# Intel-HLS/GenomicsDB

Measured on AMD Instinct MI355X. Metric: combined-gVCF positions/sec, higher is better.
Workload: dtype u8/int32

## Files before the change

__graft_entry__.py:

```python
import os
import sys

ROOT = os.path.dirname(os.path.abspath(__file__))
sys.path.insert(0, ROOT)
sys.path.insert(0, os.path.join(ROOT, "tests"))


def build():
    from genomicsdb_amd import build as b
    lib = b.build_native(verbose=True)
    b.build_oracle()
    b.build_hostsim()
    b.build_hostsim_variants()
    b.build_hostsim_import()
    b.build_hostsim_inflate()
    b.build_hostsim_import_bcf()
    b.build_hostsim_import_csv()
    b.build_hostsim_dispatch()
    b.build_hostsim_merge()
    b.build_hostsim_merge_files()
    b.build_hostsim_split()
    b.build_hostsim_histogram()
    b.build_hostsim_index()
    b.build_hostsim_vcfdiff()
    b.build_hostsim_import_stream()
    b.build_hostsim_columns()
    b.build_jni_importer_harness()
    from genomicsdb_amd import synth
    synth.lib()
    import genomicsdb_amd
    from genomicsdb_amd import _lib
    L = _lib.lib()
    for s in _lib.SYMBOLS:
        getattr(L, s)
    print("built", lib)


def smoke():
    import helpers
    from golden_cases import CASES
    import genomicsdb_amd
    case = [c for c in CASES if c[0] == "t6_7_8_vcf_at_0"][0]
    name, callsets, vid, ov, golden, mode = case
    cells = helpers.cells_for(callsets, vid)
    q, pb = helpers.query_json(callsets, vid, ov, mode)
    want, _, _ = helpers.oracle_run(q, cells)
    s = genomicsdb_amd.GenomicsDBQueryStream(query_json=q, cells=cells, buffer_capacity=4096)
    got = s.read()
    s.close()
    assert got == want, "device output differs from the oracle"
    assert got == helpers.golden_text(golden)
    print("smoke ok: %d bytes, bit-exact vs oracle and reference golden" % len(got))


if __name__ == "__main__":
    build()
    if len(sys.argv) > 1 and sys.argv[1] == "smoke":
        smoke()
```

genomicsdb_amd/build.py:

```python
import os
import subprocess
import sys

PKG = os.path.dirname(os.path.abspath(__file__))
ROOT = os.path.dirname(PKG)
CSRC = os.path.join(PKG, "csrc")
OBJ = os.path.join(ROOT, "build", "obj")
LIB = os.path.join(PKG, "libgenomicsdb_amd.so")
TOOL = os.path.join(PKG, "gt_mpi_gather")
TOOLS = {"gt_mpi_gather": TOOL, "vcf2tiledb": os.path.join(PKG, "vcf2tiledb"), "test_genomicsdb_importer": os.path.join(PKG, "test_genomicsdb_importer"),
         "vcf_histogram": os.path.join(PKG, "vcf_histogram"), "vcfdiff": os.path.join(PKG, "vcfdiff")}

SOURCES = [
    "kernels/gdb_pipeline.hip",
    "kernels/gdb_bgzf.hip",
    "kernels/gdb_import.hip",
    "kernels/gdb_import_stream.hip",
    "kernels/gdb_inflate.hip",
    "kernels/gdb_merge.hip",
    "kernels/gdb_split.hip",
    "kernels/gdb_histogram.hip",
    "kernels/gdb_index.hip",
    "kernels/gdb_vcfdiff.hip",
    "kernels/gdb_columns.hip",
# ... 83 lines not shown

def build_hostsim():
    subprocess.check_call(["make", "-s", "-C", os.path.join(ROOT, "tests", "hostsim")])
    subprocess.check_call(["make", "-s", "-C", os.path.join(ROOT, "tests", "jni_harness")])
    subprocess.check_call(["make", "-s", "-C", os.path.join(ROOT, "tests", "compat")])


def build_hostsim_variants():
    subprocess.check_call(["make", "-s", "-C", os.path.join(ROOT, "tests", "hostsim_variants")])
    return os.path.join(ROOT, "tests", "hostsim_variants", "libhostsim_variants.so")


def build_hostsim_import():
    subprocess.check_call(["make", "-s", "-C", os.path.join(ROOT, "tests", "hostsim_import")])
    return os.path.join(ROOT, "tests", "hostsim_import", "libhostsim_import.so")


def build_hostsim_import_bcf():
    d = os.path.join(ROOT, "tests", "hostsim_import_bcf")
    subprocess.check_call(["make", "-s", "-C", d])
    return os.path.join(d, "libhostsim_import_bcf.so"), os.path.join(d, "malformed_bcf")


def build_hostsim_import_csv():
    d = os.path.join(ROOT, "tests", "hostsim_import_csv")
    subprocess.check_call(["make", "-s", "-C", d])
    return os.path.join(d, "libhostsim_import_csv.so"), os.path.join(d, "hostsim_import_csv_main")


def build_hostsim_import_stream():
    d = os.path.join(ROOT, "tests", "hostsim_import_stream")
    subprocess.check_call(["make", "-s", "-C", d])
    return os.path.join(d, "libhostsim_import_stream.so"), os.path.join(d, "hostsim_import_stream_main")


def build_jni_importer_harness():
    d = os.path.join(ROOT, "tests", "jni_importer_harness")
    subprocess.check_call(["make", "-s", "-C", d])
    return os.path.join(d, "jni_importer_harness")


def build_hostsim_merge():
    d = os.path.join(ROOT, "tests", "hostsim_merge")
    subprocess.check_call(["make", "-s", "-C", d])
    return os.path.join(d, "libhostsim_merge.so"), os.path.join(d, "hostsim_merge_main")


def build_hostsim_merge_files():
    d = os.path.join(ROOT, "tests", "hostsim_merge_files")
    subprocess.check_call(["make", "-s", "-C", d])
    return os.path.join(d, "libhostsim_merge_files.so"), os.path.join(d, "hostsim_merge_files_main")


def build_hostsim_split():
    d = os.path.join(ROOT, "tests", "hostsim_split")
    subprocess.check_call(["make", "-s", "-C", d])
    return os.path.join(d, "hostsim_split")


def build_hostsim_histogram():
    d = os.path.join(ROOT, "tests", "hostsim_histogram")
    subprocess.check_call(["make", "-s", "-C", d])
    return os.path.join(d, "hostsim_histogram")


def build_hostsim_index():
    d = os.path.join(ROOT, "tests", "hostsim_index")
    subprocess.check_call(["make", "-s", "-C", d])
    return os.path.join(d, "libhostsim_index.so"), os.path.join(d, "hostsim_index")


def build_hostsim_vcfdiff():
    d = os.path.join(ROOT, "tests", "hostsim_vcfdiff")
    subprocess.check_call(["make", "-s", "-C", d])
    return os.path.join(d, "hostsim_vcfdiff")


def build_hostsim_columns():
    d = os.path.join(ROOT, "tests", "hostsim_columns")
    subprocess.check_call(["make", "-s", "-C", d])
    return os.path.join(d, "libhostsim_columns.so"), os.path.join(d, "hostsim_columns_main")


def build_hostsim_inflate():
    subprocess.check_call(["make", "-s", "-C", os.path.join(ROOT, "tests", "hostsim_inflate")])
    return os.path.join(ROOT, "tests", "hostsim_inflate", "libhostsim_inflate.so")


def build_hostsim_tile_inflate():
    d = os.path.join(ROOT, "tests", "hostsim_tile_inflate")
    subprocess.check_call(["make", "-s", "-C", d])
    return os.path.join(d, "libhostsim_tile_inflate.so"), os.path.join(d, "tile_inflate_fuzz")


def build_hostsim_dispatch():
    subprocess.check_call(["make", "-s", "-C", os.path.join(ROOT, "tests", "hostsim_dispatch")])
    return os.path.join(ROOT, "tests", "hostsim_dispatch", "libhostsim_dispatch.so")


if __name__ == "__main__":
    print(build_native(verbose=True))
    print(build_oracle())
```

genomicsdb_amd/csrc/core/gdb_core.hpp:

```cpp
#pragma once
#include "gdb_types.h"

#if defined(__HIP_DEVICE_COMPILE__)
#define GDB_FETCH_ADD_U64(p, v) atomicAdd((unsigned long long*)(p), (unsigned long long)(v))
#else
static inline unsigned long long gdb_fetch_add_u64(unsigned long long* p, unsigned long long v) { const unsigned long long o = *p; *p = o + v; return o; }
#define GDB_FETCH_ADD_U64(p, v) gdb_fetch_add_u64((unsigned long long*)(p), (unsigned long long)(v))
#endif

#define GDB_CF_REFBLOCK 1u
#define GDB_CF_DELETION 2u
#define GDB_CF_HAS_NR 4u
#define GDB_CF_HEAVY 8u
#define GDB_CF_IN_WINDOW 16u
#define GDB_CF_NALT(f) (((f) >> 8) & 0xFFu)
#define GDB_CF_PLOIDY(f) (((f) >> 16) & 0xFu)

#define GDB_RF_NON_REF_EXISTS 1u
#define GDB_RF_REMAPPING_NEEDED 2u
#define GDB_RF_SKIP_G_FIELDS 4u

#define GDB_IF_SPANNING 1u
#define GDB_IF_GT_OVERRIDE 2u
#define GDB_IF_NO_NR 4u
// ... 58 lines not shown
};
struct ByteSink {
  char* p;
  char* base;
  GDB_HD explicit ByteSink(char* q) : p(q), base(q) {}
  GDB_HD void put(char c) { *p++ = c; }
  GDB_HD void write(const char* s, int len) { for (int i = 0; i < len; ++i) *p++ = s[i]; }
  GDB_HD uint32_t pos() const { return (uint32_t)(p - base); }
  GDB_HD void patch_u32(uint32_t at, uint32_t v) { for (int i = 0; i < 4; ++i) base[at + i] = (char)((v >> (8 * i)) & 0xFFu); }
};

#if defined(__HIPCC__)
typedef __attribute__((address_space(3))) char gdb_lds_char;
struct LdsCapSink {
  gdb_lds_char* p;
  uint32_t n, cap;
  __device__ __forceinline__ LdsCapSink(gdb_lds_char* q, uint32_t c) : p(q), n(0), cap(c) {}
  __device__ __forceinline__ void put(char c) { if (n < cap) p[n] = c; ++n; }
  __device__ __forceinline__ void write(const char* s, int len) { for (int i = 0; i < len; ++i) put(s[i]); }
  __device__ __forceinline__ void put_word(uint64_t w, int len) {
    if (n + 8u <= cap) { const uint32_t a = (uint32_t)(uintptr_t)p + n; asm volatile("ds_write_b64 %0, %1" ::"v"(a), "v"(w) : "memory"); n += (uint32_t)len; }
    else for (int i = 0; i < len; ++i) { put((char)(w & 0xFFu)); w >>= 8; }
  }
  __device__ __forceinline__ uint32_t pos() const { return n; }
  __device__ __forceinline__ void patch_u32(uint32_t at, uint32_t v) { for (int i = 0; i < 4; ++i) if (at + i < cap) p[at + i] = (char)((v >> (8 * i)) & 0xFFu); }
};
constexpr uint32_t kSpillTail = 512;
struct SpillPool { char* buf; };
struct LdsSpillSink {
  gdb_lds_char* p;
  uint32_t n, cap;
  uint32_t acc;
  char* tail;
  __device__ __forceinline__ LdsSpillSink(gdb_lds_char* q, uint32_t c, const SpillPool& sp, int64_t record) : p(q), n(0), cap(c), acc(0), tail(sp.buf + (size_t)record * kSpillTail) {}
  __device__ __forceinline__ void put(char c) {
    if (n < cap) p[n] = c;
    else {
      const uint32_t at = n - cap;
      acc |= (uint32_t)(uint8_t)c << (8u * (at & 3u));
      if ((at & 3u) == 3u) { if (at < kSpillTail) *reinterpret_cast<uint32_t*>(tail + (at & ~3u)) = acc; acc = 0; }
    }
    ++n;
  }
  __device__ __forceinline__ void flush() { if (n > cap && ((n - cap) & 3u) && n - cap < kSpillTail) { *reinterpret_cast<uint32_t*>(tail + ((n - cap) & ~3u)) = acc; acc = 0; } }
  __device__ __forceinline__ void write(const char* s, int len) { for (int i = 0; i < len; ++i) put(s[i]); }
  __device__ __forceinline__ void put_word(uint64_t w, int len) {
    if (n + 8u <= cap) { const uint32_t a = (uint32_t)(uintptr_t)p + n; asm volatile("ds_write_b64 %0, %1" ::"v"(a), "v"(w) : "memory"); n += (uint32_t)len; }
    else for (int i = 0; i < len; ++i) { put((char)(w & 0xFFu)); w >>= 8; }
  }
  __device__ __forceinline__ bool complete() const { return n <= cap + kSpillTail; }
  __device__ __forceinline__ uint32_t pos() const { return n; }
  __device__ __forceinline__ void patch_u32(uint32_t at, uint32_t v) { for (int i = 0; i < 4; ++i) if (at + i < cap) p[at + i] = (char)((v >> (8 * i)) & 0xFFu); }
};
#endif

GDB_HD uint32_t gdb_f2u(float f) { union { float f; uint32_t u; } x; x.f = f; return x.u; }
GDB_HD bool gdb_int_valid(int32_t v) { return v != GDB_BCF_INT32_MISSING && v != GDB_BCF_INT32_VECTOR_END; }
GDB_HD bool gdb_float_valid(float v) { uint32_t u = gdb_f2u(v); return u != GDB_BCF_FLOAT_MISSING_BITS && u != GDB_BCF_FLOAT_VECTOR_END_BITS; }
GDB_HD int gdb_alleles2gt(int a, int b) { return a > b ? a * (a + 1) / 2 + b : b * (b + 1) / 2 + a; }
GDB_HD int64_t gdb_choose(int n, int k) {
  if (k < 0 || k > n) return 0;
  int64_t r = 1;
  for (int i = 1; i <= k; ++i) r = r * (n - k + i) / i;
  return r;
}
GDB_HD int64_t gdb_genotype_index_sorted(const int* a, int p) {
  int64_t g = 0;
  for (int i = 0; i < p; ++i) g += gdb_choose(a[i] + i, i + 1);
  return g;
}
GDB_HD int64_t gdb_genotype_index(const int* a, int p) {
  int t[GDB_MAX_PLOIDY];
  for (int i = 0; i < p; ++i) { int v = a[i], j = i; while (j > 0 && t[j - 1] > v) { t[j] = t[j - 1]; --j; } t[j] = v; }
  return gdb_genotype_index_sorted(t, p);
}
GDB_HD bool gdb_next_genotype(int* a, int p, int nalleles) {
  for (int i = 0; i < p; ++i) {
    const int bound = i + 1 < p ? a[i + 1] : nalleles - 1;
    if (a[i] < bound) { ++a[i]; for (int j = 0; j < i; ++j) a[j] = 0; return true; }
  }
  return false;
}

template <class Sink> GDB_HD void put_u64(Sink& s, uint64_t v) {
  char buf[20];
  int n = 0;
  do { buf[n++] = (char)('0' + (v % 10)); v /= 10; } while (v);
  while (n) s.put(buf[--n]);
}
template <class Sink> GDB_HD void put_i64(Sink& s, int64_t v) {
  if (v < 0) { s.put('-'); put_u64(s, (uint64_t)(-(v + 1)) + 1u); } else put_u64(s, (uint64_t)v);
}
GDB_HD uint64_t gdb_pack_digits(uint32_t v, int& n) {
  uint64_t w = 0;
  n = 0;
  do { const uint32_t q = v / 10u; w = (w << 8) | (uint64_t)('0' + (v - q * 10u)); v = q; ++n; } while (v);
  return w;
}
template <class Sink> GDB_HD void put_packed(Sink& s, uint64_t w, int n) {
  for (int i = 0; i < n; ++i) { s.put((char)(w & 0xFFu)); w >>= 8; }
}
#if defined(__HIPCC__)
__device__ __forceinline__ void put_packed(LdsCapSink& s, uint64_t w, int n) { s.put_word(w, n); }
__device__ __forceinline__ void put_packed(LdsSpillSink& s, uint64_t w, int n) { s.put_word(w, n); }
#endif
template <class Sink> GDB_HD void put_u32(Sink& s, uint32_t v) {
  if (v < 10u) { s.put((char)('0' + v)); return; }
  if (v < 100u) { const uint32_t q = v / 10u; s.put((char)('0' + q)); s.put((char)('0' + (v - q * 10u))); return; }
  int n = 0;
  if (v >= 100000000u) {
    const uint32_t hi = v / 100000000u;
    v -= hi * 100000000u;
    const uint64_t wh = gdb_pack_digits(hi, n);
    put_packed(s, wh, n);
    uint64_t w = gdb_pack_digits(v, n);
    for (; n < 8; ++n) w = (w << 8) | (uint64_t)'0';
    put_packed(s, w, 8);
    return;
  }
  const uint64_t w = gdb_pack_digits(v, n);
  put_packed(s, w, n);
}
template <class Sink> GDB_HD void put_i32(Sink& s, int32_t v) {
  if (v < 0) { s.put('-'); put_u32(s, 0u - (uint32_t)v); } else put_u32(s, (uint32_t)v);
}

struct GdbBig { uint32_t w[7]; };
GDB_HD void gdb_big_mul10(GdbBig& b) {
  uint64_t c = 0;
  for (int i = 0; i < 7; ++i) { const uint64_t t = (uint64_t)b.w[i] * 10u + c; b.w[i] = (uint32_t)t; c = t >> 32; }
}
GDB_HD uint32_t gdb_big_divmod10(GdbBig& b) {
  uint64_t r = 0;
  for (int i = 6; i >= 0; --i) { const uint64_t t = (r << 32) | b.w[i]; b.w[i] = (uint32_t)(t / 10u); r = t % 10u; }
  return (uint32_t)r;
}
GDB_HD bool gdb_big_is_zero(const GdbBig& b) { uint32_t o = 0; for (int i = 0; i < 7; ++i) o |= b.w[i]; return o == 0; }
GDB_HD uint32_t gdb_big_bit(const GdbBig& b, int i) { return i >= 0 && i < 224 ? (b.w[i >> 5] >> (i & 31)) & 1u : 0u; }
GDB_HD bool gdb_big_any_below(const GdbBig& b, int n) {
  uint32_t o = 0;
  for (int i = 0; i < 7; ++i) {
    const int lo = i * 32;
    if (n >= lo + 32) o |= b.w[i]; else if (n > lo) o |= b.w[i] & ((1u << (n - lo)) - 1u);
  }
  return o != 0;
}
GDB_HD GdbBig gdb_big_shr(const GdbBig& b, int n) {
  GdbBig r;
  const int ws = n >> 5, bs = n & 31;
  for (int i = 0; i < 7; ++i) {
    const uint32_t lo = i + ws < 7 ? b.w[i + ws] : 0u, hi = i + ws + 1 < 7 ? b.w[i + ws + 1] : 0u;
    r.w[i] = bs ? (lo >> bs) | (hi << (32 - bs)) : lo;
  }
  return r;
}
GDB_HD bool gdb_big_below(const GdbBig& b, uint32_t v) { uint32_t o = 0; for (int i = 1; i < 7; ++i) o |= b.w[i]; return o == 0 && b.w[0] < v; }
GDB_HD void gdb_round_6_digits(uint32_t M, int e2, uint32_t& q, int& X) {
  GdbBig N;
  for (int i = 0; i < 7; ++i) N.w[i] = 0;
  N.w[0] = M;
  bool up;
  if (e2 >= 0 || !gdb_big_below(gdb_big_shr(N, -e2), 100000u)) {
    int s = 0;
    if (e2 >= 0) { const int ws = e2 >> 5, bs = e2 & 31; N.w[ws] = M << bs; N.w[0] = ws ? 0u : N.w[0]; if (bs && ws + 1 < 7) N.w[ws + 1] = M >> (32 - bs); }
    else s = -e2;
    GdbBig I = gdb_big_shr(N, s);
    const bool half_bit = s > 0 && gdb_big_bit(N, s - 1);
    bool sticky = s > 1 && gdb_big_any_below(N, s - 1);
    int dropped = 0;
    uint32_t last = 0;
    while (!gdb_big_below(I, 1000000u)) { if (dropped) sticky = sticky || last != 0; else sticky = sticky || half_bit; last = gdb_big_divmod10(I); ++dropped; }
    q = I.w[0];
    if (dropped) up = last > 5u || (last == 5u && (sticky || (q & 1u)));
    else up = half_bit && (sticky || (q & 1u));
    X = 5 + dropped;
  } else {
    const int s = -e2;
    int k = 0;
    while (gdb_big_below(gdb_big_shr(N, s), 100000u)) { gdb_big_mul10(N); ++k; }
    q = gdb_big_shr(N, s).w[0];
    const bool half_bit = gdb_big_bit(N, s - 1) != 0, sticky = s > 1 && gdb_big_any_below(N, s - 1);
    up = half_bit && (sticky || (q & 1u));
    X = 5 - k;
  }
  if (up && ++q == 1000000u) { q = 100000u; ++X; }
}
template <class Sink> GDB_HD void put_float_g(Sink& s, float f) {
  const uint32_t u = gdb_f2u(f) & 0x7FFFFFFFu;
  const uint32_t ex = u >> 23, man = u & 0x7FFFFFu;
  uint32_t q; int X;
  gdb_round_6_digits(ex ? man | 0x800000u : man, ex ? (int)ex - 150 : -149, q, X);
  char dg[6];
  for (int i = 5; i >= 0; --i) { dg[i] = (char)('0' + q % 10u); q /= 10u; }
  int last = 5;
  while (last > 0 && dg[last] == '0') --last;
  if (X < -4 || X >= 6) {
    s.put(dg[0]);
    if (last > 0) { s.put('.'); for (int i = 1; i <= last; ++i) s.put(dg[i]); }
    s.put('e');
    uint32_t ax = (uint32_t)(X < 0 ? -X : X);
    s.put(X < 0 ? '-' : '+');
    if (ax < 10u) s.put('0');
    put_u64(s, ax);
  } else if (X >= 0) {
    for (int i = 0; i <= X; ++i) s.put(dg[i]);
    if (last > X) { s.put('.'); for (int i = X + 1; i <= last; ++i) s.put(dg[i]); }
  } else {
    s.put('0'); s.put('.');
    for (int i = 0; i < -X - 1; ++i) s.put('0');
    for (int i = 0; i <= last; ++i) s.put(dg[i]);
  }
}

template <class Sink> GDB_HD bool put_float(Sink& s, float f) {
  const uint32_t bits = gdb_f2u(f);
  if ((bits & 0x7F800000u) == 0x7F800000u) {
    if (bits >> 31) s.put('-');
    if (bits & 0x7FFFFFu) { s.put('n'); s.put('a'); s.put('n'); } else { s.put('i'); s.put('n'); s.put('f'); }
    return true;
  }
  double d = (double)f;
  if (d == 0) { if (bits >> 31) s.put('-'); s.put('0'); return true; }
  if (d < 0) { s.put('-'); d = -d; }
  if (!(d >= 0.0001 && d <= 999999)) { put_float_g(s, f); return true; }
  uint64_t i = (uint64_t)(d * 10000000000.0);
  if (d < 0.001) i += 5; else if (d < 0.01) i += 50; else if (d < 0.1) i += 500; else if (d < 1) i += 5000;
  else if (d < 10) i += 50000; else if (d < 100) i += 500000; else if (d < 1000) i += 5000000;
  else if (d < 10000) i += 50000000; else if (d < 100000) i += 500000000; else i += 5000000000ULL;
  char dg[24];
  int p = 0;
  { char tmp[24]; int n = 0; do { tmp[n++] = (char)('0' + i % 10); i /= 10; } while (i); while (n) dg[p++] = tmp[--n]; }
  char out[40];
  int m = 0, dot = -1;
  if (p <= 10) {
    out[m++] = '0'; dot = m; out[m++] = '.';
    for (int z = 0; z < 10 - p; ++z) out[m++] = '0';
    int take = p < 6 ? p : 6;
    for (int z = 0; z < take; ++z) out[m++] = dg[z];
  } else {
    int ip = p - 10;
    for (int z = 0; z < ip; ++z) out[m++] = dg[z];
    if (ip < 6) { dot = m; out[m++] = '.'; for (int z = ip; z < 6; ++z) out[m++] = dg[z]; }
  }
  if (dot >= 0) while (m > dot + 2 && out[m - 1] == '0') --m;
  s.write(out, m);
  return true;
}

template <class T> GDB_HD const T* cell_field(const FragmentView& fr, const CombinePlan& pl, int f, int64_t c, int& n) {
  const GdbColumn& col = fr.col[f];
  if (col.off) { uint32_t a = col.off[c], b = col.off[c + 1]; n = (int)(b - a); return (const T*)col.data + a; }
  n = pl.field[f].fixed_num;
  return (const T*)col.data + (int64_t)c * n;
}
GDB_HD bool field_valid(const CellMeta& cm, int64_t c, int f) { return (cm.vmask[c] >> f) & 1ull; }

GDB_HD bool alt_token(const char* s, int len, int idx, const char*& tok, int& tlen) {
  int i = 0, k = -1;
  while (i < len) {
    while (i < len && s[i] == '|') ++i;
    if (i >= len) break;
    int j = i;
    while (j < len && s[j] != '|') ++j;
    if (++k == idx) { tok = s + i; tlen = j - i; return true; }
    i = j;
  }
  return false;
}
GDB_HD bool allele_is_symbolic(const char* a, int n) {
  if (n > 0 && a[0] == '&') return true;
  if (n == 1 && a[0] == '*') return true;
  if (n > 0 && a[0] == '<' && a[n - 1] == '>') return true;
  for (int i = 0; i < n; ++i) if (a[i] == '[' || a[i] == ']') return true;
  return false;
}
GDB_HD bool allele_is_deletion(int ref_len, const char* a, int n) {
  return ref_len > 1 && ((n == 1 && a[0] == '*') || (!allele_is_symbolic(a, n) && n < ref_len));
}

GDB_HD void classify_cell(const FragmentView& fr, const CombinePlan& pl, const CellMeta& cm, int64_t c, uint32_t* err) {
  uint64_t vmask = 0;
  for (int f = 0; f < pl.nfields; ++f) {
    const GdbFieldDesc& fd = pl.field[f];
    int n;
    bool valid = false;
    if (fd.elem == GDB_ET_INT) {
      const int32_t* p = cell_field<int32_t>(fr, pl, f, c, n);
      for (int i = 0; i < n; ++i) if (p[i] != GDB_TILEDB_NULL_INT32) { valid = true; break; }
    } else if (fd.elem == GDB_ET_FLOAT) {
      const float* p = cell_field<float>(fr, pl, f, c, n);
      for (int i = 0; i < n; ++i) if (gdb_f2u(p[i]) != GDB_TILEDB_NULL_FLOAT_BITS) { valid = true; break; }
    } else {
      const char* p = cell_field<char>(fr, pl, f, c, n);
      for (int i = 0; i < n; ++i) if (p[i] != GDB_TILEDB_NULL_CHAR) { valid = true; break; }
    }
    if (valid) vmask |= 1ull << f;
  }
  uint32_t flags = 0;
  int nalt = 0, ref_len = 0;
  if (pl.f_REF >= 0 && pl.f_ALT >= 0 && ((vmask >> pl.f_REF) & 1) && ((vmask >> pl.f_ALT) & 1)) {
    int alt_len;
    cell_field<char>(fr, pl, pl.f_REF, c, ref_len);
    const char* alt = cell_field<char>(fr, pl, pl.f_ALT, c, alt_len);
    bool deletion = false, has_nr = false;
    const char* tok; int tl;
    for (int i = 0; alt_token(alt, alt_len, i, tok, tl); ++i) {
      ++nalt;
      if (tl > 0 && tok[0] == '&') has_nr = true;
      if (ref_len > 1 && !allele_is_symbolic(tok, tl) && tl < ref_len) deletion = true;
    }
    if (deletion) flags |= GDB_CF_DELETION;
    if (has_nr) flags |= GDB_CF_HAS_NR;
    if (ref_len == 1 && nalt == 1 && has_nr) flags |= GDB_CF_REFBLOCK;
  }
  if (nalt + 1 > GDB_MAX_INPUT_ALLELES) { *err |= GDB_ERR_TOO_MANY_INPUT_ALLELES; nalt = GDB_MAX_INPUT_ALLELES - 1; }
  int ploidy = 0;
  if (pl.f_GT >= 0 && ((vmask >> pl.f_GT) & 1)) {
    int n;
    cell_field<int32_t>(fr, pl, pl.f_GT, c, n);
    ploidy = pl.field[pl.f_GT].length == GDB_VL_PP ? (n + 1) >> 1 : n;
    if (ploidy > 15) ploidy = 15;
  }
  bool heavy = !(flags & GDB_CF_REFBLOCK);
  for (int i = 0; i < pl.n_info; ++i) if ((vmask >> pl.info_field[i]) & 1) heavy = true;
  for (int i = 0; i < pl.n_histogram; ++i) if ((vmask >> pl.histogram_bin_field[i]) & 1) heavy = true;
  if (pl.qual_combine_op != GDB_OP_UNKNOWN && pl.f_QUAL >= 0 && ((vmask >> pl.f_QUAL) & 1)) heavy = true;
  if (pl.produce_FILTER_field && pl.f_FILTER >= 0 && ((vmask >> pl.f_FILTER) & 1)) heavy = true;
  if (pl.f_ID >= 0 && ((vmask >> pl.f_ID) & 1)) heavy = true;
  if (heavy) flags |= GDB_CF_HEAVY;
  flags |= ((uint32_t)nalt & 0xFFu) << 8;
  flags |= ((uint32_t)ploidy & 0xFu) << 16;
  int32_t dp = 0;
  {
    int n; bool got = false;
    if (pl.f_DP >= 0 && ((vmask >> pl.f_DP) & 1)) { const int32_t* p = cell_field<int32_t>(fr, pl, pl.f_DP, c, n); if (n > 0 && gdb_int_valid(p[0])) { dp = p[0]; got = true; } }
    if (!got && pl.f_MIN_DP >= 0 && ((vmask >> pl.f_MIN_DP) & 1)) { const int32_t* p = cell_field<int32_t>(fr, pl, pl.f_MIN_DP, c, n); if (n > 0 && gdb_int_valid(p[0])) { dp = p[0]; got = true; } }
    if (!got && pl.f_DP_FORMAT >= 0 && ((vmask >> pl.f_DP_FORMAT) & 1)) { const int32_t* p = cell_field<int32_t>(fr, pl, pl.f_DP_FORMAT, c, n); if (n > 0 && gdb_int_valid(p[0])) { dp = p[0]; got = true; } }
  }
  cm.vmask[c] = vmask;
  cm.cflags[c] = flags;
  cm.dpval[c] = dp;
}

GDB_HD uint32_t allele_hash(const char* p, int len, int suffix_from, const char* mref, int mref_len) {
  uint32_t h = 2166136261u;
  for (int i = 0; i < len; ++i) h = (h ^ (uint32_t)(unsigned char)p[i]) * 16777619u;
  if (suffix_from >= 0) for (int i = suffix_from; i < mref_len; ++i) h = (h ^ (uint32_t)(unsigned char)mref[i]) * 16777619u;
  return h;
}

GDB_HD bool allele_equal(const AlleleRef& a, const AlleleRef& b, const char* mref, int mref_len) {
  if (a.hash != b.hash) return false;
  int la = a.len + (a.suffix_from >= 0 ? mref_len - a.suffix_from : 0);
  int lb = b.len + (b.suffix_from >= 0 ? mref_len - b.suffix_from : 0);
  if (la != lb) return false;
  for (int i = 0; i < la; ++i) {
    char ca = i < a.len ? a.p[i] : mref[a.suffix_from + (i - a.len)];
    char cb = i < b.len ? b.p[i] : mref[b.suffix_from + (i - b.len)];
    if (ca != cb) return false;
  }
  return true;
}

struct MedianOrder {
  const uint64_t* keys;
  const uint32_t* inc;
  int64_t stride;
  int8_t slot[GDB_MAX_FIELDS];
  int32_t enabled;
};
GDB_HD uint32_t gdb_orderable_bits(float v) {
  uint32_t u = gdb_f2u(v);
  if (u == 0x80000000u) u = 0;
  return (u & 0x80000000u) ? ~u : (u | 0x80000000u);
}
GDB_HD uint32_t gdb_orderable_bits(int32_t v) { return (uint32_t)v ^ 0x80000000u; }

struct BigMedians {
  const int32_t* index;
  const uint32_t* value;
  const uint8_t* ok;
  int64_t stride;
  int8_t slot[GDB_MAX_FIELDS];
  int32_t enabled;
};

GDB_HD void gdb_swapf(float* a, int64_t i, int64_t j) { const float t = a[i]; a[i] = a[j]; a[j] = t; }
GDB_HD void gdb_heap_adjust(float* a, int64_t hole, int64_t len, float value) {
  const int64_t top = hole;
// ... 191 lines not shown
  ++s.n;
}
GDB_HD void gdb_id_union_add(const char* p, int len, const char** tp, int* tn, int& nt, GdbUSetHashOrder& us, int release_order, uint32_t* err) {
  if (release_order) {
    for (int i = 0; i < nt; ++i) {
      if (tn[i] != len) continue;
      bool same = true;
      for (int j = 0; j < len && same; ++j) same = tp[i][j] == p[j];
      if (same) return;
    }
    if (nt >= GDB_MAX_ID_TOKENS) { *err |= GDB_ERR_TOO_MANY_ID_TOKENS; return; }
    tp[nt] = p; tn[nt] = len;
    gdb_useth_insert_new(us, gdb_libstdcxx_hash_bytes(p, len), nt);
    ++nt;
    return;
  }
  int pos = 0, cmp = 1;
  for (; pos < nt; ++pos) {
    const int m = len < tn[pos] ? len : tn[pos];
    cmp = 0;
    for (int j = 0; j < m && cmp == 0; ++j) cmp = (int)(unsigned char)p[j] - (int)(unsigned char)tp[pos][j];
    if (cmp == 0) cmp = len - tn[pos];
    if (cmp <= 0) break;
  }
  if (pos == nt || cmp != 0) {
    if (nt >= GDB_MAX_ID_TOKENS) { *err |= GDB_ERR_TOO_MANY_ID_TOKENS; }
    else { for (int j = nt; j > pos; --j) { tp[j] = tp[j - 1]; tn[j] = tn[j - 1]; } tp[pos] = p; tn[pos] = len; ++nt; }
  }
}
GDB_HD void gdb_id_union_value(const char* p, int n, const char** tp, int* tn, int& nt, GdbUSetHashOrder& us, int release_order, uint32_t* err) {
  int last = 0;
  for (int i = 0; i <= n; ++i) {
    if (i < n && p[i] != ';') continue;
    const int len = i - last;
    if (i == n && len == 0) break;
    gdb_id_union_add(p + last, len, tp, tn, nt, us, release_order, err);
    last = i + 1;
  }
}
GDB_HD int gdb_id_union_at(const GdbUSetHashOrder& us, int release_order, int i) { return release_order ? us.tok[i] : i; }

struct TieScratch {
  float* buf;
  unsigned long long* used;
  uint64_t capacity;
};

struct ScalarPre {
  const uint32_t* val;
  int64_t stride;
  int8_t slot[GDB_MAX_FIELDS];
  int32_t enabled;
};

struct HugeScalar { int64_t nvalid, nbelow, nneg0, npos0; uint32_t sum_bits, median_bits; int32_t median_ok, pad; };
struct HugeSiteOut {
  AlleleRef merged[GDB_MAX_MERGED_ALLELES];
  const char* mref;
  int32_t mref_len, nmerged;
  int32_t filter_first_id, filter_multi, any_id, fallback;
  HugeScalar scalar[GDB_MAX_INFO_FIELDS + 2];
};
struct HugeSites {
  const int32_t* index;
  const HugeSiteOut* out;
  int32_t enabled;
};

struct SiteCtx {
  FragmentView fr;
  CombinePlan pl;
  CellMeta cm;
  RecordTable rec;
  HeavyLists hl;
  PresenceCounts pc;
  NameTables names;
  QueryWindow qw;
  SiteOut so;
  MedianOrder med;
  BigMedians big;
  TieScratch tie;
  ScalarPre pre;
  HugeSites huge;
};

GDB_HD bool inc_is_spanning(const SiteCtx& cx, int64_t t, int64_t s_k) {
  int64_t c = cx.hl.cell[t];
  return (cx.cm.cflags[c] & GDB_CF_DELETION) && s_k > cx.fr.begin[c];
}
template <class T> GDB_HD bool scalar_at(const SiteCtx& cx, const uint32_t* pre, int64_t t, int64_t s_k, int f, bool keep_spanning, bool is_float, T& v,
                                         int alt_merged = 0, bool non_ref_exists = false) {
  if (pre) {
    union { uint32_t u; T v; } x;
    x.u = pre[t];
    if (is_float ? x.u == GDB_BCF_FLOAT_MISSING_BITS : x.u == (uint32_t)GDB_BCF_INT32_MISSING) return false;
    v = x.v;
    return true;
  }
  if (!keep_spanning && inc_is_spanning(cx, t, s_k)) return false;
  const int64_t c = cx.hl.cell[t];
  if (!field_valid(cx.cm, c, f)) return false;
  int n;
  const T* p = cell_field<T>(cx.fr, cx.pl, f, c, n);
  int idx = 0;
  if (alt_merged > 0) {
    const int8_t* lut = cx.hl.i2m + cx.hl.i2m_off[t];
    const int nal = (int)GDB_CF_NALT(cx.cm.cflags[c]) + 1;
    int in = -1;
    for (int a = 0; a < nal; ++a) if (lut[a] == 1) { in = a; break; }
    if (in < 0 && non_ref_exists) for (int a = 0; a < nal; ++a) if (lut[a] == alt_merged - 1) in = a;
    idx = in - 1;
    if (in < 0 || idx < 0 || idx >= n) return false;
  }
  v = p[idx];
  return is_float ? gdb_float_valid((float)v) : gdb_int_valid((int32_t)v);
}
template <class T> GDB_HD bool reduce_scalar(const SiteCtx& cx, int64_t k, int f, int op, bool keep_spanning, T& result, uint32_t* err, int num_merged = 0,
                                             bool non_ref_exists = false, bool remapping_needed = false) {
  const int alt_merged = (remapping_needed && cx.pl.field[f].length == GDB_VL_A) ? num_merged : 0;
  const int64_t b = cx.hl.base[k], e = cx.hl.base[k + 1];
  if (op == GDB_OP_MEDIAN && cx.big.enabled && cx.big.slot[f] >= 0 && cx.big.index[k] >= 0) {
    const int64_t at = (int64_t)cx.big.slot[f] * cx.big.stride + cx.big.index[k];
    if (!cx.big.ok[at]) return false;
    if (cx.big.ok[at] == 1) {
      union { uint32_t u; T v; } x;
      x.u = cx.big.value[at];
      result = x.v;
      return true;
    }
  }
  const int64_t s_k = cx.rec.start[k];
  const bool is_float = cx.pl.field[f].elem == GDB_ET_FLOAT;
  const uint32_t* pre = (cx.pre.enabled && cx.pre.slot[f] >= 0) ? cx.pre.val + (int64_t)cx.pre.slot[f] * cx.pre.stride : nullptr;
  int64_t nvalid = 0, nbelow = 0, nneg0 = 0, npos0 = 0;
  T sum = 0;
  const HugeSiteOut* hs = (cx.huge.enabled && pre && cx.huge.index[k] >= 0 && !cx.huge.out[cx.huge.index[k]].fallback) ? &cx.huge.out[cx.huge.index[k]] : nullptr;
  if (hs) {
    const HugeScalar& hv = hs->scalar[cx.pre.slot[f]];
    nvalid = hv.nvalid; nbelow = hv.nbelow; nneg0 = hv.nneg0; npos0 = hv.npos0;
    union { uint32_t u; T v; } x;
    x.u = hv.sum_bits; sum = x.v;
    if (nvalid && op == GDB_OP_MEDIAN && hv.median_ok == 1) { x.u = hv.median_bits; result = x.v; return true; }
  } else
  for (int64_t t = b; t < e; ++t) {
    T v;
    if (!scalar_at<T>(cx, pre, t, s_k, f, keep_spanning, is_float, v, alt_merged, non_ref_exists)) continue;
    sum += v;
    ++nvalid;
    if (is_float) {
      const uint32_t u = gdb_f2u((float)v);
      nneg0 += u == 0x80000000u;
      npos0 += u == 0u;
      nbelow += v < (T)0;
    }
  }
  if (!nvalid) return false;
  if (op == GDB_OP_SUM) { result = sum; return true; }
  if (op == GDB_OP_MEAN) {
    if (is_float) result = sum / (T)nvalid;
    else result = (T)(int32_t)((uint32_t)(int32_t)sum / (uint32_t)nvalid);
    return true;
  }
  if (is_float && nneg0 && npos0 && nbelow <= nvalid / 2 && nvalid / 2 < nbelow + nneg0 + npos0) {
    const uint64_t at = cx.tie.buf ? GDB_FETCH_ADD_U64(cx.tie.used, (uint64_t)nvalid) : 0;
    if (!cx.tie.buf || at + (uint64_t)nvalid > cx.tie.capacity) { *err |= GDB_ERR_INTERNAL; return false; }
    float* a = cx.tie.buf + at;
// ... 213 lines not shown
}

template <class T, class Sink> GDB_HD bool info_vector_combine_bcf(const SiteCtx& cx, int64_t k, int f, int op, int num_merged, bool non_ref_exists, bool remapping_needed,
                                                                 Sink& sink, uint32_t* err) {
  const CombinePlan& pl = cx.pl;
  const GdbFieldDesc& fd = pl.field[f];
  const int64_t b = cx.hl.base[k], e = cx.hl.base[k + 1];
  const int64_t s_k = cx.rec.start[k];
  const int mode = info_element_mode(fd, remapping_needed);
  const bool is_float = fd.elem == GDB_ET_FLOAT;
  T r[GDB_MAX_INFO_VECTOR];
  int num_valid = 0;
  int n_total = 0;
  int32_t mn = INT32_MAX, mx = INT32_MIN + 1;
  int type = is_float ? GDB_BT_FLOAT : GDB_BT_INT8;
  for (int pass = (op == GDB_OP_CONCATENATE ? 0 : 1); pass < 2; ++pass) {
    if (pass == 1 && op == GDB_OP_CONCATENATE) {
      if (n_total == 0) return false;
      bcf_enc_int1(sink, pl.bcf_id[f]);
      if (!is_float) type = bcf_int_type(mn, mx);
      if (!is_float && n_total == 1) {}
      bcf_enc_size(sink, n_total, type);
    }
    for (int64_t t = b; t < e; ++t) {
      if (inc_is_spanning(cx, t, s_k)) continue;
      const int64_t c = cx.hl.cell[t];
      if (!field_valid(cx.cm, c, f)) continue;
      int n_in;
      const T* p = cell_field<T>(cx.fr, pl, f, c, n_in);
      info_for_each_element<T>(p, n_in, mode, cx.hl.i2m + cx.hl.i2m_off[t], (int)GDB_CF_NALT(cx.cm.cflags[c]) + 1, num_merged, non_ref_exists, (int)GDB_CF_PLOIDY(cx.cm.cflags[c]), err,
                               [&](int i, T v) -> bool {
        if (op == GDB_OP_CONCATENATE) {
          if (pass == 0) {
            ++n_total;
            if (!is_float && !elem_is_missing(v) && !elem_is_vector_end(v)) { const int32_t iv = (int32_t)v; if (iv < mn) mn = iv; if (iv > mx) mx = iv; }
          } else if (is_float) { union { T t; uint32_t u; } x; x.u = 0; x.t = v; bcf_put_u32(sink, x.u); }
          else bcf_put_int(sink, (int32_t)v, type);
          return true;
        }
        if (elem_is_missing(v) || elem_is_vector_end(v)) return true;
        if (i >= GDB_MAX_INFO_VECTOR) { *err |= GDB_ERR_INFO_VECTOR_TOO_LONG; return false; }
        if (i < num_valid && !elem_is_missing(r[i])) r[i] += v;
        else { r[i] = v; if (i >= num_valid) { for (int j = num_valid; j < i; ++j) elem_set_missing(r[j]); num_valid = i + 1; } }
        return true;
      });
    }
  }
  if (op == GDB_OP_CONCATENATE) return true;
  if (num_valid == 0) return false;
  bcf_enc_int1(sink, pl.bcf_id[f]);
  if (is_float) {
    bcf_enc_size(sink, num_valid, GDB_BT_FLOAT);
    for (int i = 0; i < num_valid; ++i) { union { T t; uint32_t u; } x; x.u = 0; x.t = r[i]; bcf_put_u32(sink, x.u); }
  } else {
    int32_t tmp[GDB_MAX_INFO_VECTOR];
    for (int i = 0; i < num_valid; ++i) tmp[i] = (int32_t)r[i];
    bcf_enc_vint(sink, tmp, num_valid);
  }
  return true;
}

#include "gdb_asa.hpp"

constexpr int kMergeScan = 8;
struct MergeIndex { uint8_t slot[256]; bool built; };
GDB_HD int merged_find_or_add(AlleleRef* merged, int& nmerged, MergeIndex& ix, const AlleleRef& cand, const char* mref, int mref_len, uint32_t* err) {
  if (nmerged <= kMergeScan) {
    for (int j = 1; j < nmerged; ++j) if (allele_equal(merged[j], cand, mref, mref_len)) return j;
  } else {
    if (!ix.built) {
      for (int h = 0; h < 256; ++h) ix.slot[h] = 0;
      for (int j = 1; j < nmerged; ++j) { uint32_t h = merged[j].hash & 255u; while (ix.slot[h]) h = (h + 1) & 255u; ix.slot[h] = (uint8_t)j; }
      ix.built = true;
    }
    for (uint32_t h = cand.hash & 255u; ix.slot[h]; h = (h + 1) & 255u)
      if (allele_equal(merged[ix.slot[h]], cand, mref, mref_len)) return ix.slot[h];
  }
  if (nmerged >= GDB_MAX_MERGED_ALLELES - 1) { *err |= GDB_ERR_TOO_MANY_MERGED_ALLELES; return nmerged - 1; }
  merged[nmerged] = cand;
  if (ix.built) { uint32_t h = cand.hash & 255u; while (ix.slot[h]) h = (h + 1) & 255u; ix.slot[h] = (uint8_t)nmerged; }
  return nmerged++;
}

GDB_HD const char* site_first_ref(const SiteCtx& cx, int64_t s_k, int& len) {
  int64_t lo = 0, hi = cx.fr.ncells;
  while (lo < hi) { int64_t mid = (lo + hi) >> 1; if (cx.fr.begin[mid] < s_k) lo = mid + 1; else hi = mid; }
  len = 0;
  if (lo < cx.fr.ncells && cx.fr.begin[lo] == s_k && field_valid(cx.cm, lo, cx.pl.f_REF)) return cell_field<char>(cx.fr, cx.pl, cx.pl.f_REF, lo, len);
  return nullptr;
}
GDB_HD const char* gdb_star_allele() { return "*"; }
template <class F> GDB_HD void site_merge_call(const SiteCtx& cx, int64_t t, int64_t s_k, const char* mref, int mref_len, bool write_luts, F& find_or_add, uint32_t* err) {
  const CombinePlan& pl = cx.pl;
    int64_t c = cx.hl.cell[t];
    uint32_t cf = cx.cm.cflags[c];
    int ref_len = 0, alt_len = 0;
    cell_field<char>(cx.fr, pl, pl.f_REF, c, ref_len);
    const char* alt = cell_field<char>(cx.fr, pl, pl.f_ALT, c, alt_len);
    int nalt = (int)GDB_CF_NALT(cf);
    int8_t* lut = write_luts ? cx.hl.i2m + cx.hl.i2m_off[t] : nullptr;
    bool spanning = (cf & GDB_CF_DELETION) && s_k > cx.fr.begin[c];
    uint8_t iflag = 0;
    if (lut) { lut[0] = 0; for (int a = 1; a <= nalt; ++a) lut[a] = -1; }
    if (spanning) {
      iflag |= GDB_IF_SPANNING;
      if (!(cf & GDB_CF_HAS_NR)) iflag |= GDB_IF_NO_NR;
      int ploidy = (int)GDB_CF_PLOIDY(cf);
      int npl = 0;
      const int32_t* plv = nullptr;
      bool pl_exists = pl.f_PL >= 0 && field_valid(cx.cm, c, pl.f_PL);
      if (pl_exists) plv = cell_field<int32_t>(cx.fr, pl, pl.f_PL, c, npl);
      int lowest = -1;
      int lowest_pl = 0x7FFFFFFF;
      const char* tok; int tl;
      for (int i = 0; alt_token(alt, alt_len, i, tok, tl); ++i) {
        int aidx = i + 1;
        if (allele_is_deletion(ref_len, tok, tl)) {
          if (lowest < 0) lowest = aidx;
          if (pl_exists) {
            int64_t gt_idx;
            if (ploidy == 0) gt_idx = 0;
            else if (ploidy == 1) gt_idx = aidx;
            else if (ploidy == 2) gt_idx = gdb_alleles2gt(aidx, aidx);
            else if (ploidy <= GDB_MAX_PLOIDY) { int hom[GDB_MAX_PLOIDY]; for (int q = 0; q < ploidy; ++q) hom[q] = aidx; gt_idx = gdb_genotype_index_sorted(hom, ploidy); }
            else { *err |= GDB_ERR_UNSUPPORTED_PLOIDY; gt_idx = 0x7FFFFFFF; }
            if (gt_idx < npl && plv[gt_idx] < lowest_pl) { lowest_pl = plv[gt_idx]; lowest = aidx; }
          }
        }
      }
      if (lowest < 0) { *err |= GDB_ERR_INTERNAL; lowest = 1; }
      AlleleRef cand{gdb_star_allele(), 1, -1, 0u};
      cand.hash = allele_hash(cand.p, cand.len, cand.suffix_from, mref, mref_len);
      const int found = find_or_add(cand);
      if (lut) lut[lowest] = (int8_t)found;
      if (lut && pl.min_PL_GT_for_spanning_deletions && pl.produce_GT_field && pl_exists && pl.f_GT >= 0 && field_valid(cx.cm, c, pl.f_GT)) {
        int nr_idx = -1;
        for (int i = 0; alt_token(alt, alt_len, i, tok, tl); ++i) if (tl > 0 && tok[0] == '&') nr_idx = i + 1;
        int red2in[3] = {0, lowest, nr_idx};
        int nred = nr_idx >= 0 ? 3 : 2;
        int best_min = 0x7FFFFFFF, best_a = -1, best_b = -1;
        if (ploidy == 1) {
          for (int a = 0; a < nred; ++a) {
            int64_t gi = red2in[a];
            int32_t v = gi < npl ? plv[gi] : GDB_BCF_INT32_MISSING;
            if (gdb_int_valid(v) && v < best_min) { best_min = v; best_a = a; }
          }
        } else if (ploidy == 2) {
          for (int a = 0; a < nred; ++a) for (int b2 = a; b2 < nred; ++b2) {
            int64_t gi = gdb_alleles2gt(red2in[a], red2in[b2]);
            int32_t v = gi < npl ? plv[gi] : GDB_BCF_INT32_MISSING;
            if (gdb_int_valid(v) && v < best_min) { best_min = v; best_a = a; best_b = b2; }
          }
        } else if (ploidy <= GDB_MAX_PLOIDY) {
          int g[GDB_MAX_PLOIDY], in[GDB_MAX_PLOIDY];
          for (int q = 0; q < ploidy; ++q) g[q] = 0;
          do {
            for (int q = 0; q < ploidy; ++q) in[q] = red2in[g[q]];
            const int64_t gi = gdb_genotype_index(in, ploidy);
            const int32_t v = gi < npl ? plv[gi] : GDB_BCF_INT32_MISSING;
            if (gdb_int_valid(v) && v < best_min) {
              best_min = v; best_a = g[0];
              for (int q = 0; q < ploidy; ++q) cx.hl.gt_override[GDB_MAX_PLOIDY * t + q] = (int8_t)g[q];
            }
          } while (gdb_next_genotype(g, ploidy, nred));
        } else *err |= GDB_ERR_UNSUPPORTED_PLOIDY;
        if (best_a >= 0) {
          iflag |= GDB_IF_GT_OVERRIDE;
          if (ploidy <= 2) {
            cx.hl.gt_override[GDB_MAX_PLOIDY * t] = (int8_t)best_a;
            cx.hl.gt_override[GDB_MAX_PLOIDY * t + 1] = (int8_t)best_b;
          }
        }
      }
    } else {
      bool suffix_needed = ref_len < mref_len;
      const char* tok; int tl;
      for (int i = 0; alt_token(alt, alt_len, i, tok, tl); ++i) {
        if (tl > 0 && tok[0] == '&') continue;
        AlleleRef cand{tok, tl, (suffix_needed && !allele_is_symbolic(tok, tl)) ? ref_len : -1, 0u};
        cand.hash = allele_hash(cand.p, cand.len, cand.suffix_from, mref, mref_len);
        const int found = find_or_add(cand);
        if (lut && i + 1 <= nalt) lut[i + 1] = (int8_t)found;
      }
    }
    if (write_luts) cx.hl.iflags[t] = iflag;
}

template <class Sink> GDB_HD void site_emit(const SiteCtx& cx, int64_t k, Sink& sink, bool write_luts, uint32_t* err) {
  const CombinePlan& pl = cx.pl;
  const int64_t s_k = cx.rec.start[k], e_k = cx.rec.end[k];
  const int64_t hb = cx.hl.base[k], he = cx.hl.base[k + 1];
  const char* mref = nullptr;
  int mref_len = 0;
  char ref_base = 'N';
  const HugeSiteOut* hsite = (cx.huge.enabled && cx.huge.index[k] >= 0 && !cx.huge.out[cx.huge.index[k]].fallback) ? &cx.huge.out[cx.huge.index[k]] : nullptr;
  {
    if (hsite) { mref = hsite->mref; mref_len = hsite->mref_len; }
    else mref = site_first_ref(cx, s_k, mref_len);
    if (!hsite) for (int64_t t = hb; t < he; ++t) {
      int64_t c = cx.hl.cell[t];
      if (cx.fr.begin[c] != s_k || !field_valid(cx.cm, c, pl.f_REF)) continue;
      int n;
      const char* r = cell_field<char>(cx.fr, pl, pl.f_REF, c, n);
      if (n > mref_len) { mref = r; mref_len = n; }
    }
    if (mref_len == 0 || (mref_len == 1 && mref[0] == 'N')) {
      int64_t off = s_k - cx.qw.ref_begin;
      char b = (cx.qw.ref_bases && off >= 0 && off < cx.qw.ref_len) ? cx.qw.ref_bases[off] : 'N';
      ref_base = (b == 'A' || b == 'C' || b == 'G' || b == 'T') ? b : 'N';
      mref = &ref_base;
      mref_len = 1;
    }
  }
  AlleleRef merged[GDB_MAX_MERGED_ALLELES];
  MergeIndex mix;
  mix.built = false;
  int nmerged = 1;
  bool non_ref_exists = cx.pc.nr_cnt[k] > 0;
  if (hsite) {
    nmerged = hsite->nmerged;
    for (int j = 1; j < nmerged; ++j) merged[j] = hsite->merged[j];
  } else {
    struct SerialMerge {
      AlleleRef* merged; int* nmerged; MergeIndex* mix; const char* mref; int mref_len; uint32_t* err;
      GDB_HD int operator()(const AlleleRef& cand) { return merged_find_or_add(merged, *nmerged, *mix, cand, mref, mref_len, err); }
    } fa{merged, &nmerged, &mix, mref, mref_len, err};
    for (int64_t t = hb; t < he; ++t) site_merge_call(cx, t, s_k, mref, mref_len, write_luts, fa, err);
  }
  const int num_merged = nmerged + (non_ref_exists ? 1 : 0);
  if (write_luts && non_ref_exists && !hsite) {
    for (int64_t t = hb; t < he; ++t) {
      int64_t c = cx.hl.cell[t];
      uint32_t cf = cx.cm.cflags[c];
      if (!(cf & GDB_CF_HAS_NR)) continue;
      int alt_len;
      const char* alt = cell_field<char>(cx.fr, pl, pl.f_ALT, c, alt_len);
      const char* tok; int tl;
      for (int i = 0; alt_token(alt, alt_len, i, tok, tl); ++i)
        if (tl > 0 && tok[0] == '&' && i + 1 <= (int)GDB_CF_NALT(cf)) cx.hl.i2m[cx.hl.i2m_off[t] + i + 1] = (int8_t)(num_merged - 1);
    }
  }
  const bool ref_block_only = (mref_len == 1 && nmerged == 1 && non_ref_exists);
  const bool skip_G = (num_merged - 1) > pl.max_diploid_alt_alleles;
  uint32_t fmt_mask = 0;
  if (!pl.sites_only_query)
    for (int i = 0; i < pl.n_format; ++i) {
      int f = pl.format_field[i];
      if (cx.pc.fmt_cnt[(int64_t)i * cx.pc.stride + k] <= 0) continue;
      if (pl.field[f].length == GDB_VL_G && skip_G) continue;
      fmt_mask |= 1u << i;
    }
  if (write_luts) {
    cx.so.num_alleles[k] = (uint8_t)num_merged;
    cx.so.rflags[k] = (uint8_t)((non_ref_exists ? GDB_RF_NON_REF_EXISTS : 0) | (!ref_block_only ? GDB_RF_REMAPPING_NEEDED : 0) | (skip_G ? GDB_RF_SKIP_G_FIELDS : 0));
    cx.so.fmt_mask[k] = fmt_mask;
  }
  int ci = find_contig(cx.qw, s_k);
  if (ci < 0) { *err |= GDB_ERR_INTERNAL; ci = 0; }
  const GdbContig& ctg = cx.qw.contigs[ci];
  if (pl.bcf_mode) {
    int n_fmt = 0;
    for (uint32_t m = fmt_mask; m; m &= m - 1) ++n_fmt;
    bcf_put_u32(sink, (uint32_t)ctg.rid);
    bcf_put_u32(sink, (uint32_t)(s_k - ctg.offset));
    bcf_put_u32(sink, (uint32_t)(e_k > s_k ? e_k - s_k + 1 : (int64_t)mref_len));
    float qv;
    uint32_t qbits = GDB_BCF_FLOAT_MISSING_BITS;
    if (pl.qual_combine_op != GDB_OP_UNKNOWN && pl.f_QUAL >= 0 && reduce_scalar<float>(cx, k, pl.f_QUAL, pl.qual_combine_op, true, qv, err)) qbits = gdb_f2u(qv);
    bcf_put_u32(sink, qbits);
    const uint32_t at_counts = sink.pos();
    bcf_put_u32(sink, (uint32_t)num_merged << 16);
    bcf_put_u32(sink, ((uint32_t)n_fmt << 24) | ((uint32_t)pl.bcf_n_sample & 0xFFFFFFu));
    {
      const char* tp[GDB_MAX_ID_TOKENS]; int tn[GDB_MAX_ID_TOKENS]; int nt = 0;
      GdbUSetHashOrder us;
      gdb_useth_init(us);
      if (pl.f_ID >= 0 && !(hsite && !hsite->any_id))
        for (int64_t t = hb; t < he; ++t) {
          const int64_t c = cx.hl.cell[t];
          if (!field_valid(cx.cm, c, pl.f_ID)) continue;
          int n;
          const char* p = cell_field<char>(cx.fr, pl, pl.f_ID, c, n);
          gdb_id_union_value(p, n, tp, tn, nt, us, pl.id_order_unordered_set, err);
        }
      int total = nt ? nt - 1 : 0;
      for (int i = 0; i < nt; ++i) total += tn[i];
      bcf_enc_size(sink, total, GDB_BT_CHAR);
      for (int i = 0; i < nt; ++i) { const int w = gdb_id_union_at(us, pl.id_order_unordered_set, i); if (i) sink.put(';'); sink.write(tp[w], tn[w]); }
    }
    bcf_enc_size(sink, mref_len, GDB_BT_CHAR);
    sink.write(mref, mref_len);
    for (int j = 1; j < nmerged; ++j) {
      const int sl = merged[j].suffix_from >= 0 ? mref_len - merged[j].suffix_from : 0;
      bcf_enc_size(sink, merged[j].len + sl, GDB_BT_CHAR);
      sink.write(merged[j].p, merged[j].len);
      if (sl) sink.write(mref + merged[j].suffix_from, sl);
    }
    if (non_ref_exists) { const char nr[] = "<NON_REF>"; bcf_enc_size(sink, 9, GDB_BT_CHAR); sink.write(nr, 9); }
    {
      int first_id = -1;
      bool multi = false;
      if (hsite) { first_id = hsite->filter_first_id; multi = hsite->filter_multi != 0; }
      else if (pl.produce_FILTER_field && pl.f_FILTER >= 0)
        for (int64_t t = hb; t < he; ++t) {
          int64_t c = cx.hl.cell[t];
          if (!field_valid(cx.cm, c, pl.f_FILTER)) continue;
          int n;
          const int32_t* p = cell_field<int32_t>(cx.fr, pl, pl.f_FILTER, c, n);
          for (int i = 0; i < n; ++i) { if (first_id < 0) first_id = p[i]; else if (p[i] != first_id) multi = true; }
        }
      if (multi) {
        GdbUSetOrder us;
        filter_union_order(cx, hb, he, us, err);
        int32_t hids[GDB_MAX_FILTER_IDS];
        int nh = 0;
        for (int i = 0; i < us.n; ++i) {
          const int32_t id = us.key[i];
          const int32_t hid = (id >= 0 && id < cx.names.n_filter_names) ? cx.names.filter_bcf_id[id] : -1;
          if (hid >= 0) hids[nh++] = hid;
        }
        bcf_enc_vint(sink, hids, nh);
      } else {
        const int32_t hid = (first_id >= 0 && first_id < cx.names.n_filter_names) ? cx.names.filter_bcf_id[first_id] : -1;
        if (hid >= 0) bcf_enc_int1(sink, hid); else sink.put((char)0);
      }
    }
    uint32_t n_info = 0;
    if (e_k > s_k) { bcf_enc_int1(sink, pl.bcf_end_id); bcf_enc_int1(sink, (int32_t)(e_k - ctg.offset + 1)); ++n_info; }
    for (int i = 0; i < pl.n_info; ++i) {
      const int f = pl.info_field[i];
      const GdbFieldDesc& fd = pl.field[f];
      if (fd.length == GDB_VL_G && (num_merged - 1) > pl.max_diploid_alt_alleles) continue;
      if (fd.ndim == 2) { bool any2 = false; if (info_asa_sum(cx, k, f, num_merged, non_ref_exists, !ref_block_only, true, sink, any2, err)) ++n_info; continue; }
      if (fd.combine_op == GDB_OP_ELEMENT_WISE_SUM || fd.combine_op == GDB_OP_CONCATENATE) {
        bool found;
        if (fd.elem == GDB_ET_FLOAT) found = info_vector_combine_bcf<float>(cx, k, f, fd.combine_op, num_merged, non_ref_exists, !ref_block_only, sink, err);
        else found = info_vector_combine_bcf<int32_t>(cx, k, f, fd.combine_op, num_merged, non_ref_exists, !ref_block_only, sink, err);
        if (found) ++n_info;
        continue;
      }
      if (fd.elem == GDB_ET_FLOAT) {
        float v;
        if (!reduce_scalar<float>(cx, k, f, fd.combine_op, false, v, err, num_merged, non_ref_exists, !ref_block_only)) continue;
// ... 57 lines not shown
  }
  sink.put('\t');
  {
    int first_id = -1;
    bool multi = false;
    if (hsite) { first_id = hsite->filter_first_id; multi = hsite->filter_multi != 0; }
    else if (pl.produce_FILTER_field && pl.f_FILTER >= 0)
      for (int64_t t = hb; t < he; ++t) {
        int64_t c = cx.hl.cell[t];
        if (!field_valid(cx.cm, c, pl.f_FILTER)) continue;
        int n;
        const int32_t* p = cell_field<int32_t>(cx.fr, pl, pl.f_FILTER, c, n);
        for (int i = 0; i < n; ++i) { if (first_id < 0) first_id = p[i]; else if (p[i] != first_id) multi = true; }
      }
    if (multi) {
      GdbUSetOrder us;
      filter_union_order(cx, hb, he, us, err);
      bool any = false;
      for (int i = 0; i < us.n; ++i) {
        const int32_t id = us.key[i];
        if (!(id >= 0 && id < cx.names.n_filter_names && cx.names.filter_name_len[id] > 0)) continue;
        if (any) sink.put(';');
        sink.write(cx.names.text + cx.names.filter_name_off[id], cx.names.filter_name_len[id]);
        any = true;
      }
      if (!any) sink.put('.');
    } else if (first_id >= 0 && first_id < cx.names.n_filter_names && cx.names.filter_name_len[first_id] > 0)
      sink.write(cx.names.text + cx.names.filter_name_off[first_id], cx.names.filter_name_len[first_id]);
    else sink.put('.');
  }
  sink.put('\t');
  {
    bool any = false;
    if (e_k > s_k) { const char t[] = "END="; sink.write(t, 4); put_i64(sink, e_k - ctg.offset + 1); any = true; }
    for (int i = 0; i < pl.n_info; ++i) {
      int f = pl.info_field[i];
      const GdbFieldDesc& fd = pl.field[f];
      if (fd.length == GDB_VL_G && (num_merged - 1) > pl.max_diploid_alt_alleles) continue;
      if (fd.ndim == 2) { info_asa_sum(cx, k, f, num_merged, non_ref_exists, !ref_block_only, false, sink, any, err); continue; }
      if (fd.combine_op == GDB_OP_ELEMENT_WISE_SUM || fd.combine_op == GDB_OP_CONCATENATE) {
        if (fd.elem == GDB_ET_FLOAT) info_vector_combine<float>(cx, k, f, fd.combine_op, num_merged, non_ref_exists, !ref_block_only, sink, any, err);
        else info_vector_combine<int32_t>(cx, k, f, fd.combine_op, num_merged, non_ref_exists, !ref_block_only, sink, any, err);
        continue;
      }
      if (fd.elem == GDB_ET_FLOAT) {
        float v;
        if (!reduce_scalar<float>(cx, k, f, fd.combine_op, false, v, err, num_merged, non_ref_exists, !ref_block_only)) continue;
        if (any) sink.put(';');
        sink.write(cx.names.text + cx.names.field_name_off[f], cx.names.field_name_len[f]);
        sink.put('=');
        put_float(sink, v);
      } else {
        int32_t v;
        if (!reduce_scalar<int32_t>(cx, k, f, fd.combine_op, false, v, err, num_merged, non_ref_exists, !ref_block_only)) continue;
        if (any) sink.put(';');
        sink.write(cx.names.text + cx.names.field_name_off[f], cx.names.field_name_len[f]);
        sink.put('=');
        put_i32(sink, v);
      }
      any = true;
    }
    for (int i = 0; i < pl.n_histogram; ++i)
      info_asa_histogram(cx, k, pl.histogram_bin_field[i], pl.histogram_count_field[i], num_merged, non_ref_exists, !ref_block_only, false, sink, any, err);
    int32_t dp = cx.pc.dp_sum[k];
    if ((pl.f_DP >= 0 || pl.f_DP_FORMAT >= 0) && dp > 0 && !ref_block_only) {
      if (any) sink.put(';');
      const char t[] = "DP="; sink.write(t, 3); put_i32(sink, dp);
      any = true;
    }
    if (!any) sink.put('.');
  }
  if (fmt_mask) {
    sink.put('\t');
    bool first = true;
    for (int i = 0; i < pl.n_format; ++i) {
      if (!((fmt_mask >> i) & 1)) continue;
      if (!first) sink.put(':');
      first = false;
      int f = pl.format_field[i];
      if (f == pl.f_DP_FORMAT || f == pl.f_DP) { sink.put('D'); sink.put('P'); }
      else sink.write(cx.names.text + cx.names.field_name_off[f], cx.names.field_name_len[f]);
    }
  }
}

struct EntryCtx {
  FragmentView fr;
  CombinePlan pl;
  CellMeta cm;
  HeavyLists hl;
};
struct RecordInfo { int num_merged; uint32_t rflags; uint32_t fmt_mask; int64_t hbase, hend; };

template <class Sink> GDB_HD void put_int_vector(Sink& s, const int32_t* p, int n) {
  if (n == 0) { s.put('.'); return; }
  for (int j = 0; j < n; ++j) {
    if (p[j] == GDB_BCF_INT32_VECTOR_END) break;
    if (j) s.put(',');
    if (p[j] == GDB_BCF_INT32_MISSING) s.put('.'); else put_i32(s, p[j]);
  }
}
template <class Sink> GDB_HD void put_int_or_missing(Sink& s, bool has, int32_t v) {
  if (!has || v == GDB_BCF_INT32_MISSING) s.put('.'); else put_i32(s, v);
}

struct EntryMaps {
  int8_t* m2i;
  const int8_t* i2m;
  int nr_in;
  int n_in;
  int64_t inc;
  uint32_t cf;
  uint8_t iflag;
  bool remap, nr_exists;
  bool light;
  GDB_HD int lookup(int j) const {
    if (light) return j == 0 ? 0 : nr_in;
    const int v = m2i[j];
    return v >= 0 ? v : nr_in;
  }
};

#define GDB_FIELD_FN GDB_HD

GDB_FIELD_FN int32_t gt_merged_allele(const EntryCtx& cx, const RecordInfo& ri, const EntryMaps& em, int32_t a, int out_i) {
  int32_t m = -1;
  if (em.iflag & GDB_IF_GT_OVERRIDE) {
    const int ra = cx.hl.gt_override[GDB_MAX_PLOIDY * em.inc + (out_i < GDB_MAX_PLOIDY ? out_i : GDB_MAX_PLOIDY - 1)];
    if (ra == 0) m = 0;
    else if (ra == 2) m = ri.num_merged - 1;
    else { for (int q = 1; q < em.n_in; ++q) if (em.i2m && em.i2m[q] >= 0 && em.i2m[q] != ri.num_merged - 1) { m = em.i2m[q]; break; } }
  } else if (a == GDB_TILEDB_NULL_INT32 || a == -1 || a == GDB_BCF_INT32_MISSING) {
    m = -1;
  } else if (!em.remap) {
    m = a;
  } else {
    int8_t mm = -1;
    if (a >= 0 && a < em.n_in) mm = em.i2m ? em.i2m[a] : (a == 0 ? (int8_t)0 : ((em.nr_exists && a == 1) ? (int8_t)(ri.num_merged - 1) : (int8_t)-1));
    if (mm >= 0) m = mm;
    else if ((em.iflag & GDB_IF_SPANNING) && (em.iflag & GDB_IF_NO_NR)) m = -1;
    else m = em.nr_exists ? ri.num_merged - 1 : -1;
  }
  return m;
}
template <class Sink> GDB_FIELD_FN Sink emit_GT(Sink s, const EntryCtx& cx, const RecordInfo& ri, const EntryMaps& em, int64_t c) {
  const CombinePlan& pl = cx.pl;
  const int f = pl.f_GT;
  int n;
  const int32_t* g = cell_field<int32_t>(cx.fr, pl, f, c, n);
  const bool pp = pl.field[f].length == GDB_VL_PP;
  const int step = pp ? 2 : 1;
  int out_i = 0;
  for (int j = 0; j < n; j += step, ++out_i) {
    if (out_i) s.put((pp && g[j - 1] > 0) ? '|' : '/');
    const int32_t m = pl.produce_GT_field ? gt_merged_allele(cx, ri, em, g[j], out_i) : -1;
    if (m < 0) s.put('.'); else put_i32(s, m);
  }
  if (out_i == 0) s.put('.');
  return s;
}

template <class Sink> GDB_FIELD_FN Sink emit_chars(Sink s, const EntryCtx& cx, int f, int64_t c) {
  int n;
  const char* p = cell_field<char>(cx.fr, cx.pl, f, c, n);
  int len = 0;
  while (len < n && p[len]) ++len;
// ... 169 lines not shown
```

genomicsdb_amd/csrc/core/gdb_stages.hpp:

```cpp
#pragma once
#include "gdb_core.hpp"

#if defined(__HIP_DEVICE_COMPILE__)
#define GDB_ATOMIC_ADD_I32(p, v) atomicAdd((int*)(p), (int)(v))
#define GDB_ATOMIC_OR_U32(p, v) atomicOr((unsigned*)(p), (unsigned)(v))
#define GDB_ATOMIC_ADD_U64(p, v) atomicAdd((unsigned long long*)(p), (unsigned long long)(v))
#else
#define GDB_ATOMIC_ADD_I32(p, v) (*(p) += (v))
#define GDB_ATOMIC_OR_U32(p, v) (*(p) |= (v))
#define GDB_ATOMIC_ADD_U64(p, v) (*(p) += (uint64_t)(v))
#endif

#define GDB_EVENT_SENTINEL 0xFFFFFFFFFFFFFFFFull

GDB_HD void stage_eff_end(const FragmentView& fr, const CellMeta& cm, const int64_t* perm, int64_t j, int64_t* rm_begin, int64_t* span, uint32_t* err) {
  const int64_t C = fr.ncells;
  const int64_t c = perm[j];
  int64_t eff = fr.end[c];
  if (j + 1 < C) {
    const int64_t nx = perm[j + 1];
    if (fr.row[nx] == fr.row[c] && fr.begin[nx] <= eff) {
      eff = fr.begin[nx] - 1;
      if (!(cm.cflags[c] & (GDB_CF_DELETION | GDB_CF_REFBLOCK))) *err |= GDB_ERR_OVERLAP_NOT_REFBLOCK_OR_DELETION;
    }
// ... 11 lines not shown
  keys += 2 * (c - c_base) - 2 * c;
  if (!cell_in_window(fr, cm, c, qb, qe)) { keys[2 * c] = GDB_EVENT_SENTINEL; keys[2 * c + 1] = GDB_EVENT_SENTINEL; return; }
  const int64_t b = fr.begin[c] > qb ? fr.begin[c] : qb;
  const int64_t e = cm.eff_end[c] < qe ? cm.eff_end[c] : qe;
  const uint64_t del = (f & GDB_CF_DELETION) ? 1u : 0u;
  keys[2 * c] = ((uint64_t)(b - qb) << 2) | del;
  keys[2 * c + 1] = ((uint64_t)(e + 1 - qb) << 2) | 2u | del;
}
GDB_HD void stage_marker_keys(const FragmentView& fr, int64_t m, int64_t qb, int64_t qe, uint64_t* two_keys) {
  const int64_t p = fr.marker_begin[m];
  if (p < qb || p > qe) { two_keys[0] = GDB_EVENT_SENTINEL; two_keys[1] = GDB_EVENT_SENTINEL; return; }
  two_keys[0] = (uint64_t)(p - qb) << 2;
  two_keys[1] = ((uint64_t)(p - qb) << 2) | 2u;
}
GDB_HD int64_t stage_event_delta(uint64_t key) {
  if (key == GDB_EVENT_SENTINEL) return 0;
  const int32_t dc = (key & 2u) ? -1 : 1;
  const int32_t dd = (key & 1u) ? dc : 0;
  return (int64_t)(((uint64_t)(uint32_t)dc << 32) | (uint64_t)(uint32_t)dd);
}
GDB_HD int64_t packed_add(int64_t a, int64_t b) {
  const uint32_t hi = (uint32_t)((uint64_t)a >> 32) + (uint32_t)((uint64_t)b >> 32);
  const uint32_t lo = (uint32_t)a + (uint32_t)b;
  return (int64_t)(((uint64_t)hi << 32) | lo);
}
GDB_HD int32_t stage_is_run_end(const uint64_t* keys, int64_t n_events, int64_t i) {
  if (keys[i] == GDB_EVENT_SENTINEL) return 0;
  if (i + 1 >= n_events || keys[i + 1] == GDB_EVENT_SENTINEL) return 1;
  return (keys[i] >> 2) != (keys[i + 1] >> 2);
}
struct Boundaries {
  int64_t* pos; int32_t* cov; int32_t* del; int64_t* nrec;
};
GDB_HD void stage_boundary_write(const uint64_t* keys, const int64_t* incl_scan, const int32_t* run_end_excl, int64_t i, int32_t is_end, const Boundaries& b, int64_t qb) {
  if (!is_end) return;
  const int64_t u = run_end_excl[i];
  b.pos[u] = (int64_t)(keys[i] >> 2) + qb;
  b.cov[u] = (int32_t)(uint32_t)((uint64_t)incl_scan[i] >> 32);
  b.del[u] = (int32_t)(uint32_t)incl_scan[i];
}
GDB_HD int64_t stage_boundary_nrec(const Boundaries& b, int64_t U, int64_t u) {
  if (u + 1 >= U || b.cov[u] <= 0) return 0;
  return b.del[u] > 0 ? (b.pos[u + 1] - b.pos[u]) : 1;
}
GDB_HD void stage_record_expand(const Boundaries& b, const int64_t* rbase, int64_t U, int64_t k, int64_t* rstart, int64_t* rend) {
  int64_t lo = 0, hi = U;
  while (lo < hi) { int64_t mid = (lo + hi) >> 1; if (rbase[mid] <= k) lo = mid + 1; else hi = mid; }
  const int64_t u = lo - 1;
  const int64_t t = k - rbase[u];
  if (b.del[u] > 0) { rstart[k] = b.pos[u] + t; rend[k] = b.pos[u] + t; }
  else { rstart[k] = b.pos[u]; rend[k] = b.pos[u + 1] - 1; }
}

GDB_HD int presence_field(const CombinePlan& pl, int i) {
  const int f = pl.format_field[i];
  if (f == pl.f_DP && pl.f_DP >= 0) return pl.f_DP_FORMAT;
  return f;
}
struct DiffArrays { int32_t* fmt; int32_t* dp; int32_t* nr; int64_t stride; };
struct DiffPacked { uint64_t* w; int64_t stride; int32_t width, per_word, nwords; };

GDB_HD bool stage_cell_range(const FragmentView& fr, const CellMeta& cm, const RecordTable& rec, int64_t c, int64_t c_base, int64_t qb, int64_t qe,
                             int64_t* heavy_count, const int32_t* first_record_at, int64_t& klo, int64_t& khi) {
  cm.k_lo[c] = -1; cm.k_hi[c] = -1; heavy_count[c - c_base] = 0;
  if (!cell_in_window(fr, cm, c, qb, qe) || rec.npos == 0) return false;
  const int64_t b = fr.begin[c] > qb ? fr.begin[c] : qb;
  const int64_t e = cm.eff_end[c] < qe ? cm.eff_end[c] : qe;
  if (first_record_at) {
    klo = first_record_at[b - qb];
    khi = (int64_t)first_record_at[e + 1 - qb] - 1;
  } else {
    int64_t lo = 0, hi = rec.npos;
    while (lo < hi) { int64_t mid = (lo + hi) >> 1; if (rec.start[mid] < b) lo = mid + 1; else hi = mid; }
    klo = lo;
    hi = rec.npos;
    while (lo < hi) { int64_t mid = (lo + hi) >> 1; if (rec.start[mid] <= e) lo = mid + 1; else hi = mid; }
    khi = lo - 1;
  }
  if (khi < klo) return false;
  cm.k_lo[c] = (int32_t)klo; cm.k_hi[c] = (int32_t)khi;
  if (cm.cflags[c] & GDB_CF_HEAVY) heavy_count[c - c_base] = khi - klo + 1;
  return true;
}
GDB_HD uint64_t stage_packed_word(const CombinePlan& pl, const DiffPacked& pk, uint64_t vmask, uint32_t cflags, int word) {
  uint64_t acc = 0;
  const int j0 = word * pk.per_word;
  for (int j = j0; j < j0 + pk.per_word && j <= pl.n_format; ++j) {
    bool on;
    if (j < pl.n_format) { const int pf = presence_field(pl, j); on = pf >= 0 && ((vmask >> pf) & 1); }
    else on = (cflags & GDB_CF_HAS_NR) != 0;
    if (on) acc |= 1ull << ((j - j0) * pk.width);
  }
  return acc;
}
GDB_HD void stage_cell_ranges(const FragmentView& fr, const CombinePlan& pl, const CellMeta& cm, const RecordTable& rec, int64_t c, int64_t c_base,
                              int64_t qb, int64_t qe, const DiffArrays& d, int64_t* heavy_count) {
  int64_t klo, khi;
  if (!stage_cell_range(fr, cm, rec, c, c_base, qb, qe, heavy_count, nullptr, klo, khi)) return;
  const uint32_t f = cm.cflags[c];
  const uint64_t vm = cm.vmask[c];
  for (int i = 0; i < pl.n_format; ++i) {
    const int pf = presence_field(pl, i);
    if (pf < 0 || !((vm >> pf) & 1)) continue;
    GDB_ATOMIC_ADD_I32(d.fmt + (int64_t)i * d.stride + klo, 1);
    GDB_ATOMIC_ADD_I32(d.fmt + (int64_t)i * d.stride + khi + 1, -1);
  }
  const int32_t dp = cm.dpval[c];
  if (dp) { GDB_ATOMIC_ADD_I32(d.dp + klo, dp); GDB_ATOMIC_ADD_I32(d.dp + khi + 1, -dp); }
  if (f & GDB_CF_HAS_NR) { GDB_ATOMIC_ADD_I32(d.nr + klo, 1); GDB_ATOMIC_ADD_I32(d.nr + khi + 1, -1); }
}

GDB_HD void stage_incidence_fill(const FragmentView& fr, const CellMeta& cm, const int64_t* hoff, int64_t c, int64_t c_base, int64_t nrows,
                                 uint64_t* keys, int64_t* vals, uint32_t* lut_len) {
  if (!(cm.cflags[c] & GDB_CF_HEAVY) || cm.k_lo[c] < 0) return;
  const int64_t base = hoff[c - c_base];
  const int64_t klo = cm.k_lo[c], khi = cm.k_hi[c];
  for (int64_t k = klo; k <= khi; ++k) {
    keys[base + (k - klo)] = (uint64_t)k * (uint64_t)nrows + (uint64_t)fr.row[c];
    vals[base + (k - klo)] = c;
  }
  (void)lut_len;
}
GDB_HD int64_t stage_heavy_base(const uint64_t* sorted_keys, int64_t T, int64_t nrows, int64_t k) {
  const uint64_t want = (uint64_t)k * (uint64_t)nrows;
  int64_t lo = 0, hi = T;
  while (lo < hi) { int64_t mid = (lo + hi) >> 1; if (sorted_keys[mid] < want) lo = mid + 1; else hi = mid; }
  return lo;
}

struct RowIndex {
  const int64_t* row_ptr;
  const int64_t* rm_cell;
  const int64_t* rm_begin;
};
struct RowWalker {
  int64_t j, j_begin, j_end;
  GDB_HD void init(const RowIndex& ri, int32_t row, int64_t s0) {
    j_begin = ri.row_ptr[row]; j_end = ri.row_ptr[row + 1];
    int64_t lo = j_begin, hi = j_end;
    while (lo < hi) { int64_t mid = (lo + hi) >> 1; if (ri.rm_begin[mid] <= s0) lo = mid + 1; else hi = mid; }
    j = lo - 1;
  }
  GDB_HD int64_t live(const RowIndex& ri, const CellMeta& cm, int64_t s) {
    while (j + 1 < j_end && ri.rm_begin[j + 1] <= s) ++j;
    if (j < j_begin) return -1;
    const int64_t c = ri.rm_cell[j];
    return (s <= cm.eff_end[c]) ? c : -1;
  }
};

GDB_HD RecordInfo load_record_info(const SiteOut& so, const HeavyLists& hl, int64_t k) {
  RecordInfo ri;
  ri.num_merged = so.num_alleles[k];
  ri.rflags = so.rflags[k];
  ri.fmt_mask = so.fmt_mask[k];
  ri.hbase = hl.base[k];
  ri.hend = hl.base[k + 1];
  return ri;
}
```

genomicsdb_amd/csrc/kernels/gdb_pipeline.hip:

```cpp
#include <hip/hip_runtime.h>

#include <fcntl.h>
#include <sys/stat.h>
#include <unistd.h>
#include <zlib.h>

#include <algorithm>
#include <cstdio>
#include <cstdlib>
#include <chrono>
#include <cstring>
#include <memory>
#include <mutex>
#include <thread>
#include <vector>

#include <rocprim/device/device_radix_sort.hpp>
#include <rocprim/device/device_reduce.hpp>
#include <rocprim/device/device_scan.hpp>
#include <rocprim/iterator/reverse_iterator.hpp>

#include "../core/gdb_stages.hpp"
#include "../core/gdb_bcf.hpp"
#include "../core/gdb_calls.hpp"
// ... 126 lines not shown
  row_ptr[r] = lo;
}
__global__ void k_eff_end(FragmentView fr, CellMeta cm, const int64_t* perm, int64_t* rm_begin, int64_t* span, uint32_t* err) {
  int64_t j = (int64_t)blockIdx.x * blockDim.x + threadIdx.x;
  if (j >= fr.ncells) return;
  uint32_t e = 0;
  stage_eff_end(fr, cm, perm, j, rm_begin, span, &e);
  if (e) atomicOr(err, e);
}
__global__ void k_cell_window(const int64_t* begin, int64_t C, int64_t lo_pos, int64_t hi_pos, int64_t* out) {
  if (blockIdx.x || threadIdx.x) return;
  int64_t lo = 0, hi = C;
  while (lo < hi) { int64_t mid = (lo + hi) >> 1; if (begin[mid] < lo_pos) lo = mid + 1; else hi = mid; }
  out[0] = lo;
  hi = C;
  while (lo < hi) { int64_t mid = (lo + hi) >> 1; if (begin[mid] <= hi_pos) lo = mid + 1; else hi = mid; }
  out[1] = lo;
}
__global__ void k_first_begin_at_or_after(const int64_t* begin, int64_t C, int64_t pos, int64_t* out) {
  if (blockIdx.x || threadIdx.x) return;
  int64_t lo = 0, hi = C;
  while (lo < hi) { const int64_t mid = (lo + hi) >> 1; if (begin[mid] < pos) lo = mid + 1; else hi = mid; }
  *out = lo < C ? begin[lo] : INT64_MAX;
}
__global__ void k_event_keys(FragmentView fr, CellMeta cm, int64_t c_base, int64_t n, int64_t qb, int64_t qe, uint64_t* keys) {
  int64_t i = (int64_t)blockIdx.x * blockDim.x + threadIdx.x;
  if (i >= n) return;
  stage_event_keys(fr, cm, c_base + i, c_base, qb, qe, keys);
}
__global__ void k_marker_keys(FragmentView fr, int64_t m_base, int64_t n, int64_t qb, int64_t qe, uint64_t* keys) {
  const int64_t i = (int64_t)blockIdx.x * blockDim.x + threadIdx.x;
  if (i < n) stage_marker_keys(fr, m_base + i, qb, qe, keys + 2 * i);
}
__global__ void k_event_delta(const uint64_t* keys, int64_t n, int64_t* delta, int32_t* run_end) {
  int64_t i = (int64_t)blockIdx.x * blockDim.x + threadIdx.x;
  if (i >= n) return;
  delta[i] = stage_event_delta(keys[i]);
  run_end[i] = stage_is_run_end(keys, n, i);
}
struct PackedAdd { __host__ __device__ int64_t operator()(const int64_t& a, const int64_t& b) const { return packed_add(a, b); } };
__global__ void k_boundary_write(const uint64_t* keys, const int64_t* incl, const int32_t* run_end, const int32_t* run_excl, int64_t n, Boundaries b, int64_t qb) {
  int64_t i = (int64_t)blockIdx.x * blockDim.x + threadIdx.x;
  if (i >= n) return;
  stage_boundary_write(keys, incl, run_excl, i, run_end[i], b, qb);
}
__global__ void k_boundary_nrec(Boundaries b, int64_t U) {
  int64_t u = (int64_t)blockIdx.x * blockDim.x + threadIdx.x;
  if (u >= U) return;
  b.nrec[u] = stage_boundary_nrec(b, U, u);
}
__global__ void k_record_expand(Boundaries b, const int64_t* rbase, int64_t U, int64_t P, int64_t* rstart, int64_t* rend) {
  int64_t k = (int64_t)blockIdx.x * blockDim.x + threadIdx.x;
  if (k >= P) return;
  stage_record_expand(b, rbase, U, k, rstart, rend);
}
__global__ void k_mark_record_starts(const int64_t* rstart, int64_t P, int64_t qb, int32_t* first_record_at) {
  const int64_t k = (int64_t)blockIdx.x * blockDim.x + threadIdx.x;
  if (k < P) first_record_at[rstart[k] - qb] = (int32_t)k;
}
__global__ void k_fill_i32(int32_t* p, int64_t n, int32_t v) {
  const int64_t i = (int64_t)blockIdx.x * blockDim.x + threadIdx.x;
  if (i < n) p[i] = v;
}
__global__ void k_unpack_counts(DiffPacked pk, int n_format, int64_t n, DiffArrays d) {
  const int64_t k = (int64_t)blockIdx.x * blockDim.x + threadIdx.x;
  if (k >= n) return;
  const uint64_t mask = pk.width >= 64 ? ~0ull : ((1ull << pk.width) - 1ull);
  for (int j = 0; j <= n_format; ++j) {
    const uint64_t w = pk.w[(int64_t)(j / pk.per_word) * pk.stride + k];
    const int32_t v = (int32_t)((w >> ((j % pk.per_word) * pk.width)) & mask);
    if (j < n_format) d.fmt[(int64_t)j * d.stride + k] = v; else d.nr[k] = v;
  }
  d.dp[k] = (int32_t)(int64_t)pk.w[(int64_t)(pk.nwords - 1) * pk.stride + k];
}
__device__ __forceinline__ uint64_t wave_run_sum(uint32_t key, uint64_t v, int lane) {
  for (int off = 1; off < 64; off <<= 1) {
    const uint32_t ok = __shfl_down(key, off, 64);
    const uint64_t ov = __shfl_down(v, off, 64);
    if (lane + off < 64 && ok == key) v += ov;
  }
  return v;
}
__global__ void k_cell_ranges(FragmentView fr, CombinePlan pl, CellMeta cm, RecordTable rec, int64_t c_base, int64_t n, int64_t qb, int64_t qe,
                              int64_t* heavy_count, int32_t* in_window_count, const int32_t* first_record_at, DiffPacked pk) {
  const int64_t i = (int64_t)blockIdx.x * blockDim.x + threadIdx.x;
  const int lane = threadIdx.x & 63;
  bool live = false;
  int64_t klo = -1 - (int64_t)lane, khi = -1;
  uint64_t vm = 0; uint32_t cf = 0; int32_t dp = 0;
  if (i < n) {
    const int64_t c = c_base + i;
    live = stage_cell_range(fr, cm, rec, c, c_base, qb, qe, heavy_count, first_record_at, klo, khi);
    if (live) { vm = cm.vmask[c]; cf = cm.cflags[c]; dp = cm.dpval[c]; } else klo = -1 - (int64_t)lane;
  }
  const int64_t prev_key = __shfl_up(klo, 1, 64);
  const bool head = lane == 0 || prev_key != klo;
  const uint32_t run_id = wave_inclusive_scan_dpp(head ? 1u : 0u);
  const int64_t prev_khi = __shfl_up(khi, 1, 64);
  const bool same_khi = live && lane > 0 && prev_key == klo && prev_khi == khi;
  const bool runs_end_together = __popcll(__ballot(same_khi)) >= 32;
  const bool head2 = head || prev_khi != khi;
  const uint32_t run_id2 = runs_end_together ? wave_inclusive_scan_dpp(head2 ? 1u : 0u) : 0u;
  for (int word = 0; word < pk.nwords; ++word) {
    uint64_t acc = 0;
    if (live) acc = word + 1 < pk.nwords ? stage_packed_word(pl, pk, vm, cf, word) : (uint64_t)(int64_t)dp;
    const uint64_t run = wave_run_sum(run_id, acc, lane);
    uint64_t* w = pk.w + (int64_t)word * pk.stride;
    if (live && head && run) atomicAdd((unsigned long long*)(w + klo), (unsigned long long)run);
    if (runs_end_together) {
      const uint64_t run2 = wave_run_sum(run_id2, acc, lane);
      if (live && head2 && run2) atomicAdd((unsigned long long*)(w + khi + 1), (unsigned long long)(0 - run2));
    } else if (live && acc) atomicAdd((unsigned long long*)(w + khi + 1), (unsigned long long)(0 - acc));
  }
  const uint64_t m = __ballot(live);
  if (lane == 0 && m) atomicAdd(in_window_count + 16 + ((blockIdx.x * 4u + (threadIdx.x >> 6)) & (kCountSpread - 1)), (int32_t)__popcll(m));
  bool left = false, cut = false;
  if (live) { const int64_t c = c_base + i; left = fr.begin[c] < qb; cut = cm.eff_end[c] < fr.end[c]; }
  const uint64_t ml = __ballot(left), mc = __ballot(cut);
  if (lane == 0 && ml) atomicAdd(in_window_count + 4, (int32_t)__popcll(ml));
  if (lane == 0 && mc) atomicAdd(in_window_count + 5, (int32_t)__popcll(mc));
}
__global__ void k_incidence_fill(FragmentView fr, CellMeta cm, const int64_t* hoff, int64_t c_base, int64_t n, int64_t nrows, uint64_t* keys, int64_t* vals) {
  int64_t i = (int64_t)blockIdx.x * blockDim.x + threadIdx.x;
  if (i >= n) return;
  stage_incidence_fill(fr, cm, hoff, c_base + i, c_base, nrows, keys, vals, nullptr);
}
__global__ void k_heavy_base(const uint64_t* sorted_keys, int64_t T, int64_t nrows, int64_t P, int64_t* hbase) {
  int64_t k = (int64_t)blockIdx.x * blockDim.x + threadIdx.x;
  if (k > P) return;
  hbase[k] = stage_heavy_base(sorted_keys, T, nrows, k);
}
__global__ void k_lut_len(const int64_t* inc_cell, const uint32_t* cflags, int64_t T, uint32_t* len) {
  int64_t t = (int64_t)blockIdx.x * blockDim.x + threadIdx.x;
  if (t >= T) return;
  len[t] = GDB_CF_NALT(cflags[inc_cell[t]]) + 1;
}

constexpr int kSortedMedianThreshold = 16;
__global__ void k_median_keys(FragmentView fr, CombinePlan pl, CellMeta cm, RecordTable rec, const uint64_t* inc_keys_sorted, const int64_t* inc_cell, int64_t T,
                              int64_t nrows, int f, int keep_spanning, uint64_t* keys, uint32_t* idx) {
  const int64_t t = (int64_t)blockIdx.x * blockDim.x + threadIdx.x;
  if (t >= T) return;
  const int64_t k = (int64_t)(inc_keys_sorted[t] / (uint64_t)nrows);
  const int64_t c = inc_cell[t];
  bool valid = field_valid(cm, c, f);
  if (valid && !keep_spanning && (cm.cflags[c] & GDB_CF_DELETION) && rec.start[k] > fr.begin[c]) valid = false;
  uint32_t bits = 0;
  if (valid) {
    int n;
    if (pl.field[f].elem == GDB_ET_FLOAT) { const float v = cell_field<float>(fr, pl, f, c, n)[0]; valid = gdb_float_valid(v); bits = gdb_orderable_bits(v); }
    else { const int32_t v = cell_field<int32_t>(fr, pl, f, c, n)[0]; valid = gdb_int_valid(v); bits = gdb_orderable_bits(v); }
  }
  keys[t] = ((uint64_t)k << 33) | (valid ? 0ull : 1ull << 32) | (valid ? bits : 0u);
  idx[t] = (uint32_t)t;
}

__global__ void k_scalar_values(FragmentView fr, CombinePlan pl, CellMeta cm, RecordTable rec, const uint64_t* inc_keys_sorted, const int64_t* inc_cell, int64_t T,
                                int64_t nrows, int f, int keep_spanning, uint32_t* out) {
  const int64_t t = (int64_t)blockIdx.x * blockDim.x + threadIdx.x;
  if (t >= T) return;
  const bool is_float = pl.field[f].elem == GDB_ET_FLOAT;
  const int64_t c = inc_cell[t];
  uint32_t bits = is_float ? GDB_BCF_FLOAT_MISSING_BITS : (uint32_t)GDB_BCF_INT32_MISSING;
  bool valid = field_valid(cm, c, f);
  if (valid && !keep_spanning && (cm.cflags[c] & GDB_CF_DELETION)) {
    const int64_t k = (int64_t)(inc_keys_sorted[t] / (uint64_t)nrows);
    if (rec.start[k] > fr.begin[c]) valid = false;
  }
  if (valid) {
    int n;
    if (is_float) { const float v = cell_field<float>(fr, pl, f, c, n)[0]; if (gdb_float_valid(v)) bits = gdb_f2u(v); }
    else { const int32_t v = cell_field<int32_t>(fr, pl, f, c, n)[0]; if (gdb_int_valid(v)) bits = (uint32_t)v; }
  }
  out[t] = bits;
}

// ... 117 lines not shown
  const uint32_t r = s_w[wv] + incl - v;
  total = s_w[kHugeBlock / 64];
  __syncthreads();
  return r;
}
__device__ uint32_t huge_tie_median(const uint32_t* __restrict__ val, int64_t hb, int64_t he, uint32_t missing, float* a, uint32_t* posL, uint32_t* posR,
                                    uint32_t* s_w, uint32_t* s_m, uint32_t* s_res) {
  const int tid = threadIdx.x;
  uint32_t total;
  {
    const int64_t ninc = he - hb, per = (ninc + kHugeBlock - 1) / kHugeBlock;
    const int64_t b = hb + min(ninc, (int64_t)tid * per), e = hb + min(ninc, (int64_t)(tid + 1) * per);
    uint32_t cnt = 0;
    for (int64_t t = b; t < e; ++t) cnt += val[t] != missing;
    uint32_t at = huge_block_scan(cnt, s_w, total);
    for (int64_t t = b; t < e; ++t) { const uint32_t u = val[t]; if (u != missing) a[at++] = __uint_as_float(u); }
  }
  __syncthreads();
  const int64_t n = total, nth = n / 2;
  int depth = 0;
  for (int64_t m = n; m > 1; m >>= 1) ++depth;
  depth *= 2;
  int64_t first = 0, last = n;
  while (last - first > 3) {
    if (depth == 0) break;
    --depth;
    if (tid == 0) { gdb_median3_to_first(a, first, last); *s_m = 0u; }
    __syncthreads();
    const float pivot = a[first];
    const int64_t len = last - first - 1, per = (len + kHugeBlock - 1) / kHugeBlock;
    const int64_t b = first + 1 + min(len, (int64_t)tid * per), e = first + 1 + min(len, (int64_t)(tid + 1) * per);
    uint32_t cl = 0, cr = 0;
    for (int64_t i = b; i < e; ++i) { const float v = a[i]; cl += !(v < pivot); cr += !(pivot < v); }
    uint32_t nl, nr;
    uint32_t atl = huge_block_scan(cl, s_w, nl);
    const uint32_t fwd = huge_block_scan(cr, s_w, nr);
    uint32_t atr = nr - fwd - cr;
    for (int64_t i = b; i < e; ++i) if (!(a[i] < pivot)) posL[atl++] = (uint32_t)i;
    for (int64_t i = e - 1; i >= b; --i) if (!(pivot < a[i])) posR[atr++] = (uint32_t)i;
    __syncthreads();
    const uint32_t both = min(nl, nr);
    uint32_t mine = 0;
    for (uint32_t k = tid; k < both; k += kHugeBlock) mine += posL[k] < posR[k];
    if (mine) atomicAdd(s_m, mine);
    __syncthreads();
    const uint32_t m = *s_m;
    for (uint32_t k = tid; k < m; k += kHugeBlock) { const uint32_t i = posL[k], j = posR[k]; const float x = a[i]; a[i] = a[j]; a[j] = x; }
    const int64_t cut = (m < nl && (m == 0 || posL[m] < posR[m - 1])) ? (int64_t)posL[m] : (int64_t)posR[m - 1];
    __syncthreads();
    if (cut <= nth) first = cut; else last = cut;
  }
  if (tid == 0) *s_res = __float_as_uint(gdb_introselect_libstdcxx(a + first, last - first, nth - first, last - first > 3 ? 0 : 1));
  __syncthreads();
  const uint32_t r = *s_res;
  __syncthreads();
  return r;
}
__global__ void __launch_bounds__(kHugeBlock) k_site_huge(const SiteCtx* __restrict__ sxp, const int32_t* __restrict__ huge_list, const int32_t* __restrict__ counter,
                                                      HugeSiteOut* __restrict__ out, uint32_t* err, int32_t* fallbacks) {
  const SiteCtx& cx = *sxp;
  const CombinePlan& pl = cx.pl;
  __shared__ uint32_t tab_hash[kHugeTable], tab_order[kHugeTable];
  __shared__ int16_t tab_midx[kHugeTable];
  __shared__ unsigned long long s_key, s_cnt[4], s_filter;
  __shared__ int32_t s_flags[4];
  __shared__ int32_t s_nocc, s_isum;
  __shared__ const char* s_mref;
  __shared__ int32_t s_mref_len;
  __shared__ uint32_t s_hist[256], s_prefix, s_mask, s_first_t;
  __shared__ long long s_rank;
  __shared__ uint32_t s_stage[2048];
  __shared__ uint32_t s_scan_w[kHugeBlock / 64 + 1], s_tie_m, s_tie_res;
  __shared__ unsigned long long s_tie_at;
  const int tid = threadIdx.x;
  const int count = min(*counter, kMaxHugeRecords);
  uint32_t e = 0;
  for (int bi = blockIdx.x; bi < count; bi += gridDim.x) {
    const int64_t k = huge_list[bi];
    const int64_t hb = cx.hl.base[k], he = cx.hl.base[k + 1];
    const int64_t s_k = cx.rec.start[k];
    HugeSiteOut& o = out[bi];
    if (tid == 0) {
      int len0 = 0;
      s_mref = site_first_ref(cx, s_k, len0);
      s_mref_len = len0;
      s_key = ((unsigned long long)(uint32_t)len0 << 32) | 0xFFFFFFFFull;
      s_flags[0] = s_flags[1] = s_flags[2] = s_flags[3] = 0;
      s_nocc = 0;
      s_filter = ~0ull;
    }
    for (int s = tid; s < kHugeTable; s += kHugeBlock) { tab_hash[s] = kHugeEmpty; tab_order[s] = 0xFFFFFFFFu; tab_midx[s] = 0; }
    __syncthreads();
    for (int64_t t = hb + tid; t < he; t += kHugeBlock) {
      const int64_t c = cx.hl.cell[t];
      if (cx.fr.begin[c] != s_k || !field_valid(cx.cm, c, pl.f_REF)) continue;
      int n;
      cell_field<char>(cx.fr, pl, pl.f_REF, c, n);
      atomicMax(&s_key, ((unsigned long long)(uint32_t)n << 32) | (unsigned long long)(0xFFFFFFFEu - (uint32_t)(t - hb)));
    }
    __syncthreads();
    if (tid == 0 && (uint32_t)s_key != 0xFFFFFFFFu) {
      const int64_t t = hb + (int64_t)(0xFFFFFFFEu - (uint32_t)s_key);
      int n;
      s_mref = cell_field<char>(cx.fr, pl, pl.f_REF, cx.hl.cell[t], n);
      s_mref_len = n;
    }
    __syncthreads();
    const char* mref = s_mref;
    const int mref_len = s_mref_len;
    HugeTable tb{tab_hash, tab_order, tab_midx, &s_flags[0]};
    for (int64_t t = hb + tid; t < he; t += kHugeBlock) {
      HugeInsert fa{tb, (uint32_t)(t - hb) << 6, 0u};
      site_merge_call(cx, t, s_k, mref, mref_len, false, fa, &e);
      if (fa.i > 63u) s_flags[1] = 1;
    }
    __syncthreads();
    const bool skip_a = (s_flags[0] | s_flags[1]) != 0;
    for (int s = tid; s < kHugeTable && !skip_a; s += kHugeBlock) {
      if (tab_hash[s] == kHugeEmpty) continue;
      const uint32_t mine = tab_order[s];
      int rank = 0;
      for (int s2 = 0; s2 < kHugeTable; ++s2) rank += (tab_hash[s2] != kHugeEmpty && tab_order[s2] < mine) ? 1 : 0;
      atomicAdd(&s_nocc, 1);
      if (rank + 1 >= GDB_MAX_MERGED_ALLELES - 1) { e |= GDB_ERR_TOO_MANY_MERGED_ALLELES; tab_midx[s] = 1; continue; }
      tab_midx[s] = (int16_t)(rank + 1);
      HugePick pk{mine & 63u, 0u, AlleleRef{nullptr, 0, -1, 0u}, false};
      uint32_t e2 = 0;
      site_merge_call(cx, hb + (int64_t)(mine >> 6), s_k, mref, mref_len, false, pk, &e2);
      if (pk.found) o.merged[rank + 1] = pk.out; else s_flags[1] = 1;
    }
    __syncthreads();
    const int nmerged = min(1 + s_nocc, GDB_MAX_MERGED_ALLELES - 1);
    const int num_merged = nmerged + (cx.pc.nr_cnt[k] > 0 ? 1 : 0);
    const bool skip_b = (s_flags[0] | s_flags[1]) != 0;
    for (int64_t t = hb + tid; t < he && !skip_b; t += kHugeBlock) {
      HugeLookup fc{tb, o.merged, mref, mref_len, &s_flags[1]};
      site_merge_call(cx, t, s_k, mref, mref_len, true, fc, &e);
      const int64_t c = cx.hl.cell[t];
      const uint32_t cf = cx.cm.cflags[c];
      if (cx.pc.nr_cnt[k] > 0 && (cf & GDB_CF_HAS_NR)) {
        int alt_len;
        const char* alt = cell_field<char>(cx.fr, pl, pl.f_ALT, c, alt_len);
        const char* tok; int tl;
        for (int i = 0; alt_token(alt, alt_len, i, tok, tl); ++i)
          if (tl > 0 && tok[0] == '&' && i + 1 <= (int)GDB_CF_NALT(cf)) cx.hl.i2m[cx.hl.i2m_off[t] + i + 1] = (int8_t)(num_merged - 1);
      }
    }
    const bool do_filter = pl.produce_FILTER_field && pl.f_FILTER >= 0;
    if (do_filter || pl.f_ID >= 0)
      for (int64_t t = hb + tid; t < he; t += kHugeBlock) {
        const int64_t c = cx.hl.cell[t];
        if (pl.f_ID >= 0 && field_valid(cx.cm, c, pl.f_ID)) s_flags[3] = 1;
        if (do_filter && field_valid(cx.cm, c, pl.f_FILTER)) {
          int n;
          const int32_t* p = cell_field<int32_t>(cx.fr, pl, pl.f_FILTER, c, n);
          if (n > 0) atomicMin(&s_filter, ((unsigned long long)(uint32_t)(t - hb) << 32) | (unsigned long long)(uint32_t)p[0]);
        }
      }
    __syncthreads();
    if (do_filter && s_filter != ~0ull) {
      const int32_t first_id = (int32_t)(uint32_t)s_filter;
      for (int64_t t = hb + tid; t < he; t += kHugeBlock) {
        const int64_t c = cx.hl.cell[t];
        if (!field_valid(cx.cm, c, pl.f_FILTER)) continue;
        int n;
        const int32_t* p = cell_field<int32_t>(cx.fr, pl, pl.f_FILTER, c, n);
        for (int i = 0; i < n; ++i) if (p[i] != first_id) s_flags[2] = 1;
// ... 44 lines not shown
            if (tid == 0) for (int64_t j = 0; j < m; ++j) { const uint32_t u = s_stage[j]; if (u != missing) fsum += __uint_as_float(u); }
            __syncthreads();
          }
          sum_bits = __float_as_uint(fsum);
        }
        uint32_t median_bits = 0;
        int32_t median_ok = 0;
        if (op == GDB_OP_MEDIAN && total_valid > 0) {
          if (tid == 0) { s_prefix = 0; s_mask = 0; s_rank = total_valid / 2; }
          __syncthreads();
          for (int pass = 0; pass < 4; ++pass) {
            const int shift = 24 - 8 * pass;
            if (tid < 256) s_hist[tid] = 0;
            __syncthreads();
            const uint32_t prefix = s_prefix, mask = s_mask;
            for (int64_t t = hb + tid; t < he; t += kHugeBlock) {
              const uint32_t u = val[t];
              if (u == missing) continue;
              const uint32_t key = is_float ? gdb_orderable_bits(__uint_as_float(u)) : gdb_orderable_bits((int32_t)u);
              if ((key & mask) == prefix) atomicAdd(&s_hist[(key >> shift) & 255u], 1u);
            }
            __syncthreads();
            if (tid == 0) {
              long long r = s_rank;
              uint32_t b = 0;
              for (; b < 255u && r >= (long long)s_hist[b]; ++b) r -= s_hist[b];
              s_rank = r; s_prefix = prefix | (b << shift); s_mask = mask | (255u << shift);
            }
            __syncthreads();
          }
          const uint32_t want = s_prefix;
          for (int64_t t = hb + tid; t < he; t += kHugeBlock) {
            const uint32_t u = val[t];
            if (u == missing) continue;
            const uint32_t key = is_float ? gdb_orderable_bits(__uint_as_float(u)) : gdb_orderable_bits((int32_t)u);
            if (key == want) atomicMin(&s_first_t, (uint32_t)(t - hb));
          }
          __syncthreads();
          if (s_first_t != 0xFFFFFFFFu) {
            median_bits = val[hb + s_first_t];
            const bool zero = is_float && (median_bits << 1) == 0u;
            median_ok = (zero && s_cnt[2] && s_cnt[3]) ? 2 : 1;
          }
          if (median_ok == 2 && cx.tie.buf) {
            if (tid == 0) s_tie_at = atomicAdd(cx.tie.used, 3ull * (unsigned long long)total_valid);
            __syncthreads();
            const unsigned long long at = s_tie_at;
            if (at + 3ull * (unsigned long long)total_valid <= cx.tie.capacity) {
              float* a = cx.tie.buf + at;
              median_bits = huge_tie_median(val, hb, he, missing, a, (uint32_t*)(a + total_valid), (uint32_t*)(a + 2 * total_valid), s_scan_w, &s_tie_m, &s_tie_res);
              median_ok = 1;
            }
            __syncthreads();
          }
        }
        if (tid == 0) {
          HugeScalar& hv = o.scalar[slot];
          hv.nvalid = total_valid; hv.nbelow = (long long)s_cnt[1]; hv.nneg0 = (long long)s_cnt[2]; hv.npos0 = (long long)s_cnt[3];
          hv.sum_bits = sum_bits; hv.median_bits = median_bits; hv.median_ok = median_ok; hv.pad = 0;
        }
        __syncthreads();
      }
    __syncthreads();
  }
  if (e) atomicOr(err, e);
}

constexpr int kSiteStride = 256;
#ifndef GDBAMD_SITE_CAP
#define GDBAMD_SITE_CAP 128
#endif
constexpr int kSiteCap = GDBAMD_SITE_CAP;
constexpr int kSiteStripWords = kSiteCap / 4 + 1;
__global__ void k_site_order_keys(const int64_t* __restrict__ hbase, int64_t P, uint32_t* __restrict__ key, int32_t* __restrict__ val) {
  const int64_t k = (int64_t)blockIdx.x * blockDim.x + threadIdx.x;
  if (k >= P) return;
  const int64_t n = hbase[k + 1] - hbase[k];
  key[k] = (uint32_t)(n > 255 ? 255 : n);
  val[k] = (int32_t)k;
}
#ifndef GDBAMD_SITE_ATTR
#define GDBAMD_SITE_ATTR __attribute__((amdgpu_waves_per_eu(4)))
#endif
__global__ void __launch_bounds__(64) GDBAMD_SITE_ATTR k_site_size(const SiteCtx* __restrict__ sxp, const int32_t* __restrict__ order, char* __restrict__ staging, SpillPool spill, int32_t* __restrict__ spill_chunk, uint32_t* err) {
  const SiteCtx& sx = *sxp;
  __shared__ uint32_t strip[64 * kSiteStripWords];
  int64_t k = (int64_t)blockIdx.x * blockDim.x + threadIdx.x;
  if (k >= sx.rec.npos) return;
  if (order) k = order[k];
  uint32_t e = 0;
  uint32_t* mine = strip + threadIdx.x * kSiteStripWords;
  LdsSpillSink cs((gdb_lds_char*)mine, (uint32_t)kSiteCap, spill, k);
  site_emit(sx, k, cs, true, &e);
  cs.flush();
  sx.so.prefix_len[k] = cs.n;
  spill_chunk[k] = (cs.n > (uint32_t)kSiteCap && cs.complete()) ? 0 : -1;
  const uint32_t nstaged = min(cs.n, (uint32_t)kSiteCap);
  uint4* dst = reinterpret_cast<uint4*>(staging + (size_t)k * kSiteStride);
  for (uint32_t q = 0; (q << 4) < nstaged; ++q) dst[q] = make_uint4(mine[4 * q], mine[4 * q + 1], mine[4 * q + 2], mine[4 * q + 3]);
  if (e) atomicOr(err, e);
}
__global__ void __launch_bounds__(256) k_site_copy(const uint32_t* __restrict__ prefix_len, const char* __restrict__ staging, const char* __restrict__ spill_buf,
                                                   const int32_t* __restrict__ spill_chunk, int64_t k_begin, int64_t k_end,
                                                   const uint64_t* __restrict__ chunk_off, int nchunks, uint64_t page_base, char* __restrict__ arena) {
  const int64_t k = k_begin + (int64_t)blockIdx.x * 4 + (threadIdx.x >> 6);
  const uint32_t lane = threadIdx.x & 63u;
  if (k >= k_end) return;
  const uint32_t n_all = prefix_len[k];
  char* rec = arena + (chunk_off[k * nchunks] - page_base);
  if (lane == 0) arena[chunk_off[(k + 1) * nchunks] - page_base - 1] = '\n';
  uint32_t n = n_all;
  if (n_all > (uint32_t)kSiteCap) {
    const int32_t sc = spill_chunk[k];
    if (sc < 0) return;
    const char* tail = spill_buf + (size_t)k * kSpillTail;
    for (uint32_t i = lane; i < n_all - (uint32_t)kSiteCap; i += 64u) rec[(uint32_t)kSiteCap + i] = tail[i];
    n = (uint32_t)kSiteCap;
  }
  const uint32_t a = (uint32_t)((uintptr_t)rec & 3u);
  const uint32_t cur = reinterpret_cast<const uint32_t*>(staging + (size_t)k * kSiteStride)[lane];
  uint32_t prev = (uint32_t)__shfl_up((int)cur, 1);
  if (lane == 0) prev = 0;
  const uint32_t w = a ? __builtin_amdgcn_alignbyte(cur, prev, 4u - a) : cur;
  const int32_t r0 = (int32_t)(4u * lane) - (int32_t)a;
  if (r0 >= 0 && r0 + 3 < (int32_t)n) {
    *reinterpret_cast<uint32_t*>(rec + r0) = w;
  } else {
#pragma unroll
    for (int b = 0; b < 4; ++b) if (r0 + b >= 0 && r0 + b < (int32_t)n) rec[r0 + b] = (char)((w >> (8 * b)) & 0xFFu);
  }
  if (lane == 63 && a && 256 - (int32_t)a < (int32_t)n)
    for (int32_t r = 256 - (int32_t)a; r < (int32_t)n; ++r) rec[r] = (char)((cur >> (8 * (r & 3))) & 0xFFu);
}
__global__ void k_site_write(const SiteCtx* __restrict__ sxp, const char* __restrict__ staging, const char* __restrict__ spill_buf, const int32_t* __restrict__ spill_chunk, int64_t k_begin, int64_t k_end, const uint64_t* chunk_off, int nchunks,
                             uint64_t page_base, char* arena, uint32_t* err) {
  const SiteCtx& sx = *sxp;
  int64_t k = k_begin + (int64_t)blockIdx.x * blockDim.x + threadIdx.x;
  if (k >= k_end) return;
  uint32_t e = 0;
  char* dst = arena + (chunk_off[k * nchunks] - page_base);
  const uint32_t n = sx.so.prefix_len[k];
  if (n <= (uint32_t)kSiteCap) {
    return;
  } else if (spill_chunk[k] >= 0) {
    return;
  } else {
    ByteSink bs(dst);
    site_emit(sx, k, bs, false, &e);
  }
  arena[chunk_off[(k + 1) * nchunks] - page_base - 1] = '\n';
  if (e) atomicOr(err, e);
}

constexpr int kCtxSlots = GDB_MAX_PIPELINES_PER_PROCESS;
__constant__ EntryCtx c_ex[kCtxSlots];
static std::mutex g_ctx_slot_mutex;
static bool g_ctx_slot_used[kCtxSlots];

__device__ __noinline__ void entry_store(int cs, RecordInfo ri, int64_t c, char* dst, uint32_t* e) {
  (void)entry_emit(c_ex[cs], ri, c, ByteSink(dst), e);
}
__device__ __noinline__ uint32_t entry_store_lds_capped(int cs, RecordInfo ri, int64_t c, gdb_lds_char* dst, uint32_t cap, uint32_t* e) {
  return entry_emit(c_ex[cs], ri, c, LdsCapSink(dst, cap), e).n;
}

__device__ __noinline__ void entry_bin_store(int cs, RecordInfo ri, int64_t c, char* dst, uint32_t* e) {
  (void)entry_emit_bin(c_ex[cs], ri, c, ByteSink(dst), e);
}
__device__ __noinline__ uint32_t entry_bin_lds_capped(int cs, RecordInfo ri, int64_t c, gdb_lds_char* dst, uint32_t cap, uint32_t* e) {
  return entry_emit_bin(c_ex[cs], ri, c, LdsCapSink(dst, cap), e).n;
}

constexpr int kTypeHash = 4096;
constexpr int kMaxTypes = 64;
constexpr uint32_t kUntabledType = 255u;
constexpr uint64_t kEmptyKey = ~0ull;

__device__ __forceinline__ uint64_t record_type_key(uint32_t fmt_mask, uint32_t num_merged, uint32_t rflags) {
  return (uint64_t)fmt_mask | ((uint64_t)num_merged << 32) | ((uint64_t)rflags << 40);
}
__device__ __forceinline__ uint32_t type_hash(uint64_t k) {
  k ^= k >> 33; k *= 0xff51afd7ed558ccdull; k ^= k >> 29;
  return (uint32_t)k & (kTypeHash - 1);
}
__device__ __forceinline__ void type_insert_global(uint64_t key, int32_t k, unsigned long long* hkeys, int32_t* hrep) {
  uint32_t h = type_hash(key);
  for (int probe = 0; probe < kTypeHash; ++probe, h = (h + 1) & (kTypeHash - 1)) {
    unsigned long long cur = __atomic_load_n(&hkeys[h], __ATOMIC_RELAXED);
    if (cur == kEmptyKey) cur = atomicCAS(&hkeys[h], (unsigned long long)kEmptyKey, (unsigned long long)key);
    if (cur == kEmptyKey || cur == key) {
      if (__atomic_load_n(&hrep[h], __ATOMIC_RELAXED) > k) atomicMin(&hrep[h], k);
      return;
    }
  }
}
__global__ void __launch_bounds__(kBlock) k_type_insert(SiteOut so, int64_t P, unsigned long long* hkeys, int32_t* hrep) {
  constexpr int kLocal = 128;
  __shared__ unsigned long long lkey[kLocal];
  __shared__ int32_t lrep[kLocal];
  if (threadIdx.x < kLocal) { lkey[threadIdx.x] = kEmptyKey; lrep[threadIdx.x] = INT32_MAX; }
  __syncthreads();
  const int64_t k = (int64_t)blockIdx.x * blockDim.x + threadIdx.x;
  if (k < P) {
    const uint64_t key = record_type_key(so.fmt_mask[k], so.num_alleles[k], so.rflags[k]);
    uint32_t h = type_hash(key) & (kLocal - 1);
    bool placed = false;
    for (int probe = 0; probe < kLocal && !placed; ++probe, h = (h + 1) & (kLocal - 1)) {
      unsigned long long cur = lkey[h];
      if (cur == kEmptyKey) cur = atomicCAS(&lkey[h], (unsigned long long)kEmptyKey, (unsigned long long)key);
      if (cur == kEmptyKey || cur == key) { atomicMin(&lrep[h], (int32_t)k); placed = true; }
    }
    if (!placed) type_insert_global(key, (int32_t)k, hkeys, hrep);
  }
  __syncthreads();
  if (threadIdx.x < kLocal && lkey[threadIdx.x] != kEmptyKey) type_insert_global(lkey[threadIdx.x], lrep[threadIdx.x], hkeys, hrep);
}
__global__ void k_type_assign(const unsigned long long* hkeys, const int32_t* hrep, int max_types, uint8_t* hid, int32_t* type_rep, int32_t* ntypes) {
  if (blockIdx.x) return;
  constexpr int per = kTypeHash / 64;
  const int lane = threadIdx.x;
  uint32_t cnt = 0;
  for (int j = 0; j < per; ++j) cnt += hkeys[lane * per + j] != kEmptyKey;
  const uint32_t incl = wave_inclusive_scan_dpp(cnt);
  int n = (int)(incl - cnt);
  for (int j = 0; j < per; ++j) {
    const int h = lane * per + j;
    if (hkeys[h] == kEmptyKey) continue;
    if (n < max_types) { hid[h] = (uint8_t)n; type_rep[n] = hrep[h]; } else hid[h] = (uint8_t)kUntabledType;
    ++n;
  }
  if (lane == 63) *ntypes = min((int)incl, max_types);
// ... 1564 lines not shown
      uint32_t* const out = part + ((int64_t)ch * P + k) * W;
      const uint32_t key = d.y ? d.x : 0xFFFFFFFEu;
      const bool same = words == prev_words && !__any((int)(key != prev_key));
      prev_key = key; prev_words = words;
      if (!same) {
        mine = 0;
        const char* src = ((d.x & kOverflowBit) ? pool_ovf : pool) + (size_t)(d.x & ~kOverflowBit) * 16;
        for (int w0 = 0; w0 < words; w0 += 4) {
          u32x4 v = {0u, 0u, 0u, 0u};
          if (d.y) v = w0 == 0 ? h : *reinterpret_cast<const u32x4*>(src + 4 * w0);
#pragma unroll
          for (int c = 0; c < 4; ++c) {
            if (w0 + c >= words) break;
            const uint32_t r = bcf_pair_reduce(v[c]);
            if (lane == w0 + c) mine = r;
          }
        }
      }
      if (lane < words) out[lane] = mine;
    }
  }
}
struct BcfLayout {
  uint32_t* fmeta;
  uint32_t* foff;
  uint32_t* l_indiv;
  uint64_t* rec_size;
};
__global__ void k_bcf_layout(CombinePlan pl, const uint32_t* __restrict__ part, const uint32_t* __restrict__ fmt_mask, const uint32_t* __restrict__ prefix_len, int64_t P, int nchunks,
                             int F, BcfLayout lay) {
  const int64_t k = (int64_t)blockIdx.x * blockDim.x + threadIdx.x;
  if (k >= P) return;
  const uint32_t mask = fmt_mask[k];
  const int W = (F + 1) >> 1;
  uint32_t at = 8u + prefix_len[k];
  const uint32_t indiv_begin = at;
  int q = 0;
  for (int i = 0; i < pl.n_format; ++i) {
    if (!((mask >> i) & 1u)) continue;
    uint32_t sum = 0;
    for (int ch = 0; ch < nchunks; ++ch) sum = bcf_summary_max(sum, (part[((int64_t)ch * P + k) * W + (q >> 1)] >> (16 * (q & 1))) & 0xFFFFu);
    const int t = bcf_field_type(pl, i, sum);
    const uint32_t cnt = bcf_summary_n(sum) ? bcf_summary_n(sum) : 1u;
    const int f = pl.format_field[i];
    const int32_t key = (f == pl.f_DP && pl.f_DP_FORMAT >= 0) ? pl.bcf_dp_id : pl.bcf_id[f];
    const uint32_t hdr = (uint32_t)bcf_enc_int1_bytes(key) + (uint32_t)bcf_enc_size_bytes((int)cnt);
    lay.fmeta[k * F + q] = cnt | ((uint32_t)t << 16) | (hdr << 24);
    lay.foff[k * F + q] = at;
    at += hdr + (uint32_t)pl.bcf_n_sample * cnt * (uint32_t)bcf_type_width(t);
    ++q;
  }
  lay.l_indiv[k] = at - indiv_begin;
  lay.rec_size[k] = at;
}
__global__ void k_bcf_max_record(const uint64_t* rec_size, int64_t P, unsigned long long* max_record) {
  const int64_t k = (int64_t)blockIdx.x * blockDim.x + threadIdx.x;
  unsigned long long mine = k < P ? rec_size[k] : 0ull;
  for (int d = 32; d > 0; d >>= 1) { const unsigned long long o = __shfl_xor(mine, d); mine = o > mine ? o : mine; }
  if ((threadIdx.x & 63) == 0 && mine) atomicMax(max_record, mine);
}
__global__ void k_bcf_shared(const SiteCtx* __restrict__ sxp, const char* __restrict__ staging, const char* __restrict__ spill_buf, const int32_t* __restrict__ spill_chunk,
                             int64_t k_begin, int64_t k_end, const uint64_t* __restrict__ rec_off, uint64_t page_base, BcfLayout lay, int F, char* __restrict__ arena, uint32_t* err) {
  const SiteCtx& sx = *sxp;
  const int64_t k = k_begin + (int64_t)blockIdx.x * blockDim.x + threadIdx.x;
  if (k >= k_end) return;
  const CombinePlan& pl = sx.pl;
  char* rec = arena + (rec_off[k] - page_base);
  const uint32_t n = sx.so.prefix_len[k];
  ByteSink head(rec);
  bcf_put_u32(head, n);
  bcf_put_u32(head, lay.l_indiv[k]);
  char* dst = rec + 8;
  uint32_t e = 0;
  if (n <= (uint32_t)kSiteCap) {
    const char* src = staging + (size_t)k * kSiteStride;
    for (uint32_t i = 0; i < n; ++i) dst[i] = src[i];
  } else if (spill_chunk[k] >= 0) {
    const char* src = staging + (size_t)k * kSiteStride;
    for (uint32_t i = 0; i < (uint32_t)kSiteCap; ++i) dst[i] = src[i];
    const char* tail = spill_buf + (size_t)k * kSpillTail;
    for (uint32_t i = kSiteCap; i < n; ++i) dst[i] = tail[i - kSiteCap];
  } else {
    ByteSink bs(dst);
    site_emit(sx, k, bs, false, &e);
  }
  const uint32_t mask = sx.so.fmt_mask[k];
  int q = 0;
  for (int i = 0; i < pl.n_format; ++i) {
    if (!((mask >> i) & 1u)) continue;
    const uint32_t m = lay.fmeta[k * F + q];
    ByteSink fs(rec + lay.foff[k * F + q]);
    const int f = pl.format_field[i];
    bcf_enc_int1(fs, (f == pl.f_DP && pl.f_DP_FORMAT >= 0) ? pl.bcf_dp_id : pl.bcf_id[f]);
    bcf_enc_size(fs, (int)(m & 0xFFFFu), (int)((m >> 16) & 0xFu));
    ++q;
  }
  if (e) atomicOr(err, e);
}
struct __attribute__((packed)) PackedU16 { uint16_t v; };
#ifndef GDB_BCF_ENTRY_CAP
#define GDB_BCF_ENTRY_CAP 96
#endif
constexpr int kBcfEntryCap = GDB_BCF_ENTRY_CAP;
constexpr int kBcfImageSample = 32;
template <class Out, class In> __device__ __forceinline__ void bcf_sample_values(Out* out, const In* in, uint32_t n, uint32_t cnt, uint32_t t, uint32_t first, uint32_t rest) {
  if (t == GDB_BT_CHAR) {
    for (uint32_t j = 0; j < cnt; ++j) out[j] = j < n ? in[j] : (char)(j == 0 ? first : rest);
  } else if (t == GDB_BT_INT8) {
    for (uint32_t j = 0; j < cnt; ++j) {
      const int32_t v = (int32_t)(j < n ? reinterpret_cast<const uint32_t*>(in)[j] : (j == 0 ? first : rest));
      out[j] = v == GDB_BCF_INT32_MISSING ? (char)0x80 : v == GDB_BCF_INT32_VECTOR_END ? (char)0x81 : (char)v;
    }
  } else if (t == GDB_BT_INT16) {
    for (uint32_t j = 0; j < cnt; ++j) {
      const int32_t v = (int32_t)(j < n ? reinterpret_cast<const uint32_t*>(in)[j] : (j == 0 ? first : rest));
      reinterpret_cast<PackedU16*>(out + 2u * j)->v = v == GDB_BCF_INT32_MISSING ? (uint16_t)0x8000u : v == GDB_BCF_INT32_VECTOR_END ? (uint16_t)0x8001u : (uint16_t)v;
    }
  } else {
    for (uint32_t j = 0; j < cnt; ++j) reinterpret_cast<PackedU32*>(out + 4u * j)->v = j < n ? reinterpret_cast<const uint32_t*>(in)[j] : (j == 0 ? first : rest);
  }
}
__global__ void k_bcf_same_layout(const int32_t* __restrict__ order, const uint32_t* __restrict__ fmt_mask, const uint32_t* __restrict__ fmeta, int64_t np, int F, uint8_t* __restrict__ same) {
  const int64_t idx = (int64_t)blockIdx.x * blockDim.x + threadIdx.x;
  if (idx >= np) return;
  bool eq = idx > 0;
  if (eq) {
    const int64_t k = order[idx], kp = order[idx - 1];
    const uint32_t m = fmt_mask[k];
    eq = m == fmt_mask[kp];
    const int nf = __popc(m);
    for (int q = 0; eq && q < nf; ++q) eq = fmeta[k * F + q] == fmeta[kp * F + q];
  }
  same[idx] = eq ? 1 : 0;
}
#ifdef GDB_BCF_PROF
#define BCF_PROF_PARAM , unsigned long long* prof
#define BCF_PROF_ARG , bcf_prof_buffer()
#define BCF_STAMP(n) { const uint64_t now_ = __builtin_amdgcn_s_memtime(); prof_acc[n] += now_ - prof_t; prof_t = now_; }
#define BCF_COUNT(n) { ++prof_acc[n]; }
static unsigned long long* bcf_prof_buffer() { static unsigned long long* p = nullptr; if (!p) { (void)hipMalloc((void**)&p, 128); (void)hipMemset(p, 0, 128); } return p; }
#else
#define BCF_PROF_PARAM
#define BCF_PROF_ARG
#define BCF_STAMP(n)
#define BCF_COUNT(n)
#endif
struct __attribute__((packed)) PackedU128 { u32x4 v; };
constexpr int kBcfImageBytes = 3072;
constexpr int kBcfImageSets = kBcfImageBytes / (16 * kAsmRows);
constexpr int kBcfBatch = 4;
__global__ void __launch_bounds__(kAsmRows) __attribute__((amdgpu_waves_per_eu(4))) k_bcf_write(CombinePlan pl, const ResMatrix resolved, const char* __restrict__ pool, const char* __restrict__ pool_ovf,
                                                      const uint32_t* __restrict__ fmt_mask, const int32_t* __restrict__ order, const uint8_t* __restrict__ same_layout, int64_t np, int nchunks,
                                                      int F, int32_t N, BcfLayout lay, const uint64_t* __restrict__ rec_off, uint64_t page_base, char* __restrict__ arena BCF_PROF_PARAM) {
  __shared__ __attribute__((aligned(16))) char s_entry[kAsmRows * kBcfEntryCap];
#ifdef GDB_BCF_PROF
  uint64_t prof_acc[12] = {0, 0, 0, 0, 0, 0, 0, 0, 0, 0, 0, 0}; uint64_t prof_t = __builtin_amdgcn_s_memtime();
#endif
  __shared__ __attribute__((aligned(16))) char s_image[kBcfImageBytes + 16];
  __shared__ uint2 s_rows[kBcfBatch][kAsmRows];
  __shared__ uint8_t s_changed[kAsmRows];
  const int64_t unit = xcd_aware_unit<1>(((np + kBcfRun - 1) / kBcfRun) * (int64_t)nchunks);
  if (unit < 0) return;
  const int64_t i0 = (unit / nchunks) * kBcfRun, i1 = min(np, i0 + (int64_t)kBcfRun);
  const int ch = (int)(unit % nchunks);
  const int lane = threadIdx.x;
  const uint32_t nsamp = (uint32_t)min((int32_t)kAsmRows, N - ch * kAsmRows);
  const bool flag = pl.use_missing_values_not_vector_end != 0;
// ... 610 lines not shown
  if (k > K) return;
  len[k] = k < K ? off[list[k] + 1] - off[list[k]] : 0u;
}
__global__ void k_gather_var(const uint64_t* list, int64_t K, const uint32_t* off, const char* src, uint32_t elem_size, const uint32_t* new_off, char* dst) {
  const int64_t k = (int64_t)blockIdx.x * blockDim.x + threadIdx.x;
  if (k >= K) return;
  const uint32_t a = off[list[k]], n = (off[list[k] + 1] - a) * elem_size;
  const char* s = src + (size_t)a * elem_size;
  char* d = dst + (size_t)new_off[k] * elem_size;
  for (uint32_t b = 0; b < n; ++b) d[b] = s[b];
}

__global__ void k_fragment_part_check(const int32_t* __restrict__ row, const int64_t* __restrict__ begin, const int64_t* __restrict__ end, int64_t n, int32_t nrows, uint32_t* err) {
  const int64_t d = (int64_t)blockIdx.x * blockDim.x + threadIdx.x;
  if (d >= n) return;
  bool bad = row[d] < 0 || row[d] >= nrows || end[d] < begin[d];
  if (d > 0 && (begin[d] < begin[d - 1] || (begin[d] == begin[d - 1] && row[d] <= row[d - 1]))) bad = true;
  if (bad) atomicOr(err, (uint32_t)GDB_ERR_CELL_STREAM);
}
__global__ void k_fragment_offsets_check(const uint32_t* __restrict__ off, int64_t n, uint32_t total, uint32_t* err) {
  const int64_t i = (int64_t)blockIdx.x * blockDim.x + threadIdx.x;
  if (i > n) return;
  const bool bad = (i == 0 && off[0] != 0u) || (i == n && off[n] != total) || (i < n && off[i + 1] < off[i]);
  if (bad) atomicOr(err, (uint32_t)GDB_ERR_CELL_STREAM);
}
__global__ void k_copy_offsets(const uint32_t* src, int64_t n, uint32_t base, uint32_t* dst) {
  int64_t i = (int64_t)blockIdx.x * blockDim.x + threadIdx.x;
  if (i < n) dst[i] = src[i] + base;
}
__global__ void k_gather_record_offsets(const uint64_t* chunk_off, int nchunks, int64_t P, uint64_t* rec_off, unsigned long long* max_record) {
  int64_t k = (int64_t)blockIdx.x * blockDim.x + threadIdx.x;
  unsigned long long mine = 0;
  if (k <= P) {
    const uint64_t at = chunk_off[k * nchunks];
    rec_off[k] = at;
    if (k < P) mine = chunk_off[(k + 1) * nchunks] - at;
  }
  for (int d = 32; d > 0; d >>= 1) { const unsigned long long o = __shfl_xor(mine, d); mine = o > mine ? o : mine; }
  __shared__ unsigned long long wave_max[kBlock / 64];
  if ((threadIdx.x & 63) == 0) wave_max[threadIdx.x >> 6] = mine;
  __syncthreads();
  if (threadIdx.x == 0) {
    for (int w = 1; w < kBlock / 64; ++w) mine = wave_max[w] > mine ? wave_max[w] : mine;
    if (mine) atomicMax(max_record, mine);
  }
}

}

struct DevicePipeline::Impl {
  HostPlan hp;
  int device = 0;
  hipStream_t stream = nullptr;
  hipStream_t stream_page = nullptr;
  bool page_priority = false;
  hipEvent_t ev_page_fork = nullptr, ev_page_join = nullptr;
  hipStream_t stream_compute = nullptr, stream_stage = nullptr;
  void use_stage_stream() {
    static const bool on = getenv("GDBAMD_STAGE_PRIORITY") && atoi(getenv("GDBAMD_STAGE_PRIORITY")) != 0;
    if (!on) return;
    if (!stream_stage) {
      int least = 0, greatest = 0;
      HIP_CHECK(hipDeviceGetStreamPriorityRange(&least, &greatest));
      HIP_CHECK(hipStreamCreateWithPriority(&stream_stage, hipStreamDefault, greatest));
    }
    HIP_CHECK(hipStreamSynchronize(stream_compute));
    stream = stream_stage;
  }
  void use_compute_stream() { stream = stream_compute; }
  FragmentView fr;
  bool owns_fragment = false;
  std::vector<void*> owned;
  DevBuf<char> names_text, contig_names, ref_bases;
  DevBuf<int32_t> field_name_off, field_name_len, filter_name_off, filter_name_len, filter_bcf_id;
  DevBuf<uint32_t> bcf_part, bcf_fmeta, bcf_foff, bcf_lindiv; DevBuf<uint64_t> bcf_rec_size; DevBuf<uint8_t> bcf_same;
  DevBuf<GdbContig> contigs;
  int64_t ref_begin = 0, ref_len = 0;
  DevBuf<uint64_t> vmask; DevBuf<uint32_t> cflags; DevBuf<int32_t> dpval, k_lo, k_hi; DevBuf<int64_t> eff_end;
  DevBuf<int32_t> row_keys, row_keys_sorted; DevBuf<int64_t> cell_ids, perm, rm_begin, row_ptr, span, span_max, cwin;
  int64_t max_span = 0;
  DevBuf<uint64_t> ev_keys, ev_keys_sorted; DevBuf<int64_t> ev_delta, ev_incl; DevBuf<int32_t> run_end, run_excl;
  DevBuf<int64_t> bpos, bnrec, rbase; DevBuf<int32_t> bcov, bdel;
  DevBuf<int64_t> rstart, rend;
  DevBuf<int32_t> diff, first_record_at; DevBuf<uint64_t> diff_packed; DevBuf<int64_t> heavy_count, hoff;
  DevBuf<uint64_t> inc_keys, inc_keys_sorted; DevBuf<int64_t> inc_vals, inc_vals_sorted, hbase;
  DevBuf<uint32_t> lut_len, i2m_off; DevBuf<int8_t> i2m, gt_override; DevBuf<uint8_t> iflags;
  DevBuf<uint8_t> num_alleles, rflags; DevBuf<uint32_t> fmt_mask, prefix_len; DevBuf<char> site_staging, spill_buf; DevBuf<int32_t> spill_chunk;
  DevBuf<uint64_t> chunk_size, chunk_off, rec_off; DevBuf<unsigned long long> max_record;
  std::unique_ptr<BgzfDeviceCompressor> bgzf;
  void queue_compression(int ai, char* arena, uint64_t page_bytes) {
    if (!hp.bgzf || page_bytes == 0) return;
    if (!bgzf) { bgzf.reset(new BgzfDeviceCompressor); bgzf->set_text(!hp.plan.bcf_mode); bgzf->set_bcf2(hp.plan.bcf_mode != 0); }
    bgzf->enqueue(ai, arena, page_bytes, arena, (void*)stream);
  }
  DevBuf<unsigned int> slot_bump;
  bool long_texts_seen = false;
  uint64_t pool_ovf_need = 0;
  DevBuf<char> arena[2], temp;
  DevBuf<uint32_t> err; DevBuf<int32_t> counters;
  DevBuf<uint32_t> site_key, site_key_sorted; DevBuf<int32_t> site_ord_in, site_ord;
  int ctx_slot = -1;
  DevBuf<char> calls_names, calls_text; DevBuf<int32_t> calls_name_off; DevBuf<uint64_t> calls_len, calls_off; bool calls_names_ready = false; DevBuf<int64_t> calls_array_row; size_t calls_array_row_n = 0;
  DevBuf<int64_t> var_cell, var_end, var_iota, var_sorted, var_run, var_order; DevBuf<uint64_t> var_key, var_key_sorted, var_leader; uint64_t variants_bytes = 0;
  hipEvent_t ev_prep[4] = {nullptr, nullptr, nullptr, nullptr};
  hipEvent_t ev_page[2][4] = {{nullptr, nullptr, nullptr, nullptr}, {nullptr, nullptr, nullptr, nullptr}};
  hipEvent_t arena_release[2] = {nullptr, nullptr};
  struct HostBlock { uint64_t q[80]; uint32_t page_err[2]; } *hb = nullptr;
  DevBuf<SiteCtx> d_sx;
  DevBuf<uint64_t> med_keys, med_keys_sorted; DevBuf<uint32_t> med_idx, med_idx_sorted;
  DevBuf<int32_t> big_index, big_list; DevBuf<uint32_t> big_value; DevBuf<uint8_t> big_ok;
  DevBuf<unsigned long long> remap_total;
  DevBuf<int32_t> huge_index, huge_list; DevBuf<HugeSiteOut> huge_out; DevBuf<SiteCtx> d_sx0;
  DevBuf<uint32_t> slot_cell; DevBuf<float> tie_buf; DevBuf<unsigned long long> tie_used; DevBuf<uint32_t> scalar_pre;
  DevBuf<unsigned long long> type_hkeys; DevBuf<int32_t> type_hrep, type_rep; DevBuf<uint8_t> type_hid, rtype;
  DevBuf<WalkCell> walk; DevBuf<int64_t> walk_inv;
  DevBuf<int32_t> jhint;
  DevBuf<unsigned long long> dbg_counters;
  DevBuf<uint32_t> pl_cnt, pl_ofs; DevBuf<PieceEntry> plist;
  uint32_t walk_epoch = 0;
  DevBuf<uint8_t> raw_cells; DevBuf<uint64_t> raw_off; DevBuf<int32_t> raw_row_map, raw_qrow; DevBuf<uint32_t> raw_keep, raw_dest, raw_len, raw_voff, raw_mark, raw_mdest;
  DevBuf<int64_t> raw_begin, raw_end;
  DevBuf<uint64_t> walk_bitmap, walk_pos, walk_out; DevBuf<uint32_t> walk_wcount, walk_wrank, walk_succ, walk_jump_a, walk_jump_b, walk_flag, walk_dest; DevBuf<uint8_t> walk_reach;
  DevBuf<int64_t> walk_cut; DevBuf<unsigned long long> walk_kept_bytes;
  DevBuf<uint8_t> inflate_in, inflate_out, inflate_scratch, inflate_status; DevBuf<uint64_t> inflate_off; DevBuf<uint32_t> inflate_want;
  DevBuf<long long> carry_last; DevBuf<uint64_t> carry_keys, carry_sorted; int64_t carried_cells = 0;
  DevBuf<uint2> chk_resolved; DevBuf<uint64_t> chk_sizes; DevBuf<unsigned long long> chk_count;
  DevBuf<uint2> resolved;
  DevBuf<uint32_t> res_off; DevBuf<uint8_t> res_len8;
  DevBuf<unsigned int> slot_over;
  DevBuf<uint32_t> type_occ;
  DevBuf<uint32_t> untabled, ubase; DevBuf<int32_t> urec, iota, order; DevBuf<uint32_t> order_keys, order_keys_sorted;
  DevBuf<uint64_t> tmask; DevBuf<uint32_t> nslots, tbase, slot_len, slot_units, slot_off; DevBuf<uint2> slot_desc; DevBuf<char> pool, pool_ovf;
  bool classified = false;
  uint64_t fragment_generation = 0;
  struct Part { FragmentView v; std::vector<size_t> data_bytes; std::vector<void*> bufs; };
  std::vector<Part> parts;
  std::vector<int> col_elem_size; std::vector<bool> col_var; std::vector<int> col_fixed_num;
  std::unique_ptr<DevicePipeline::FragmentFile> ff;
  struct IntervalState {
    bool active = false;
    int64_t P = 0, kp = 0;
    int nchunks = 0;
    uint64_t max_record_bytes = 0, total_bytes = 0;
    float write_kernel_ms = 0;
    std::vector<uint64_t> rec_off;
    IntervalStats stats;
    SiteCtx sx; EntryCtx ex; RowIndex ri; SiteOut so; RecordTable rec; AsmCtx ac; PieceCtx pc2;
    AssemblyKnobs knobs{};
    AssemblySizing sz{};
    int NT = 0, bcf_F = 0; BcfLayout lay{nullptr, nullptr, nullptr, nullptr};
    EventBuf eb{nullptr, nullptr, nullptr, 0};
    DevicePipeline::PageView last_page;
  } iv;
  ResMatrix res_view() const { return iv.sz.res_compact ? ResMatrix{nullptr, res_off.p, res_len8.p} : ResMatrix{resolved.p, nullptr, nullptr}; }

  void* temp_storage(size_t bytes) { temp.ensure(bytes + 256); return temp.p; }
  template <class K, class V> void sort_pairs(const K* kin, K* kout, const V* vin, V* vout, size_t n, int end_bit) {
    size_t bytes = 0;
    HIP_CHECK(rocprim::radix_sort_pairs(nullptr, bytes, kin, kout, vin, vout, n, 0, end_bit, stream));
    void* t = temp_storage(bytes);
    HIP_CHECK(rocprim::radix_sort_pairs(t, bytes, kin, kout, vin, vout, n, 0, end_bit, stream));
  }
  template <class K> void sort_keys(const K* kin, K* kout, size_t n, int end_bit) {
    size_t bytes = 0;
    HIP_CHECK(rocprim::radix_sort_keys(nullptr, bytes, kin, kout, n, 0, end_bit, stream));
    void* t = temp_storage(bytes);
    HIP_CHECK(rocprim::radix_sort_keys(t, bytes, kin, kout, n, 0, end_bit, stream));
// ... 1372 lines not shown
  classify_fragment();
  CellMeta cm{S.vmask.p, S.cflags.p, S.dpval.p, S.eff_end.p, S.k_lo.p, S.k_hi.p};
  S.cwin.ensure(4);
  STAGE("k_cell_window");
  hipLaunchKernelGGL(k_cell_window, dim3(1), dim3(64), 0, st, fr.begin, C, qb > INT64_MIN + S.max_span ? qb - S.max_span : INT64_MIN, qe, S.cwin.p);
  if (fr.nmarkers > 0) hipLaunchKernelGGL(k_cell_window, dim3(1), dim3(64), 0, st, fr.marker_begin, fr.nmarkers, qb, qe, S.cwin.p + 2);
  int64_t cw[4] = {0, 0, 0, 0};
  S.read_back_many({{cw, S.cwin.p, (fr.nmarkers > 0 ? 4 : 2) * sizeof(int64_t)}});
  const int64_t c_base = cw[0], c_end = cw[1];
  const int64_t CW = c_end - c_base;
  if (CW <= 0) return;
  const int64_t m_base = cw[2], MW = std::max<int64_t>(0, cw[3] - cw[2]);
  const int64_t NE = 2 * CW + 2 * MW;
  S.ev_keys.ensure(NE); S.ev_keys_sorted.ensure(NE); S.ev_delta.ensure(NE); S.ev_incl.ensure(NE); S.run_end.ensure(NE); S.run_excl.ensure(NE + 1);
  STAGE("k_event_keys");
  hipLaunchKernelGGL(k_event_keys, dim3(blocks_for(CW)), dim3(kBlock), 0, st, fr, cm, c_base, CW, qb, qe, S.ev_keys.p);
  if (MW > 0) hipLaunchKernelGGL(k_marker_keys, dim3(blocks_for(MW)), dim3(kBlock), 0, st, fr, m_base, MW, qb, qe, S.ev_keys.p + 2 * CW);
  {
    const uint64_t span = (uint64_t)(qe - qb) + 2u;
    const int eb = span >= (1ull << 60) ? 64 : bits_for(span << 2);
    S.sort_keys(S.ev_keys.p, S.ev_keys_sorted.p, (size_t)NE, eb);
  }
  STAGE("k_event_delta");
  hipLaunchKernelGGL(k_event_delta, dim3(blocks_for(NE)), dim3(kBlock), 0, st, S.ev_keys_sorted.p, NE, S.ev_delta.p, S.run_end.p);
  S.incl_scan(S.ev_delta.p, S.ev_incl.p, (size_t)NE, PackedAdd());
  S.excl_scan(S.run_end.p, S.run_excl.p, (size_t)NE);
  const int64_t U = S.read_back_sum(S.run_excl.p + (NE - 1), S.run_end.p + (NE - 1));
  int64_t P = 0;
  if (U > 0) {
    S.bpos.ensure(U + 1); S.bcov.ensure(U + 1); S.bdel.ensure(U + 1); S.bnrec.ensure(U + 1); S.rbase.ensure(U + 1);
    Boundaries bd{S.bpos.p, S.bcov.p, S.bdel.p, S.bnrec.p};
    STAGE("k_boundary_write");
    hipLaunchKernelGGL(k_boundary_write, dim3(blocks_for(NE)), dim3(kBlock), 0, st, S.ev_keys_sorted.p, S.ev_incl.p, S.run_end.p, S.run_excl.p, NE, bd, qb);
    STAGE("k_boundary_nrec");
    hipLaunchKernelGGL(k_boundary_nrec, dim3(blocks_for(U)), dim3(kBlock), 0, st, bd, U);
    S.excl_scan(S.bnrec.p, S.rbase.p, (size_t)U);
    P = S.read_back_sum(S.rbase.p + (U - 1), S.bnrec.p + (U - 1));
    if (P > 0) {
      S.rstart.ensure(P); S.rend.ensure(P);
      STAGE("k_record_expand");
      hipLaunchKernelGGL(k_record_expand, dim3(blocks_for(P)), dim3(kBlock), 0, st, bd, S.rbase.p, U, P, S.rstart.p, S.rend.p);
    }
  }
  stats.num_records = P;
  if (P == 0) {
    stats.err_bits = S.read_back(S.err.p);
    if (stats.err_bits) throw GenomicsDBDeviceException(err_bits_text(stats.err_bits));
    return;
  }
  if (P >= (1ll << 31)) throw GenomicsDBDeviceException("more than 2^31 records in one interval: split the query interval");
  RecordTable rec{P, S.rstart.p, S.rend.p};
  const int nf = pl.n_format;
  const int64_t stride = P + 1;
  const size_t ndiff = (size_t)(nf + 2) * (size_t)stride;
  S.diff.ensure(ndiff);
  DiffPacked pk;
  pk.width = 1; while (pk.width < 32 && (1ll << pk.width) <= (int64_t)N) ++pk.width;
  pk.per_word = 64 / pk.width;
  pk.nwords = (nf + 1 + pk.per_word - 1) / pk.per_word + 1;
  pk.stride = stride;
  S.diff_packed.ensure((size_t)pk.nwords * stride);
  pk.w = S.diff_packed.p;
  HIP_CHECK(hipMemsetAsync(pk.w, 0, (size_t)pk.nwords * stride * sizeof(uint64_t), st));
  int32_t* d_fmt = S.diff.p;
  int32_t* d_dp = S.diff.p + (size_t)nf * stride;
  int32_t* d_nr = d_dp + stride;
  DiffArrays da{d_fmt, d_dp, d_nr, stride};
  S.heavy_count.ensure(CW + 1); S.hoff.ensure(CW + 2);
  const int32_t* first_record_at = nullptr;
  if ((uint64_t)(qe - qb) + 2u <= (1ull << 27)) {
    const int64_t W = qe - qb + 2;
    S.first_record_at.ensure(W);
    hipLaunchKernelGGL(k_fill_i32, dim3(blocks_for(W)), dim3(kBlock), 0, st, S.first_record_at.p, W, (int32_t)P);
    hipLaunchKernelGGL(k_mark_record_starts, dim3(blocks_for(P)), dim3(kBlock), 0, st, S.rstart.p, P, qb, S.first_record_at.p);
    {
      auto rin = rocprim::make_reverse_iterator(S.first_record_at.p + W);
      size_t bytes = 0;
      HIP_CHECK(rocprim::inclusive_scan(nullptr, bytes, rin, rin, (size_t)W, rocprim::minimum<int32_t>(), st));
      void* t = S.temp_storage(bytes);
      HIP_CHECK(rocprim::inclusive_scan(t, bytes, rin, rin, (size_t)W, rocprim::minimum<int32_t>(), st));
    }
    first_record_at = S.first_record_at.p;
  }
  STAGE("k_cell_ranges");
  hipLaunchKernelGGL(k_cell_ranges, dim3(blocks_for(CW)), dim3(kBlock), 0, st, fr, pl, cm, rec, c_base, CW, qb, qe, S.heavy_count.p, S.counters.p, first_record_at, pk);
  S.incl_scan(pk.w, pk.w, (size_t)pk.nwords * stride, rocprim::plus<uint64_t>());
  hipLaunchKernelGGL(k_unpack_counts, dim3(blocks_for(stride)), dim3(kBlock), 0, st, pk, nf, stride, da);
  S.excl_scan(S.heavy_count.p, S.hoff.p, (size_t)CW);
  int64_t T_a = 0, T_b = 0;
  int32_t n_in_window = 0, spread[kCountSpread], sweep_counts[2] = {0, 0};
  S.read_back_many({{&T_a, S.hoff.p + (CW - 1), sizeof(int64_t)}, {&T_b, S.heavy_count.p + (CW - 1), sizeof(int64_t)}, {spread, S.counters.p + 16, sizeof(spread)},
                    {sweep_counts, S.counters.p + 4, sizeof(sweep_counts)}});
  for (int i = 0; i < kCountSpread; ++i) n_in_window += spread[i];
  stats.gt_profile[GT_NUM_CELLS] = (uint64_t)CW;
  stats.gt_profile[GT_NUM_CELLS_IN_LEFT_SWEEP] = (uint64_t)sweep_counts[0];
  stats.gt_profile[GT_NUM_VALID_CELLS_IN_QUERY] = (uint64_t)n_in_window;
  stats.gt_profile[GT_NUM_ATTR_CELLS_ACCESSED] = (uint64_t)n_in_window * (uint64_t)pl.nfields;
  stats.gt_profile[GT_NUM_PQ_FLUSHES_DUE_TO_OVERLAPPING_CELLS] = (uint64_t)sweep_counts[1];
  stats.gt_profile[GT_NUM_OPERATOR_INVOCATIONS] = (uint64_t)P;
  const int64_t T = T_a + T_b;
  stats.num_heavy_incidences = T;
  stats.num_cells_in_window = n_in_window;
  S.inc_keys.ensure(T + 1); S.inc_keys_sorted.ensure(T + 1); S.inc_vals.ensure(T + 1); S.inc_vals_sorted.ensure(T + 1);
  S.hbase.ensure(P + 2); S.lut_len.ensure(T + 2); S.i2m_off.ensure(T + 2); S.iflags.ensure(T + 1); S.gt_override.ensure((size_t)GDB_MAX_PLOIDY * T + 2);
  uint32_t lut_total = 0;
  if (T > 0) {
    STAGE("k_incidence_fill");
    hipLaunchKernelGGL(k_incidence_fill, dim3(blocks_for(CW)), dim3(kBlock), 0, st, fr, cm, S.hoff.p, c_base, CW, (int64_t)N, S.inc_keys.p, S.inc_vals.p);
    S.sort_pairs(S.inc_keys.p, S.inc_keys_sorted.p, S.inc_vals.p, S.inc_vals_sorted.p, (size_t)T, bits_for((uint64_t)P * (uint64_t)N));
    STAGE("k_lut_len");
    hipLaunchKernelGGL(k_lut_len, dim3(blocks_for(T)), dim3(kBlock), 0, st, S.inc_vals_sorted.p, S.cflags.p, T, S.lut_len.p);
    HIP_CHECK(hipMemsetAsync(S.lut_len.p + T, 0, sizeof(uint32_t), st));
    S.excl_scan(S.lut_len.p, S.i2m_off.p, (size_t)T + 1);
    if ((uint64_t)T * GDB_MAX_INPUT_ALLELES >= (1ull << 32)) throw GenomicsDBDeviceException("allele LUT storage exceeds 2^32 entries: split the query interval");
    lut_total = (uint32_t)((uint64_t)T * GDB_MAX_INPUT_ALLELES);
  } else {
    HIP_CHECK(hipMemsetAsync(S.i2m_off.p, 0, 2 * sizeof(uint32_t), st));
  }
  STAGE("k_heavy_base");
  hipLaunchKernelGGL(k_heavy_base, dim3(blocks_for(P + 1)), dim3(kBlock), 0, st, S.inc_keys_sorted.p, T, (int64_t)N, P, S.hbase.p);
  S.i2m.ensure((size_t)lut_total + 16);
  HeavyLists hl{S.hbase.p, S.inc_vals_sorted.p, S.i2m_off.p, S.i2m.p, S.iflags.p, S.gt_override.p};
  HIP_CHECK(hipEventRecord(ev[1], st));
  S.num_alleles.ensure(P); S.rflags.ensure(P); S.fmt_mask.ensure(P); S.prefix_len.ensure(P);
  SiteOut so{S.num_alleles.p, S.rflags.p, S.fmt_mask.p, S.prefix_len.p};
  QueryWindow qw;
  memset(&qw, 0, sizeof(qw));
  qw.qb = qb; qw.qe = qe;
  qw.contigs = S.contigs.p; qw.ncontigs = (int32_t)S.hp.contigs.size(); qw.contig_names = S.contig_names.p;
  qw.ref_bases = S.ref_len ? S.ref_bases.p : nullptr; qw.ref_begin = S.ref_begin; qw.ref_len = S.ref_len;
  NameTables nt{S.names_text.p, S.field_name_off.p, S.field_name_len.p, S.filter_name_off.p, S.filter_name_len.p, (int32_t)S.hp.filter_name_off.size(), S.filter_bcf_id.p};
  PresenceCounts pc{d_fmt, d_dp, d_nr, stride};
  MedianOrder med;
  memset(&med, 0, sizeof(med));
  for (int f = 0; f < GDB_MAX_FIELDS; ++f) med.slot[f] = -1;
  if (T > (int64_t)kSortedMedianThreshold * P || getenv("GDBAMD_SORTED_MEDIAN")) {
    std::vector<std::pair<int, int>> fields;
    for (int i = 0; i < pl.n_info; ++i) if (pl.field[pl.info_field[i]].combine_op == GDB_OP_MEDIAN && pl.field[pl.info_field[i]].length != GDB_VL_A) fields.push_back(std::make_pair(pl.info_field[i], 0));
    if (pl.qual_combine_op == GDB_OP_MEDIAN && pl.f_QUAL >= 0) fields.push_back(std::make_pair(pl.f_QUAL, 1));
    if (!fields.empty() && T > 0 && P < (1ll << 31)) {
      S.med_keys.ensure((size_t)T); S.med_idx.ensure((size_t)T);
      S.med_keys_sorted.ensure(fields.size() * (size_t)T); S.med_idx_sorted.ensure(fields.size() * (size_t)T);
      for (size_t s = 0; s < fields.size(); ++s) {
        hipLaunchKernelGGL(k_median_keys, dim3(blocks_for(T)), dim3(kBlock), 0, st, fr, pl, cm, rec, (const uint64_t*)S.inc_keys_sorted.p, (const int64_t*)S.inc_vals_sorted.p, T,
                           (int64_t)N, fields[s].first, fields[s].second, S.med_keys.p, S.med_idx.p);
        S.sort_pairs(S.med_keys.p, S.med_keys_sorted.p + s * (size_t)T, S.med_idx.p, S.med_idx_sorted.p + s * (size_t)T, (size_t)T, std::min(64, 33 + bits_for((uint64_t)P)));
        med.slot[fields[s].first] = (int8_t)s;
      }
      med.keys = S.med_keys_sorted.p; med.inc = S.med_idx_sorted.p; med.stride = T; med.enabled = 1;
    }
  }
  BigMedians big;
  memset(&big, 0, sizeof(big));
  for (int f = 0; f < GDB_MAX_FIELDS; ++f) big.slot[f] = -1;
  if (!med.enabled && T > 0) {
    std::vector<std::pair<int, int>> fields;
    for (int i = 0; i < pl.n_info; ++i) if (pl.field[pl.info_field[i]].combine_op == GDB_OP_MEDIAN && pl.field[pl.info_field[i]].length != GDB_VL_A) fields.push_back(std::make_pair(pl.info_field[i], 0));
    if (pl.qual_combine_op == GDB_OP_MEDIAN && pl.f_QUAL >= 0) fields.push_back(std::make_pair(pl.f_QUAL, 1));
    if (!fields.empty()) {
      S.big_index.ensure((size_t)P); S.big_list.ensure(kMaxBigRecords); S.big_value.ensure(fields.size() * (size_t)kMaxBigRecords); S.big_ok.ensure(fields.size() * (size_t)kMaxBigRecords);
      hipLaunchKernelGGL(k_big_records, dim3(blocks_for(P)), dim3(kBlock), 0, st, (const int64_t*)S.hbase.p, P, S.big_index.p, S.big_list.p, S.counters.p + 2);
      for (size_t s = 0; s < fields.size(); ++s) {
        hipLaunchKernelGGL(k_big_medians, dim3(64), dim3(kBlock), 0, st, fr, pl, cm, rec, hl, (const int32_t*)S.big_list.p, (const int32_t*)(S.counters.p + 2), fields[s].first, (int)s,
                           fields[s].second, (int64_t)kMaxBigRecords, S.big_value.p, S.big_ok.p);
        big.slot[fields[s].first] = (int8_t)s;
      }
      big.index = S.big_index.p; big.value = S.big_value.p; big.ok = S.big_ok.p; big.stride = kMaxBigRecords; big.enabled = 1;
    }
  }
  TieScratch tie{nullptr, nullptr, 0};
  {
    int nf = (pl.qual_combine_op == GDB_OP_MEDIAN && pl.f_QUAL >= 0) ? 1 : 0;
    for (int i = 0; i < pl.n_info; ++i) if (pl.field[pl.info_field[i]].combine_op == GDB_OP_MEDIAN && pl.field[pl.info_field[i]].elem == GDB_ET_FLOAT) ++nf;
    if (nf && T > 0) {
      tie.capacity = 5ull * (uint64_t)nf * (uint64_t)T;
      S.tie_buf.ensure((size_t)tie.capacity + 4); S.tie_used.ensure(1);
      HIP_CHECK(hipMemsetAsync(S.tie_used.p, 0, sizeof(unsigned long long), st));
      tie.buf = S.tie_buf.p; tie.used = S.tie_used.p;
    }
  }
  ScalarPre pre;
  memset(&pre, 0, sizeof(pre));
  for (int f = 0; f < GDB_MAX_FIELDS; ++f) pre.slot[f] = -1;
  if (T > 0) {
    std::vector<std::pair<int, int>> fields;
    for (int i = 0; i < pl.n_info; ++i) {
      const GdbFieldDesc& fd = pl.field[pl.info_field[i]];
      if ((fd.combine_op == GDB_OP_MEDIAN || fd.combine_op == GDB_OP_SUM || fd.combine_op == GDB_OP_MEAN) && (fd.elem == GDB_ET_FLOAT || fd.elem == GDB_ET_INT) && fd.length != GDB_VL_A)
        fields.push_back(std::make_pair(pl.info_field[i], 0));
    }
    if (pl.qual_combine_op != GDB_OP_UNKNOWN && pl.f_QUAL >= 0) fields.push_back(std::make_pair(pl.f_QUAL, 1));
    if (!fields.empty()) {
      S.scalar_pre.ensure(fields.size() * (size_t)T);
      for (size_t s = 0; s < fields.size(); ++s) {
        hipLaunchKernelGGL(k_scalar_values, dim3(blocks_for(T)), dim3(kBlock), 0, st, fr, pl, cm, rec, (const uint64_t*)S.inc_keys_sorted.p, (const int64_t*)S.inc_vals_sorted.p, T,
                           (int64_t)N, fields[s].first, fields[s].second, S.scalar_pre.p + s * (size_t)T);
        pre.slot[fields[s].first] = (int8_t)s;
      }
      pre.val = S.scalar_pre.p; pre.stride = T; pre.enabled = 1;
    }
  }
  HugeSites huge;
  memset(&huge, 0, sizeof(huge));
  SiteCtx sx0{fr, pl, cm, rec, hl, pc, nt, qw, so, med, big, tie, pre, huge};
  const int32_t huge_threshold = (P > 0 && T / P >= 24 && P <= (int64_t)kMaxHugeRecords) ? 24 : kHugeRecord;
  if (T > (int64_t)huge_threshold && !getenv("GDBAMD_NO_HUGE_SITES")) {
    S.huge_index.ensure((size_t)P); S.huge_list.ensure(kMaxHugeRecords); S.huge_out.ensure(kMaxHugeRecords); S.d_sx0.ensure(1);
    HIP_CHECK(hipMemcpyAsync(S.d_sx0.p, &sx0, sizeof(SiteCtx), hipMemcpyHostToDevice, st));
    STAGE("k_site_huge");
    hipLaunchKernelGGL(k_huge_records, dim3(blocks_for(P)), dim3(kBlock), 0, st, (const int64_t*)S.hbase.p, P, huge_threshold, S.huge_index.p, S.huge_list.p, S.counters.p + 3);
    hipLaunchKernelGGL(k_site_huge, dim3(1024), dim3(kHugeBlock), 0, st, (const SiteCtx*)S.d_sx0.p, (const int32_t*)S.huge_list.p, (const int32_t*)(S.counters.p + 3), S.huge_out.p, S.err.p, S.counters.p + 6);
    huge.index = S.huge_index.p; huge.out = S.huge_out.p; huge.enabled = 1;
  }
  SiteCtx sx{fr, pl, cm, rec, hl, pc, nt, qw, so, med, big, tie, pre, huge};
  S.d_sx.ensure(1);
  HIP_CHECK(hipMemcpyAsync(S.d_sx.p, &sx, sizeof(SiteCtx), hipMemcpyHostToDevice, st));
  STAGE("k_site_size");
  S.site_staging.ensure((size_t)P * kSiteStride + 64);
  S.spill_buf.ensure((size_t)P * kSpillTail); S.spill_chunk.ensure((size_t)P);
  const int32_t* site_order = nullptr;
  {
    static const bool sorted_sites = !(getenv("GDBAMD_SITE_ORDER") && atoi(getenv("GDBAMD_SITE_ORDER")) == 0);
    if (sorted_sites && P >= 4096) {
      S.site_key.ensure((size_t)P); S.site_key_sorted.ensure((size_t)P); S.site_ord_in.ensure((size_t)P); S.site_ord.ensure((size_t)P);
      hipLaunchKernelGGL(k_site_order_keys, dim3(blocks_for(P)), dim3(kBlock), 0, st, (const int64_t*)S.hbase.p, P, S.site_key.p, S.site_ord_in.p);
      S.sort_pairs(S.site_key.p, S.site_key_sorted.p, S.site_ord_in.p, S.site_ord.p, (size_t)P, 8);
      site_order = S.site_ord.p;
    }
  }
  hipLaunchKernelGGL(k_site_size, dim3(blocks_for(P, 64)), dim3(64), 0, st, S.d_sx.p, site_order, S.site_staging.p, SpillPool{S.spill_buf.p}, S.spill_chunk.p, S.err.p);
  S.remap_total.ensure(1);
  HIP_CHECK(hipMemsetAsync(S.remap_total.p, 0, sizeof(unsigned long long), st));
  for (int i = 0; i < pl.n_format; ++i)
    if (pl.format_field[i] == pl.f_PL && pl.f_PL >= 0)
      hipLaunchKernelGGL(k_remap_elements, dim3(blocks_for(P)), dim3(kBlock), 0, st, so, (const int32_t*)(d_fmt + (size_t)i * stride), P, i, S.remap_total.p);
  HIP_CHECK(hipEventRecord(ev[2], st));
  const int nchunks = (N + kAsmRows - 1) / kAsmRows;
  const size_t nchunk_total = (size_t)P * nchunks;
  S.chunk_size.ensure(nchunk_total + 1); S.chunk_off.ensure(nchunk_total + 2); S.rec_off.ensure(P + 2);
  RowIndex ri{S.row_ptr.p, S.perm.p, S.rm_begin.p};
  EntryCtx ex{fr, pl, cm, hl};
  HIP_CHECK(hipMemcpyToSymbolAsync(HIP_SYMBOL(c_ex), &ex, sizeof(EntryCtx), (size_t)S.ctx_slot * sizeof(EntryCtx), hipMemcpyHostToDevice, st));
  if (T >= (1ll << 32)) throw GenomicsDBDeviceException("more than 2^32 (record, variant call) incidences in one interval: split the query interval");
  S.type_hkeys.ensure(kTypeHash); S.type_hrep.ensure(kTypeHash); S.type_hid.ensure(kTypeHash); S.type_rep.ensure(kMaxTypes); S.rtype.ensure(P);
  HIP_CHECK(hipMemsetAsync(S.type_hkeys.p, 0xFF, kTypeHash * sizeof(unsigned long long), st));
  HIP_CHECK(hipMemsetAsync(S.type_hrep.p, 0x7F, kTypeHash * sizeof(int32_t), st));
  HIP_CHECK(hipMemsetAsync(S.type_hid.p, 0xFF, kTypeHash, st));
  HIP_CHECK(hipMemsetAsync(S.type_rep.p, 0, kMaxTypes * sizeof(int32_t), st));
  STAGE("k_type_insert");
  hipLaunchKernelGGL(k_type_insert, dim3(blocks_for(P)), dim3(kBlock), 0, st, so, P, S.type_hkeys.p, S.type_hrep.p);
  hipLaunchKernelGGL(k_type_assign, dim3(1), dim3(64), 0, st, S.type_hkeys.p, S.type_hrep.p, max_tabled_types(), S.type_hid.p, S.type_rep.p, S.counters.p + 1);
  S.untabled.ensure(P + 1); S.ubase.ensure(P + 1); S.urec.ensure(P + 1);
  hipLaunchKernelGGL(k_type_lookup, dim3(blocks_for(P)), dim3(kBlock), 0, st, so, P, S.type_hkeys.p, S.type_hid.p, S.rtype.p, S.untabled.p);
  S.excl_scan(S.untabled.p, S.ubase.p, (size_t)P);
  S.tmask.ensure(CW); S.nslots.ensure(CW + 1); S.tbase.ensure(CW + 1);
  STAGE("k_cell_types");
  {
    const size_t nocc = (size_t)kMaxTypes * (size_t)(P + 1);
    S.type_occ.ensure(nocc);
    HIP_CHECK(hipMemsetAsync(S.type_occ.p, 0, nocc * sizeof(uint32_t), st));
    hipLaunchKernelGGL(k_type_onehot, dim3(blocks_for(P)), dim3(kBlock), 0, st, (const uint8_t*)S.rtype.p, P, S.type_occ.p);
    S.excl_scan(S.type_occ.p, S.type_occ.p, nocc);
  }
  hipLaunchKernelGGL(k_cell_types, dim3(blocks_for(CW)), dim3(kBlock), 0, st, S.cflags.p, S.k_lo.p, S.k_hi.p, (const uint32_t*)S.type_occ.p, P,
                     (const int32_t*)(S.counters.p + 1), c_base, CW, S.tmask.p, S.nslots.p);
  S.excl_scan(S.nslots.p, S.tbase.p, (size_t)CW);
  uint32_t ur_a = 0, ur_b = 0, sl_a = 0, sl_b = 0;
  int32_t ntypes = 0;
  int32_t huge_counts[4] = {0, 0, 0, 0};
  S.read_back_many({{&ur_a, S.ubase.p + (P - 1), 4}, {&ur_b, S.untabled.p + (P - 1), 4}, {&sl_a, S.tbase.p + (CW - 1), 4}, {&sl_b, S.nslots.p + (CW - 1), 4},
                    {&ntypes, S.counters.p + 1, 4}, {huge_counts, S.counters.p + 3, sizeof(huge_counts)}});
  stats.huge_records = std::min(huge_counts[0], (int32_t)kMaxHugeRecords);
  stats.huge_fallbacks = huge_counts[3];
  const int64_t UR = (int64_t)ur_a + ur_b;
  const uint64_t SL = (uint64_t)sl_a + sl_b;
  if (UR > 0) hipLaunchKernelGGL(k_untabled_records, dim3(blocks_for(P)), dim3(kBlock), 0, st, S.untabled.p, S.ubase.p, P, S.urec.p);
  const uint64_t NS = (uint64_t)kMaxTypes + SL + (uint64_t)T + (uint64_t)UR * (uint64_t)N;
  if (NS >= (1ull << 32)) throw GenomicsDBDeviceException("entry text table exceeds 2^32 slots: split the query interval");
  S.slot_len.ensure(NS + 1); S.slot_units.ensure(NS + 1); S.slot_off.ensure(NS + 1); S.slot_desc.ensure(NS + 1);
  if (NS * (uint64_t)(kSlotStride / 16) >= (uint64_t)kOverflowBit) throw GenomicsDBDeviceException("entry text table exceeds 32 GiB: split the query interval");
  S.pool.ensure((size_t)NS * kSlotStride + 64);
  S.slot_bump.ensure(kBumpShards * 4);
  HIP_CHECK(hipMemsetAsync(S.slot_bump.p, 0, kBumpShards * 4 * sizeof(unsigned int), st));
  S.slot_over.ensure(kBumpShards);
  HIP_CHECK(hipMemsetAsync(S.slot_over.p, 0, kBumpShards * sizeof(unsigned int), st));
  bool wide = S.long_texts_seen;
  if (const char* e = getenv("GDBAMD_SLOT_STRIP")) wide = atoi(e) >= 256;
  auto shard_units_of = [&](size_t cap_bytes) { return (uint32_t)std::min<uint64_t>((uint64_t)(cap_bytes > 64 ? (cap_bytes - 64) / 16 : 0) / kBumpShards, ((uint64_t)kOverflowBit - 1) / kBumpShards); };
  if (wide) S.pool_ovf.ensure(std::max<size_t>((size_t)kBumpShards * ((size_t)S.pool_ovf_need * 16 + ((size_t)S.pool_ovf_need * 16 >> 3)), (size_t)1 << 20) + 64);
  SlotTable stt{S.slot_len.p, S.slot_off.p, S.pool.p, S.pool_ovf.p, (uint32_t)kMaxTypes, (uint32_t)(kMaxTypes + SL), (uint32_t)(kMaxTypes + SL + (uint64_t)T), S.slot_off.p, S.slot_bump.p,
                wide ? shard_units_of(S.pool_ovf.cap) : 0u, (int32_t)S.ctx_slot, pl.bcf_mode, pl.bcf_mode ? (uint32_t)kSlotStride : (uint32_t)kInlineText,
                (const int64_t*)S.hoff.p, (const int32_t*)S.k_lo.p, c_base, S.slot_over.p};
  STAGE("k_slots<0>");
#define GDB_SLOT_KERNELS(PASSN, W) do { \
  hipLaunchKernelGGL((k_slots_nocall<PASSN, W>), dim3(1), dim3(kMaxTypes), 0, st, stt, so, S.type_rep.p, ntypes, S.err.p); \
  if (SL > 0) hipLaunchKernelGGL((k_slots_light<PASSN, W>), dim3(blocks_for((int64_t)SL, light_block<W>())), dim3(light_block<W>()), 0, st, stt, so, S.type_rep.p, S.tmask.p, S.tbase.p, (const uint32_t*)S.slot_cell.p, c_base, (int64_t)SL, slot_regroup() ? 1 : 0, S.err.p); \
  if (T > 0) hipLaunchKernelGGL((k_slots_heavy<PASSN, W>), dim3(blocks_for(T, 64)), dim3(64), 0, st, stt, so, S.inc_keys_sorted.p, S.inc_vals_sorted.p, T, (int64_t)N, S.err.p); \
  if (UR > 0) hipLaunchKernelGGL((k_slots_untabled<PASSN, W>), dim3(blocks_for(UR * N, 64)), dim3(64), 0, st, stt, so, ri, rec, S.urec.p, UR, N, S.err.p); \
} while (0)
  if (SL > 0) {
    S.slot_cell.ensure(SL + 1);
    hipLaunchKernelGGL(k_slot_cells, dim3(blocks_for(CW)), dim3(kBlock), 0, st, (const uint32_t*)S.tbase.p, (const uint32_t*)S.nslots.p, CW, S.slot_cell.p);
  }
  if (wide) GDB_SLOT_KERNELS(0, kStripWordsWide); else GDB_SLOT_KERNELS(0, kStripWords);
  unsigned int bump_sh[kBumpShards * 4], over_sh[kBumpShards];
  S.read_back_many({{bump_sh, S.slot_bump.p, sizeof(bump_sh)}, {over_sh, S.slot_over.p, sizeof(over_sh)}});
  bool any_over255 = false;
  for (int sh = 0; sh < kBumpShards; ++sh) any_over255 |= over_sh[sh] != 0;
  uint64_t left_texts = 0, long_texts = 0, shard_need = 0, total_units = 0;
  for (int sh = 0; sh < kBumpShards; ++sh) {
    left_texts += bump_sh[sh * 4 + 1]; long_texts += bump_sh[sh * 4 + 3];
    shard_need = std::max<uint64_t>(shard_need, (uint64_t)bump_sh[sh * 4] + bump_sh[sh * 4 + 2]);
    total_units += (uint64_t)bump_sh[sh * 4] + bump_sh[sh * 4 + 2];
// ... 330 lines not shown
```

Before: 40.49 million.

## Pack numeric text formatting, precompute first cell per site, specialize site kernels by mode

Number formatting for integers and floats now builds digits in packed 64-bit words and writes them in one go, replacing per-character digit arrays. A new pass inside the cell-range kernel records the first cell at each record position, so site emission no longer binary-searches all cells for the reference allele. Site emission is templated on BCF versus text mode, with a separate size kernel per mode, so the mode branch is resolved at compile time. ALT tokenization moves to a stateful iterator that no longer rescans from the start for each token. The cost is an extra buffer plus memset, larger code, and an added numtext test build.

```diff
diff --git a/__graft_entry__.py b/__graft_entry__.py
--- a/__graft_entry__.py
+++ b/__graft_entry__.py
@@ -25,6 +25,7 @@
     b.build_hostsim_vcfdiff()
     b.build_hostsim_import_stream()
     b.build_hostsim_columns()
+    b.build_hostsim_numtext()
     b.build_jni_importer_harness()
     from genomicsdb_amd import synth
     synth.lib()
diff --git a/genomicsdb_amd/build.py b/genomicsdb_amd/build.py
--- a/genomicsdb_amd/build.py
+++ b/genomicsdb_amd/build.py
@@ -189,6 +189,12 @@
     return os.path.join(d, "libhostsim_columns.so"), os.path.join(d, "hostsim_columns_main")
 
 
+def build_hostsim_numtext():
+    d = os.path.join(ROOT, "tests", "hostsim_numtext")
+    subprocess.check_call(["make", "-s", "-C", d])
+    return os.path.join(d, "libhostsim_numtext.so"), os.path.join(d, "hostsim_numtext_main")
+
+
 def build_hostsim_inflate():
     subprocess.check_call(["make", "-s", "-C", os.path.join(ROOT, "tests", "hostsim_inflate")])
     return os.path.join(ROOT, "tests", "hostsim_inflate", "libhostsim_inflate.so")
diff --git a/genomicsdb_amd/csrc/core/gdb_core.hpp b/genomicsdb_amd/csrc/core/gdb_core.hpp
--- a/genomicsdb_amd/csrc/core/gdb_core.hpp
+++ b/genomicsdb_amd/csrc/core/gdb_core.hpp
@@ -164,15 +164,6 @@
   return false;
 }
 
-template <class Sink> GDB_HD void put_u64(Sink& s, uint64_t v) {
-  char buf[20];
-  int n = 0;
-  do { buf[n++] = (char)('0' + (v % 10)); v /= 10; } while (v);
-  while (n) s.put(buf[--n]);
-}
-template <class Sink> GDB_HD void put_i64(Sink& s, int64_t v) {
-  if (v < 0) { s.put('-'); put_u64(s, (uint64_t)(-(v + 1)) + 1u); } else put_u64(s, (uint64_t)v);
-}
 GDB_HD uint64_t gdb_pack_digits(uint32_t v, int& n) {
   uint64_t w = 0;
   n = 0;
@@ -206,6 +197,32 @@
 template <class Sink> GDB_HD void put_i32(Sink& s, int32_t v) {
   if (v < 0) { s.put('-'); put_u32(s, 0u - (uint32_t)v); } else put_u32(s, (uint32_t)v);
 }
+template <class Sink> GDB_HD void put_u32_pad8(Sink& s, uint32_t v) {
+  int n = 0;
+  uint64_t w = gdb_pack_digits(v, n);
+  for (; n < 8; ++n) w = (w << 8) | (uint64_t)'0';
+  put_packed(s, w, 8);
+}
+template <class Sink> GDB_HD void put_u64(Sink& s, uint64_t v) {
+  if (v <= 0xFFFFFFFFull) { put_u32(s, (uint32_t)v); return; }
+  const uint64_t hi = v / 100000000ull;
+  const uint32_t lo = (uint32_t)(v - hi * 100000000ull);
+  if (hi <= 0xFFFFFFFFull) put_u32(s, (uint32_t)hi);
+  else {
+    const uint64_t top = hi / 100000000ull;
+    put_u32(s, (uint32_t)top);
+    put_u32_pad8(s, (uint32_t)(hi - top * 100000000ull));
+  }
+  put_u32_pad8(s, lo);
+}
+template <class Sink> GDB_HD void put_i64(Sink& s, int64_t v) {
+  if (v < 0) { s.put('-'); put_u64(s, (uint64_t)(-(v + 1)) + 1u); } else put_u64(s, (uint64_t)v);
+}
+GDB_HD uint64_t gdb_packed_insert_dot(uint64_t w, int ip) {
+  const uint64_t head = w & ((1ull << (8 * ip)) - 1ull);
+  return head | ((uint64_t)'.' << (8 * ip)) | ((w >> (8 * ip)) << (8 * (ip + 1)));
+}
+GDB_HD uint64_t gdb_packed_zero_dot() { return 0x303030302E30ull; }
 
 struct GdbBig { uint32_t w[7]; };
 GDB_HD void gdb_big_mul10(GdbBig& b) {
@@ -272,25 +289,20 @@
   const uint32_t ex = u >> 23, man = u & 0x7FFFFFu;
   uint32_t q; int X;
   gdb_round_6_digits(ex ? man | 0x800000u : man, ex ? (int)ex - 150 : -149, q, X);
-  char dg[6];
-  for (int i = 5; i >= 0; --i) { dg[i] = (char)('0' + q % 10u); q /= 10u; }
   int last = 5;
-  while (last > 0 && dg[last] == '0') --last;
+  { uint32_t t = q; while (last > 0) { const uint32_t t10 = t / 10u; if (t - t10 * 10u) break; t = t10; --last; } }
+  int nd = 0;
+  const uint64_t w = gdb_pack_digits(q, nd);
   if (X < -4 || X >= 6) {
-    s.put(dg[0]);
-    if (last > 0) { s.put('.'); for (int i = 1; i <= last; ++i) s.put(dg[i]); }
-    s.put('e');
-    uint32_t ax = (uint32_t)(X < 0 ? -X : X);
-    s.put(X < 0 ? '-' : '+');
-    if (ax < 10u) s.put('0');
-    put_u64(s, ax);
+    if (last > 0) put_packed(s, gdb_packed_insert_dot(w, 1), 2 + last); else s.put((char)(w & 0xFFu));
+    const uint32_t ax = (uint32_t)(X < 0 ? -X : X);
+    const uint32_t a10 = ax / 10u;
+    put_packed(s, (uint64_t)'e' | ((uint64_t)(X < 0 ? '-' : '+') << 8) | ((uint64_t)('0' + a10) << 16) | ((uint64_t)('0' + (ax - a10 * 10u)) << 24), 4);
   } else if (X >= 0) {
-    for (int i = 0; i <= X; ++i) s.put(dg[i]);
-    if (last > X) { s.put('.'); for (int i = X + 1; i <= last; ++i) s.put(dg[i]); }
+    if (last > X) put_packed(s, gdb_packed_insert_dot(w, X + 1), last + 2); else put_packed(s, w, X + 1);
   } else {
-    s.put('0'); s.put('.');
-    for (int i = 0; i < -X - 1; ++i) s.put('0');
-    for (int i = 0; i <= last; ++i) s.put(dg[i]);
+    put_packed(s, gdb_packed_zero_dot(), 2 + (-X - 1));
+    put_packed(s, w, last + 1);
   }
 }
 
@@ -309,23 +321,34 @@
   if (d < 0.001) i += 5; else if (d < 0.01) i += 50; else if (d < 0.1) i += 500; else if (d < 1) i += 5000;
   else if (d < 10) i += 50000; else if (d < 100) i += 500000; else if (d < 1000) i += 5000000;
   else if (d < 10000) i += 50000000; else if (d < 100000) i += 500000000; else i += 5000000000ULL;
-  char dg[24];
-  int p = 0;
-  { char tmp[24]; int n = 0; do { tmp[n++] = (char)('0' + i % 10); i /= 10; } while (i); while (n) dg[p++] = tmp[--n]; }
-  char out[40];
-  int m = 0, dot = -1;
+  const uint64_t hi64 = i / 100000000ull;
+  const uint32_t hi = (uint32_t)hi64, lo = (uint32_t)(i - hi64 * 100000000ull);
+  uint32_t T;
+  int p;
+  if (hi) {
+    int ph = 1;
+    for (uint32_t t = hi; t >= 10u; t /= 10u) ++ph;
+    p = 8 + ph;
+    if (ph >= 6) { T = hi; for (int z = ph; z > 6; --z) T /= 10u; }
+    else { uint32_t l = lo, m = hi; for (int z = 0; z < 2 + ph; ++z) l /= 10u; for (int z = ph; z < 6; ++z) m *= 10u; T = m + l; }
+  } else {
+    p = 1;
+    for (uint32_t t = lo; t >= 10u; t /= 10u) ++p;
+    T = lo;
+    for (int z = p; z > 6; --z) T /= 10u;
+  }
+  int L = 6;
+  { uint32_t t = T; while (L > 1) { const uint32_t t10 = t / 10u; if (t - t10 * 10u) break; t = t10; --L; } }
+  int nd = 0;
+  const uint64_t w = gdb_pack_digits(T, nd);
   if (p <= 10) {
-    out[m++] = '0'; dot = m; out[m++] = '.';
-    for (int z = 0; z < 10 - p; ++z) out[m++] = '0';
-    int take = p < 6 ? p : 6;
-    for (int z = 0; z < take; ++z) out[m++] = dg[z];
+    put_packed(s, gdb_packed_zero_dot(), 2 + (10 - p));
+    put_packed(s, w, L);
   } else {
-    int ip = p - 10;
-    for (int z = 0; z < ip; ++z) out[m++] = dg[z];
-    if (ip < 6) { dot = m; out[m++] = '.'; for (int z = ip; z < 6; ++z) out[m++] = dg[z]; }
-  }
-  if (dot >= 0) while (m > dot + 2 && out[m - 1] == '0') --m;
-  s.write(out, m);
+    const int ip = p - 10;
+    if (ip < 6) put_packed(s, gdb_packed_insert_dot(w, ip), ip + 1 + (L > ip ? L - ip : 1));
+    else put_packed(s, w, 6);
+  }
   return true;
 }
 
@@ -349,6 +372,22 @@
   }
   return false;
 }
+struct AltTokens {
+  const char* s;
+  int len, i;
+  int idx;
+  GDB_HD AltTokens(const char* s_, int len_) : s(s_), len(len_), i(0), idx(-1) {}
+  GDB_HD bool next(const char*& tok, int& tlen) {
+    while (i < len && s[i] == '|') ++i;
+    if (i >= len) return false;
+    int j = i;
+    while (j < len && s[j] != '|') ++j;
+    tok = s + i; tlen = j - i;
+    i = j;
+    ++idx;
+    return true;
+  }
+};
 GDB_HD bool allele_is_symbolic(const char* a, int n) {
   if (n > 0 && a[0] == '&') return true;
   if (n == 1 && a[0] == '*') return true;
@@ -386,7 +425,7 @@
     const char* alt = cell_field<char>(fr, pl, pl.f_ALT, c, alt_len);
     bool deletion = false, has_nr = false;
     const char* tok; int tl;
-    for (int i = 0; alt_token(alt, alt_len, i, tok, tl); ++i) {
+    for (AltTokens at(alt, alt_len); at.next(tok, tl);) {
       ++nalt;
       if (tl > 0 && tok[0] == '&') has_nr = true;
       if (ref_len > 1 && !allele_is_symbolic(tok, tl) && tl < ref_len) deletion = true;
@@ -744,6 +783,7 @@
   TieScratch tie;
   ScalarPre pre;
   HugeSites huge;
+  const int64_t* first_cell_at;
 };
 
 GDB_HD bool inc_is_spanning(const SiteCtx& cx, int64_t t, int64_t s_k) {
@@ -1123,10 +1163,15 @@
   return nmerged++;
 }
 
-GDB_HD const char* site_first_ref(const SiteCtx& cx, int64_t s_k, int& len) {
+GDB_HD const char* site_first_ref(const SiteCtx& cx, int64_t k, int64_t s_k, int& len) {
+  len = 0;
+  if (cx.first_cell_at) {
+    const int64_t c = cx.first_cell_at[k];
+    if (c >= 0 && field_valid(cx.cm, c, cx.pl.f_REF)) return cell_field<char>(cx.fr, cx.pl, cx.pl.f_REF, c, len);
+    return nullptr;
+  }
   int64_t lo = 0, hi = cx.fr.ncells;
   while (lo < hi) { int64_t mid = (lo + hi) >> 1; if (cx.fr.begin[mid] < s_k) lo = mid + 1; else hi = mid; }
-  len = 0;
   if (lo < cx.fr.ncells && cx.fr.begin[lo] == s_k && field_valid(cx.cm, lo, cx.pl.f_REF)) return cell_field<char>(cx.fr, cx.pl, cx.pl.f_REF, lo, len);
   return nullptr;
 }
@@ -1154,8 +1199,8 @@
       int lowest = -1;
       int lowest_pl = 0x7FFFFFFF;
       const char* tok; int tl;
-      for (int i = 0; alt_token(alt, alt_len, i, tok, tl); ++i) {
-        int aidx = i + 1;
+      for (AltTokens at(alt, alt_len); at.next(tok, tl);) {
+        int aidx = at.idx + 1;
         if (allele_is_deletion(ref_len, tok, tl)) {
           if (lowest < 0) lowest = aidx;
           if (pl_exists) {
@@ -1176,7 +1221,7 @@
       if (lut) lut[lowest] = (int8_t)found;
       if (lut && pl.min_PL_GT_for_spanning_deletions && pl.produce_GT_field && pl_exists && pl.f_GT >= 0 && field_valid(cx.cm, c, pl.f_GT)) {
         int nr_idx = -1;
-        for (int i = 0; alt_token(alt, alt_len, i, tok, tl); ++i) if (tl > 0 && tok[0] == '&') nr_idx = i + 1;
+        for (AltTokens at(alt, alt_len); at.next(tok, tl);) if (tl > 0 && tok[0] == '&') nr_idx = at.idx + 1;
         int red2in[3] = {0, lowest, nr_idx};
         int nred = nr_idx >= 0 ? 3 : 2;
         int best_min = 0x7FFFFFFF, best_a = -1, best_b = -1;
@@ -1216,18 +1261,18 @@
     } else {
       bool suffix_needed = ref_len < mref_len;
       const char* tok; int tl;
-      for (int i = 0; alt_token(alt, alt_len, i, tok, tl); ++i) {
+      for (AltTokens at(alt, alt_len); at.next(tok, tl);) {
         if (tl > 0 && tok[0] == '&') continue;
         AlleleRef cand{tok, tl, (suffix_needed && !allele_is_symbolic(tok, tl)) ? ref_len : -1, 0u};
         cand.hash = allele_hash(cand.p, cand.len, cand.suffix_from, mref, mref_len);
         const int found = find_or_add(cand);
-        if (lut && i + 1 <= nalt) lut[i + 1] = (int8_t)found;
+        if (lut && at.idx + 1 <= nalt) lut[at.idx + 1] = (int8_t)found;
       }
     }
     if (write_luts) cx.hl.iflags[t] = iflag;
 }
 
-template <class Sink> GDB_HD void site_emit(const SiteCtx& cx, int64_t k, Sink& sink, bool write_luts, uint32_t* err) {
+template <bool BCF, class Sink> GDB_HD void site_emit_as(const SiteCtx& cx, int64_t k, Sink& sink, bool write_luts, uint32_t* err) {
   const CombinePlan& pl = cx.pl;
   const int64_t s_k = cx.rec.start[k], e_k = cx.rec.end[k];
   const int64_t hb = cx.hl.base[k], he = cx.hl.base[k + 1];
@@ -1237,7 +1282,7 @@
   const HugeSiteOut* hsite = (cx.huge.enabled && cx.huge.index[k] >= 0 && !cx.huge.out[cx.huge.index[k]].fallback) ? &cx.huge.out[cx.huge.index[k]] : nullptr;
   {
     if (hsite) { mref = hsite->mref; mref_len = hsite->mref_len; }
-    else mref = site_first_ref(cx, s_k, mref_len);
+    else mref = site_first_ref(cx, k, s_k, mref_len);
     if (!hsite) for (int64_t t = hb; t < he; ++t) {
       int64_t c = cx.hl.cell[t];
       if (cx.fr.begin[c] != s_k || !field_valid(cx.cm, c, pl.f_REF)) continue;
@@ -1277,8 +1322,8 @@
       int alt_len;
       const char* alt = cell_field<char>(cx.fr, pl, pl.f_ALT, c, alt_len);
       const char* tok; int tl;
-      for (int i = 0; alt_token(alt, alt_len, i, tok, tl); ++i)
-        if (tl > 0 && tok[0] == '&' && i + 1 <= (int)GDB_CF_NALT(cf)) cx.hl.i2m[cx.hl.i2m_off[t] + i + 1] = (int8_t)(num_merged - 1);
+      for (AltTokens at(alt, alt_len); at.next(tok, tl);)
+        if (tl > 0 && tok[0] == '&' && at.idx + 1 <= (int)GDB_CF_NALT(cf)) cx.hl.i2m[cx.hl.i2m_off[t] + at.idx + 1] = (int8_t)(num_merged - 1);
     }
   }
   const bool ref_block_only = (mref_len == 1 && nmerged == 1 && non_ref_exists);
@@ -1299,7 +1344,7 @@
   int ci = find_contig(cx.qw, s_k);
   if (ci < 0) { *err |= GDB_ERR_INTERNAL; ci = 0; }
   const GdbContig& ctg = cx.qw.contigs[ci];
-  if (pl.bcf_mode) {
+  if constexpr (BCF) {
     int n_fmt = 0;
     for (uint32_t m = fmt_mask; m; m &= m - 1) ++n_fmt;
     bcf_put_u32(sink, (uint32_t)ctg.rid);
@@ -1523,6 +1568,9 @@
       else sink.write(cx.names.text + cx.names.field_name_off[f], cx.names.field_name_len[f]);
     }
   }
+}
+template <class Sink> GDB_HD void site_emit(const SiteCtx& cx, int64_t k, Sink& sink, bool write_luts, uint32_t* err) {
+  if (cx.pl.bcf_mode) site_emit_as<true>(cx, k, sink, write_luts, err); else site_emit_as<false>(cx, k, sink, write_luts, err);
 }
 
 struct EntryCtx {
diff --git a/genomicsdb_amd/csrc/core/gdb_stages.hpp b/genomicsdb_amd/csrc/core/gdb_stages.hpp
--- a/genomicsdb_amd/csrc/core/gdb_stages.hpp
+++ b/genomicsdb_amd/csrc/core/gdb_stages.hpp
@@ -117,6 +117,19 @@
   if (cm.cflags[c] & GDB_CF_HEAVY) heavy_count[c - c_base] = khi - klo + 1;
   return true;
 }
+GDB_HD void stage_first_cell(const FragmentView& fr, const RecordTable& rec, int64_t c, int64_t qb, int64_t qe, const int32_t* first_record_at,
+                             int64_t* first_cell_at) {
+  const int64_t b = fr.begin[c];
+  if (b < qb || b > qe || (c > 0 && fr.begin[c - 1] == b)) return;
+  int64_t k;
+  if (first_record_at) k = first_record_at[b - qb];
+  else {
+    int64_t lo = 0, hi = rec.npos;
+    while (lo < hi) { int64_t mid = (lo + hi) >> 1; if (rec.start[mid] < b) lo = mid + 1; else hi = mid; }
+    k = lo;
+  }
+  if (k < rec.npos && rec.start[k] == b) first_cell_at[k] = c;
+}
 GDB_HD uint64_t stage_packed_word(const CombinePlan& pl, const DiffPacked& pk, uint64_t vmask, uint32_t cflags, int word) {
   uint64_t acc = 0;
   const int j0 = word * pk.per_word;
diff --git a/genomicsdb_amd/csrc/kernels/gdb_pipeline.hip b/genomicsdb_amd/csrc/kernels/gdb_pipeline.hip
--- a/genomicsdb_amd/csrc/kernels/gdb_pipeline.hip
+++ b/genomicsdb_amd/csrc/kernels/gdb_pipeline.hip
@@ -232,7 +232,7 @@
   return v;
 }
 __global__ void k_cell_ranges(FragmentView fr, CombinePlan pl, CellMeta cm, RecordTable rec, int64_t c_base, int64_t n, int64_t qb, int64_t qe,
-                              int64_t* heavy_count, int32_t* in_window_count, const int32_t* first_record_at, DiffPacked pk) {
+                              int64_t* heavy_count, int32_t* in_window_count, const int32_t* first_record_at, DiffPacked pk, int64_t* first_cell_at) {
   const int64_t i = (int64_t)blockIdx.x * blockDim.x + threadIdx.x;
   const int lane = threadIdx.x & 63;
   bool live = false;
@@ -242,6 +242,7 @@
     const int64_t c = c_base + i;
     live = stage_cell_range(fr, cm, rec, c, c_base, qb, qe, heavy_count, first_record_at, klo, khi);
     if (live) { vm = cm.vmask[c]; cf = cm.cflags[c]; dp = cm.dpval[c]; } else klo = -1 - (int64_t)lane;
+    stage_first_cell(fr, rec, c, qb, qe, first_record_at, first_cell_at);
   }
   const int64_t prev_key = __shfl_up(klo, 1, 64);
   const bool head = lane == 0 || prev_key != klo;
@@ -525,7 +526,7 @@
     HugeSiteOut& o = out[bi];
     if (tid == 0) {
       int len0 = 0;
-      s_mref = site_first_ref(cx, s_k, len0);
+      s_mref = site_first_ref(cx, k, s_k, len0);
       s_mref_len = len0;
       s_key = ((unsigned long long)(uint32_t)len0 << 32) | 0xFFFFFFFFull;
       s_flags[0] = s_flags[1] = s_flags[2] = s_flags[3] = 0;
@@ -736,7 +737,7 @@
 #ifndef GDBAMD_SITE_ATTR
 #define GDBAMD_SITE_ATTR __attribute__((amdgpu_waves_per_eu(4)))
 #endif
-__global__ void __launch_bounds__(64) GDBAMD_SITE_ATTR k_site_size(const SiteCtx* __restrict__ sxp, const int32_t* __restrict__ order, char* __restrict__ staging, SpillPool spill, int32_t* __restrict__ spill_chunk, uint32_t* err) {
+template <bool BCF> __device__ __forceinline__ void site_size_body(const SiteCtx* __restrict__ sxp, const int32_t* __restrict__ order, char* __restrict__ staging, const SpillPool& spill, int32_t* __restrict__ spill_chunk, uint32_t* err) {
   const SiteCtx& sx = *sxp;
   __shared__ uint32_t strip[64 * kSiteStripWords];
   int64_t k = (int64_t)blockIdx.x * blockDim.x + threadIdx.x;
@@ -745,7 +746,7 @@
   uint32_t e = 0;
   uint32_t* mine = strip + threadIdx.x * kSiteStripWords;
   LdsSpillSink cs((gdb_lds_char*)mine, (uint32_t)kSiteCap, spill, k);
-  site_emit(sx, k, cs, true, &e);
+  site_emit_as<BCF>(sx, k, cs, true, &e);
   cs.flush();
   sx.so.prefix_len[k] = cs.n;
   spill_chunk[k] = (cs.n > (uint32_t)kSiteCap && cs.complete()) ? 0 : -1;
@@ -753,6 +754,12 @@
   uint4* dst = reinterpret_cast<uint4*>(staging + (size_t)k * kSiteStride);
   for (uint32_t q = 0; (q << 4) < nstaged; ++q) dst[q] = make_uint4(mine[4 * q], mine[4 * q + 1], mine[4 * q + 2], mine[4 * q + 3]);
   if (e) atomicOr(err, e);
+}
+__global__ void __launch_bounds__(64) GDBAMD_SITE_ATTR k_site_size(const SiteCtx* __restrict__ sxp, const int32_t* __restrict__ order, char* __restrict__ staging, SpillPool spill, int32_t* __restrict__ spill_chunk, uint32_t* err) {
+  site_size_body<false>(sxp, order, staging, spill, spill_chunk, err);
+}
+__global__ void __launch_bounds__(64) GDBAMD_SITE_ATTR k_site_size_bcf(const SiteCtx* __restrict__ sxp, const int32_t* __restrict__ order, char* __restrict__ staging, SpillPool spill, int32_t* __restrict__ spill_chunk, uint32_t* err) {
+  site_size_body<true>(sxp, order, staging, spill, spill_chunk, err);
 }
 __global__ void __launch_bounds__(256) k_site_copy(const uint32_t* __restrict__ prefix_len, const char* __restrict__ staging, const char* __restrict__ spill_buf,
                                                    const int32_t* __restrict__ spill_chunk, int64_t k_begin, int64_t k_end,
@@ -800,7 +807,7 @@
     return;
   } else {
     ByteSink bs(dst);
-    site_emit(sx, k, bs, false, &e);
+    site_emit_as<false>(sx, k, bs, false, &e);
   }
   arena[chunk_off[(k + 1) * nchunks] - page_base - 1] = '\n';
   if (e) atomicOr(err, e);
@@ -2531,7 +2538,7 @@
     for (uint32_t i = kSiteCap; i < n; ++i) dst[i] = tail[i - kSiteCap];
   } else {
     ByteSink bs(dst);
-    site_emit(sx, k, bs, false, &e);
+    site_emit_as<true>(sx, k, bs, false, &e);
   }
   const uint32_t mask = sx.so.fmt_mask[k];
   int q = 0;
@@ -3308,7 +3315,7 @@
   DevBuf<uint64_t> ev_keys, ev_keys_sorted; DevBuf<int64_t> ev_delta, ev_incl; DevBuf<int32_t> run_end, run_excl;
   DevBuf<int64_t> bpos, bnrec, rbase; DevBuf<int32_t> bcov, bdel;
   DevBuf<int64_t> rstart, rend;
-  DevBuf<int32_t> diff, first_record_at; DevBuf<uint64_t> diff_packed; DevBuf<int64_t> heavy_count, hoff;
+  DevBuf<int32_t> diff, first_record_at; DevBuf<uint64_t> diff_packed; DevBuf<int64_t> heavy_count, hoff, first_cell_at;
   DevBuf<uint64_t> inc_keys, inc_keys_sorted; DevBuf<int64_t> inc_vals, inc_vals_sorted, hbase;
   DevBuf<uint32_t> lut_len, i2m_off; DevBuf<int8_t> i2m, gt_override; DevBuf<uint8_t> iflags;
   DevBuf<uint8_t> num_alleles, rflags; DevBuf<uint32_t> fmt_mask, prefix_len; DevBuf<char> site_staging, spill_buf; DevBuf<int32_t> spill_chunk;
@@ -4847,8 +4854,10 @@
     }
     first_record_at = S.first_record_at.p;
   }
+  S.first_cell_at.ensure((size_t)P);
+  HIP_CHECK(hipMemsetAsync(S.first_cell_at.p, 0xFF, (size_t)P * sizeof(int64_t), st));
   STAGE("k_cell_ranges");
-  hipLaunchKernelGGL(k_cell_ranges, dim3(blocks_for(CW)), dim3(kBlock), 0, st, fr, pl, cm, rec, c_base, CW, qb, qe, S.heavy_count.p, S.counters.p, first_record_at, pk);
+  hipLaunchKernelGGL(k_cell_ranges, dim3(blocks_for(CW)), dim3(kBlock), 0, st, fr, pl, cm, rec, c_base, CW, qb, qe, S.heavy_count.p, S.counters.p, first_record_at, pk, S.first_cell_at.p);
   S.incl_scan(pk.w, pk.w, (size_t)pk.nwords * stride, rocprim::plus<uint64_t>());
   hipLaunchKernelGGL(k_unpack_counts, dim3(blocks_for(stride)), dim3(kBlock), 0, st, pk, nf, stride, da);
   S.excl_scan(S.heavy_count.p, S.hoff.p, (size_t)CW);
@@ -4967,7 +4976,7 @@
   }
   HugeSites huge;
   memset(&huge, 0, sizeof(huge));
-  SiteCtx sx0{fr, pl, cm, rec, hl, pc, nt, qw, so, med, big, tie, pre, huge};
+  SiteCtx sx0{fr, pl, cm, rec, hl, pc, nt, qw, so, med, big, tie, pre, huge, S.first_cell_at.p};
   const int32_t huge_threshold = (P > 0 && T / P >= 24 && P <= (int64_t)kMaxHugeRecords) ? 24 : kHugeRecord;
   if (T > (int64_t)huge_threshold && !getenv("GDBAMD_NO_HUGE_SITES")) {
     S.huge_index.ensure((size_t)P); S.huge_list.ensure(kMaxHugeRecords); S.huge_out.ensure(kMaxHugeRecords); S.d_sx0.ensure(1);
@@ -4977,7 +4986,7 @@
     hipLaunchKernelGGL(k_site_huge, dim3(1024), dim3(kHugeBlock), 0, st, (const SiteCtx*)S.d_sx0.p, (const int32_t*)S.huge_list.p, (const int32_t*)(S.counters.p + 3), S.huge_out.p, S.err.p, S.counters.p + 6);
     huge.index = S.huge_index.p; huge.out = S.huge_out.p; huge.enabled = 1;
   }
-  SiteCtx sx{fr, pl, cm, rec, hl, pc, nt, qw, so, med, big, tie, pre, huge};
+  SiteCtx sx{fr, pl, cm, rec, hl, pc, nt, qw, so, med, big, tie, pre, huge, S.first_cell_at.p};
   S.d_sx.ensure(1);
   HIP_CHECK(hipMemcpyAsync(S.d_sx.p, &sx, sizeof(SiteCtx), hipMemcpyHostToDevice, st));
   STAGE("k_site_size");
@@ -4993,7 +5002,8 @@
       site_order = S.site_ord.p;
     }
   }
-  hipLaunchKernelGGL(k_site_size, dim3(blocks_for(P, 64)), dim3(64), 0, st, S.d_sx.p, site_order, S.site_staging.p, SpillPool{S.spill_buf.p}, S.spill_chunk.p, S.err.p);
+  if (pl.bcf_mode) hipLaunchKernelGGL(k_site_size_bcf, dim3(blocks_for(P, 64)), dim3(64), 0, st, S.d_sx.p, site_order, S.site_staging.p, SpillPool{S.spill_buf.p}, S.spill_chunk.p, S.err.p);
+  else hipLaunchKernelGGL(k_site_size, dim3(blocks_for(P, 64)), dim3(64), 0, st, S.d_sx.p, site_order, S.site_staging.p, SpillPool{S.spill_buf.p}, S.spill_chunk.p, S.err.p);
   S.remap_total.ensure(1);
   HIP_CHECK(hipMemsetAsync(S.remap_total.p, 0, sizeof(unsigned long long), st));
   for (int i = 0; i < pl.n_format; ++i)
```

Result: faster. 41.53 million (median of 6 runs) (+2.6%).
